# wq2012/SpectralCluster

Measured on AMD Instinct MI355X. Metric: predict() calls/sec, n=8192 d=256 ICASSP2018 (GraphCut, eigengap k in [2,20], cosine k-means), higher is better.
Workload: dtype f64; 1 GPU; icassp2018_graphcut_n8192_d256_k8_max20; n_samples=8192, n_features=256, parallelism=replicas x1, collectives=none

## Files before the change

### include/spectralcluster_amd.h

```cpp
#ifndef SPECTRALCLUSTER_AMD_H_
#define SPECTRALCLUSTER_AMD_H_

#include <stddef.h>
#include <stdint.h>

#ifdef __cplusplus
extern "C" {
#endif

#define SC_ABI_VERSION 10
#define SC_MAX_OPS 16
#define SC_MAX_BLUR_RADIUS 32
#define SC_MAX_EIG 128
#define SC_MAX_STAGES 16

typedef struct sc_handle_s* sc_handle;

typedef enum sc_status {
  SC_OK = 0,
  SC_ERR_INVALID = -1,
  SC_ERR_OOM = -2,
  SC_ERR_HIP = -3,
  SC_ERR_NOT_CONVERGED = -4,
  SC_ERR_UNSUPPORTED = -5,
// ... 104 lines not shown

typedef struct sc_diag {
  int32_t n;
  int32_t n_clusters_raw;
  int32_t n_clusters;
  int32_t eig_path;
  double max_delta;
  int32_t n_eigenvalues;
  int32_t eig_descending;
  double eigenvalues[SC_MAX_EIG];
  int32_t eig_matvec_passes;
  int32_t eig_block;
  int32_t eig_basis;
  int32_t eig_cycles;
  double eig_max_residual;
  int32_t kmeans_iterations;
  int32_t symmetry_state;
  int32_t eig_host_chain;
  int32_t eig_fallback;
  float stage_ms[SC_MAX_STAGES];
  int32_t diffuse_path;
  int32_t free_candidates;
  int32_t free_overflow_rows;
  int32_t free_tiles_run;
} sc_diag;

int sc_abi_version(void);
int sc_struct_sizes(int* config_bytes, int* diag_bytes);

enum { SC_DTYPE_F64 = 0, SC_DTYPE_F32 = 1, SC_DTYPE_F16 = 2, SC_DTYPE_BF16 = 3 };
enum { SC_MEM_HOST = 0, SC_MEM_DEVICE = 1 };
typedef struct sc_array {
  const void* data;
  int32_t dtype;
  int32_t location;
  int64_t rows, cols;
  int64_t row_stride;
  int64_t col_stride;
} sc_array;
int sc_array_layout(int* array_bytes, int* field_offsets);
int sc_device_count(void);
int sc_device_info(int device, char* name, int name_len, char* arch, int arch_len,
                   int* compute_units, int64_t* total_mem_bytes);

int sc_create(int device, sc_handle* out);
int sc_destroy(sc_handle h);
int sc_reserve(sc_handle h, int n_max, int d_max);
const char* sc_last_error(sc_handle h);
int sc_synchronize(sc_handle h);
void* sc_stream(sc_handle h);
int sc_set_profiling(sc_handle h, int level);
int sc_set_diffuse_mode(sc_handle h, int mode);
int sc_set_free_prune(sc_handle h, int on);

int sc_config_default(sc_config* cfg);
int sc_gaussian_weights(double sigma, int32_t* radius, double* weights);
int sc_set_blur_weights(sc_handle h, int radius, const double* weights);

int sc_predict(sc_handle h, const double* x, int n, int d, const sc_config* cfg,
               int64_t* labels, sc_diag* diag);

int sc_predict_array(sc_handle h, const sc_array* x, const sc_config* cfg, int64_t* labels,
                     sc_diag* diag);

int sc_set_embeddings(sc_handle h, const double* x, int n, int d);
int sc_set_embeddings_array(sc_handle h, const sc_array* x);
int sc_compute_affinity(sc_handle h);
int sc_set_affinity(sc_handle h, const double* affinity, int n);
int sc_eig_ncluster(sc_handle h, const sc_config* cfg, sc_diag* diag);
int sc_num_eigenvalues(sc_handle h);
int sc_get_eigenvalues(sc_handle h, double* out, int count);
int sc_num_eigenvectors(sc_handle h);
int sc_get_eigenvectors(sc_handle h, double* out, int n, int ncols);
int sc_cluster(sc_handle h, const sc_config* cfg, int n_clusters,
               int64_t* labels, sc_diag* diag);
int sc_set_constraint(sc_handle h, const double* constraint_matrix, int n);
int sc_set_constraint_band(sc_handle h, const double* band, int n);
int sc_set_constraint_pairs(sc_handle h, const int32_t* rows, const int32_t* cols,
                            const double* vals, int count, int n);
int sc_constraint_pairs_info(sc_handle h, int* count, size_t* pair_bytes);
int sc_clear_constraint(sc_handle h);
int sc_apply_constraint(sc_handle h, const sc_config* cfg);
int sc_constraint_info(sc_handle h, int* kind, int* n, size_t* band_bytes,
                       size_t* dense_bytes);
int sc_run_resident(sc_handle h, const sc_config* cfg, int64_t* labels,
                    sc_diag* diag);
int sc_eig_ncluster_sweep(sc_handle h, const sc_config* cfg, const double* p_values, int count,
                          sc_diag* diags);
int sc_sweep_adopt(sc_handle h, const sc_config* cfg, int index, sc_diag* diag);
int sc_predict_batch(sc_handle h, const double* const* xs, const int* ns, int d,
                     int count, const sc_config* cfg, int64_t* const* labels,
                     sc_diag* diags);
int sc_predict_batch_streams(sc_handle h, const double* const* xs, const int* ns, int d,
                             int count, const sc_config* cfg, int64_t* const* labels,
                             sc_diag* diags, int streams);
int sc_predict_batch_grouped(sc_handle h, const double* const* xs, const int* ns, int d,
                             int count, const sc_config* cfg, int64_t* const* labels,
                             sc_diag* diags, int group);
int sc_predict_batch_arrays(sc_handle h, const sc_array* xs, int count, const sc_config* cfg,
                            int64_t* const* labels, sc_diag* diags, int group, int streams);
int sc_predict_batch_constrained(sc_handle h, const sc_array* xs, const double* const* bands,
                                 int count, const sc_config* cfg, int64_t* const* labels,
                                 sc_diag* diags, int group);
typedef struct sc_constraint_desc {
  int32_t kind;
  int32_t count;
// ... 69 lines not shown

typedef struct sc_pool_s* sc_pool;
enum { SC_POOL_CACHE = 0, SC_POOL_CENTROIDS = 1 };
int sc_pool_create(sc_handle h, int capacity, int d, int u1, int u2, sc_pool* out);
int sc_pool_destroy(sc_pool pool);
int sc_pool_reset(sc_pool pool, int slot);
int sc_pool_rows(sc_pool pool, int slot);
int sc_pool_append(sc_pool pool, const int32_t* slots, const int32_t* counts, int count,
                   const sc_array* rows);
int sc_pool_precluster(sc_pool pool, const int32_t* slots, int count, int64_t* const* labels_out);
int sc_pool_centroids(sc_pool pool, int slot, sc_array* out);
int sc_pool_fallback(sc_pool pool, const int32_t* slots, int count, double distance_threshold,
                     int64_t* const* labels_out);
int sc_pool_cache(sc_pool pool, int slot, sc_array* out);
int sc_pool_get(sc_pool pool, int slot, int what, double* out);
int sc_pool_compress(sc_pool pool, int slot);

int sc_affinity_stats(sc_handle h, double* out);
int sc_affinity_gmm_bic(sc_handle h, int diagonal_offset, double* bic1, double* bic2);
int sc_naive_cluster(sc_handle h, const double* x, int n, int d, double threshold,
                     double adaptation_threshold, double* centroids, int32_t* counts,
                     int32_t* n_centroids, int capacity, int64_t* labels);

int sc_stage_ingest(sc_handle h, const sc_array* x, double* out);
int sc_stage_affinity(sc_handle h, const double* x, int n, int d, double* out);
int sc_stage_refine(sc_handle h, int op, const sc_config* cfg, const double* in,
                    int n, double* out);
int sc_stage_constraint(sc_handle h, const sc_config* cfg, const double* affinity,
                        const double* constraint_matrix, int n, double* out);
int sc_stage_constraint_band(sc_handle h, const sc_config* cfg, const double* affinity,
                             const double* band, int n, double* out);
int sc_stage_constraint_band_group(sc_handle h, const sc_config* cfg, int count, const int32_t* ns,
                                   const double* const* affinities, const double* const* bands,
                                   double* const* outs);
int sc_stage_constraint_pairs(sc_handle h, const sc_config* cfg, const double* affinity,
                              const int32_t* rows, const int32_t* cols, const double* vals,
                              int count, int n, double* out);
int sc_stage_constraint_pairs_group(sc_handle h, const sc_config* cfg, int count,
                                    const int32_t* ns, const double* const* affinities,
                                    const int32_t* const* rows, const int32_t* const* cols,
                                    const double* const* vals, const int32_t* counts,
                                    double* const* outs);
int sc_stage_diffuse_rowstats(sc_handle h, const double* a, int n, int mode, double* rowmax,
                              double* rowsum, int32_t* info);
enum {
  SC_BLOCK_ROUTE_SYM = 1,
  SC_BLOCK_ROUTE_TWO_PRODUCT = 2,
  SC_BLOCK_ROUTE_GROUPED = 4
};
int sc_stage_block_operator(sc_handle h, int count, const int32_t* ns,
                            const double* const* matrices, const double* const* cvecs,
                            const double* const* pvecs, const double* const* vs_scales,
                            const double* const* vs, double* const* ws, int route);
int sc_stage_krylov_state(sc_handle h, int32_t* info, double* q, double* t, double* g, double* c,
                          double* p);
enum { SC_FRONT_ROUTE_SINGLE = 0, SC_FRONT_ROUTE_GROUPED = 1, SC_FRONT_ROUTE_SWEEP = 2,
       SC_FRONT_ROUTE_SHORT_SWEEP = 3, SC_FRONT_ROUTE_SHORT_WAVE = 4 };
enum {
  SC_FRONT_INFO_DIFFUSE_PATH = 0,
  SC_FRONT_INFO_SYMMETRIC = 1,
  SC_FRONT_INFO_FOLDED_ROWNORM = 2,
  SC_FRONT_INFO_FREE_OP = 3,
  SC_FRONT_INFO_DIGITS_FUSED = 4,
  SC_FRONT_INFO_BLUR_KERNEL = 5,
  SC_FRONT_INFO_BLUR_ROWS = 6,
  SC_FRONT_INFO_FREE_CANDIDATES = 7,
  SC_FRONT_INFO_FREE_OVERFLOW_ROWS = 8,
  SC_FRONT_INFO_FREE_FORMS_S = 9,
  SC_FRONT_INFO_CROP_SOURCE = 10,
  SC_FRONT_INFO_CUT_KERNEL = 11,
  SC_FRONT_INFO_WRITTEN = 12,
  SC_FRONT_INFO_LAUNCHES = 13,
  SC_FRONT_INFO_COUNT = 16
};
typedef struct sc_front_out {
  double* a0;
  double* cropval;
  double* cut;
  double* a;
  double* s;
  double* rowmax;
  double* rowsum;
  double* c;
  double* p;
  double* t;
  int32_t info[SC_FRONT_INFO_COUNT];
} sc_front_out;
int sc_stage_front(sc_handle h, int route, const sc_config* cfg, int count, const int32_t* ns,
                   int d, const double* const* xs, const double* affinity,
                   const double* p_values, sc_front_out* outs);
enum { SC_TD_BACKTRANSFORM_GLOBAL = 1 };
int sc_stage_tridiag(sc_handle h, const double* m, int n, const double* c, const double* p,
                     double* d, double* e, double* tau, double* reflectors);
int sc_stage_tridiag_values(sc_handle h, const double* d, const double* e, int n,
                            double* values_desc);
int sc_stage_td_backtransform(sc_handle h, const double* reflectors, const double* tau, int n,
                              double* z, int cols, int flags);
int sc_stage_laplacian(sc_handle h, int laplacian_type, const double* in, int n,
                       double* out);
int sc_stage_sym_eig(sc_handle h, const double* m, int n, int count, int descend,
                     double* values, double* vectors, sc_diag* diag);
int sc_stage_eig(sc_handle h, const double* m, int n, int count, int descend,
                 double* values, double* vectors, sc_diag* diag);
int sc_random_state_doubles(uint32_t seed, int count, double* out);
int sc_uniform_choice(int n, double u);
int sc_host_symmetric_eig(const double* a, int m, double* values, double* vectors);
int sc_host_symmetric_eig_partial(const double* a, int m, int need, double* values,
                                  double* vectors);
// ... 59 lines not shown
```

### spectralcluster_amd/_lib.py

```python

from __future__ import annotations

import ctypes
import os
import threading
import typing

import numpy as np

SC_MAX_OPS = 16
SC_MAX_BLUR_RADIUS = 32
SC_MAX_EIG = 128
SC_MAX_STAGES = 16

SC_OK = 0
SC_ERR_INVALID = -1
SC_ERR_OOM = -2
SC_ERR_HIP = -3
SC_ERR_NOT_CONVERGED = -4
SC_ERR_UNSUPPORTED = -5
SC_ERR_NON_FINITE = -6

STAGE_NAMES = ("affinity", "refine", "diffuse", "scaling", "eig", "kmeans",
               "total", "blur", "threshold_sym", "matvec", "affinity_gemm",
# ... 138 lines not shown
      ("threshold", ctypes.c_double),
  ]


class ScConstraintDesc(ctypes.Structure):
  _fields_ = [
      ("kind", ctypes.c_int32),
      ("count", ctypes.c_int32),
      ("band", ctypes.POINTER(ctypes.c_double)),
      ("rows", ctypes.POINTER(ctypes.c_int32)),
      ("cols", ctypes.POINTER(ctypes.c_int32)),
      ("vals", ctypes.POINTER(ctypes.c_double)),
  ]


SC_AUTOTUNE_PERCENTILE_OVER_NME, SC_AUTOTUNE_PERCENTILE_SQRT_OVER_NME = 1, 2


class ScAutoTune(ctypes.Structure):
  _fields_ = [
      ("p_min", ctypes.c_double),
      ("p_max", ctypes.c_double),
      ("step", ctypes.c_double),
      ("levels", ctypes.c_int32),
      ("proxy", ctypes.c_int32),
  ]


AUTOTUNE_EVALUATE = ctypes.CFUNCTYPE(ctypes.c_int, _c_double_p, ctypes.c_int, _c_double_p,
                                     ctypes.c_void_p)

_c_int64_p = ctypes.POINTER(ctypes.c_int64)
_c_int_p = ctypes.POINTER(ctypes.c_int)
_handle_t = ctypes.c_void_p

PROTOTYPES = {
    "sc_abi_version": (ctypes.c_int, []),
    "sc_struct_sizes": (ctypes.c_int, [ctypes.POINTER(ctypes.c_int),
                                       ctypes.POINTER(ctypes.c_int)]),
    "sc_array_layout": (ctypes.c_int, [ctypes.POINTER(ctypes.c_int),
                                       ctypes.POINTER(ctypes.c_int)]),
    "sc_device_count": (ctypes.c_int, []),
    "sc_device_info": (ctypes.c_int, [ctypes.c_int, ctypes.c_char_p, ctypes.c_int,
                                      ctypes.c_char_p, ctypes.c_int, _c_int_p,
                                      _c_int64_p]),
    "sc_create": (ctypes.c_int, [ctypes.c_int, ctypes.POINTER(_handle_t)]),
    "sc_destroy": (ctypes.c_int, [_handle_t]),
    "sc_reserve": (ctypes.c_int, [_handle_t, ctypes.c_int, ctypes.c_int]),
    "sc_last_error": (ctypes.c_char_p, [_handle_t]),
    "sc_synchronize": (ctypes.c_int, [_handle_t]),
    "sc_set_profiling": (ctypes.c_int, [_handle_t, ctypes.c_int]),
    "sc_set_diffuse_mode": (ctypes.c_int, [_handle_t, ctypes.c_int]),
    "sc_set_free_prune": (ctypes.c_int, [_handle_t, ctypes.c_int]),
    "sc_stage_diffuse_rowstats": (ctypes.c_int, [_handle_t, _c_double_p, ctypes.c_int,
                                                 ctypes.c_int, _c_double_p, _c_double_p,
                                                 ctypes.POINTER(ctypes.c_int32)]),
    "sc_stage_block_operator": (ctypes.c_int, [_handle_t, ctypes.c_int,
                                               ctypes.POINTER(ctypes.c_int32),
                                               ctypes.POINTER(_c_double_p),
                                               ctypes.POINTER(_c_double_p),
                                               ctypes.POINTER(_c_double_p),
                                               ctypes.POINTER(_c_double_p),
                                               ctypes.POINTER(_c_double_p),
                                               ctypes.POINTER(_c_double_p), ctypes.c_int]),
    "sc_stage_krylov_state": (ctypes.c_int, [_handle_t, ctypes.POINTER(ctypes.c_int32),
                                             _c_double_p, _c_double_p, _c_double_p, _c_double_p,
                                             _c_double_p]),
    "sc_stage_front": (ctypes.c_int, [_handle_t, ctypes.c_int, ctypes.POINTER(ScConfig),
                                      ctypes.c_int, ctypes.POINTER(ctypes.c_int32), ctypes.c_int,
                                      ctypes.POINTER(_c_double_p), _c_double_p, _c_double_p,
                                      ctypes.POINTER(ScFrontOut)]),
    "sc_stage_tridiag": (ctypes.c_int, [_handle_t, _c_double_p, ctypes.c_int, _c_double_p,
                                        _c_double_p, _c_double_p, _c_double_p, _c_double_p,
                                        _c_double_p]),
    "sc_stage_tridiag_values": (ctypes.c_int, [_handle_t, _c_double_p, _c_double_p, ctypes.c_int,
                                               _c_double_p]),
    "sc_stage_td_backtransform": (ctypes.c_int, [_handle_t, _c_double_p, _c_double_p,
                                                 ctypes.c_int, _c_double_p, ctypes.c_int,
                                                 ctypes.c_int]),
    "sc_config_default": (ctypes.c_int, [ctypes.POINTER(ScConfig)]),
    "sc_gaussian_weights": (ctypes.c_int, [ctypes.c_double,
                                           ctypes.POINTER(ctypes.c_int32),
                                           _c_double_p]),
    "sc_predict": (ctypes.c_int, [_handle_t, _c_double_p, ctypes.c_int, ctypes.c_int,
                                  ctypes.POINTER(ScConfig), _c_int64_p,
                                  ctypes.POINTER(ScDiag)]),
    "sc_set_embeddings": (ctypes.c_int, [_handle_t, _c_double_p, ctypes.c_int,
                                         ctypes.c_int]),
    "sc_predict_array": (ctypes.c_int, [_handle_t, ctypes.POINTER(ScArray),
                                        ctypes.POINTER(ScConfig), _c_int64_p,
                                        ctypes.POINTER(ScDiag)]),
    "sc_set_embeddings_array": (ctypes.c_int, [_handle_t, ctypes.POINTER(ScArray)]),
    "sc_predict_batch_arrays": (ctypes.c_int, [_handle_t, ctypes.POINTER(ScArray), ctypes.c_int,
                                               ctypes.POINTER(ScConfig),
                                               ctypes.POINTER(_c_int64_p),
                                               ctypes.POINTER(ScDiag), ctypes.c_int,
                                               ctypes.c_int]),
    "sc_predict_batch_constrained": (ctypes.c_int, [_handle_t, ctypes.POINTER(ScArray),
                                                    ctypes.POINTER(_c_double_p), ctypes.c_int,
                                                    ctypes.POINTER(ScConfig),
                                                    ctypes.POINTER(_c_int64_p),
                                                    ctypes.POINTER(ScDiag), ctypes.c_int]),
    "sc_constraint_desc_layout": (ctypes.c_int, [ctypes.POINTER(ctypes.c_int),
                                                 ctypes.POINTER(ctypes.c_int)]),
    "sc_predict_batch_constraints": (ctypes.c_int, [_handle_t, ctypes.POINTER(ScArray),
                                                    ctypes.POINTER(ScConstraintDesc), ctypes.c_int,
                                                    ctypes.POINTER(ScConfig),
                                                    ctypes.POINTER(_c_int64_p),
                                                    ctypes.POINTER(ScDiag), ctypes.c_int]),
    "sc_stage_ingest": (ctypes.c_int, [_handle_t, ctypes.POINTER(ScArray), _c_double_p]),
    "sc_compute_affinity": (ctypes.c_int, [_handle_t]),
    "sc_set_affinity": (ctypes.c_int, [_handle_t, _c_double_p, ctypes.c_int]),
    "sc_eig_ncluster": (ctypes.c_int, [_handle_t, ctypes.POINTER(ScConfig),
                                       ctypes.POINTER(ScDiag)]),
    "sc_num_eigenvalues": (ctypes.c_int, [_handle_t]),
    "sc_get_eigenvalues": (ctypes.c_int, [_handle_t, _c_double_p, ctypes.c_int]),
    "sc_num_eigenvectors": (ctypes.c_int, [_handle_t]),
    "sc_get_eigenvectors": (ctypes.c_int, [_handle_t, _c_double_p, ctypes.c_int,
                                           ctypes.c_int]),
    "sc_cluster": (ctypes.c_int, [_handle_t, ctypes.POINTER(ScConfig), ctypes.c_int,
# ... 422 lines not shown
```

### spectralcluster_amd/csrc/api.hip

```cpp
#include <algorithm>
#include <array>
#include <cmath>
#include <cstdio>
#include <cstdlib>
#include <cstring>
#include <vector>

#include <condition_variable>
#include <mutex>
#include <string>
#include <thread>

#include "handle.h"
#include "host_pool.h"

int ensure_matrices(sc_handle h, int n, int d, bool affinity_copy) {
  h->krylov_m = 0;
  const size_t ldn = matrix_ld(n);
  const size_t nn = (size_t)n * ldn * sizeof(double);
  if (affinity_copy) SC_TRY(grow(h, h->A0, nn));
  SC_TRY(grow(h, h->B1, nn));
  SC_TRY(grow(h, h->B2, nn));
  if (d > 0) {
    const size_t ldx = round_up(d, 16);
// ... 3 lines not shown
  const size_t nv = (size_t)round_up(n, 16) * sizeof(double);
  SC_TRY(grow(h, h->rowmax, nv));
  SC_TRY(grow(h, h->rowsum, nv));
  SC_TRY(grow(h, h->cvec, nv));
  SC_TRY(grow(h, h->pvec, nv));
  SC_TRY(grow(h, h->tvec, nv));
  SC_TRY(grow(h, h->deg, nv));
  SC_TRY(grow(h, h->splitk, gemm_splitk_workspace_bytes()));
  SC_TRY(grow(h, h->dvec, nv));
  SC_TRY(grow(h, h->cut, nv));
  SC_TRY(grow(h, h->cropval, nv));
  SC_TRY(grow(h, h->statp, (size_t)2 * n * gemm_tile_dim(n) * sizeof(double)));
  SC_TRY(grow(h, h->rmpart, (size_t)n * blur_tile_columns(n, 8) * sizeof(double)));
  SC_TRY(grow(h, h->blurw, (2 * SC_MAX_BLUR_RADIUS + 1) * sizeof(double)));
  return SC_OK;
}

int ensure_tilemap(sc_handle h, int n) {
  const int nt = gemm_tile_dim(n);
  if (nt <= kTilemapTableMax) {
    if (!h->tilemap_table.p) {
      std::vector<int2> all, one;
      for (int t = 1; t <= kTilemapTableMax; ++t) {
        h->tilemap_off[t] = (int)all.size();
        gemm_build_sym_tilemap(t, &one);
        all.insert(all.end(), one.begin(), one.end());
      }
      SC_TRY(grow(h, h->tilemap_table, all.size() * sizeof(int2)));
      SC_HIP(h, hipMemcpyAsync(h->tilemap_table.p, all.data(), all.size() * sizeof(int2),
                               hipMemcpyHostToDevice, h->stream));
      SC_HIP(h, hipStreamSynchronize(h->stream));
    }
    h->tilemap_cur = ptr<int2>(h->tilemap_table) + h->tilemap_off[nt];
    return SC_OK;
  }
  if (h->tilemap_nt != nt) {
    std::vector<int2> map;
    gemm_build_sym_tilemap(nt, &map);
    SC_TRY(grow(h, h->tilemap, map.size() * sizeof(int2)));
    SC_HIP(h, hipMemcpyAsync(h->tilemap.p, map.data(), map.size() * sizeof(int2),
                             hipMemcpyHostToDevice, h->stream));
    SC_HIP(h, hipStreamSynchronize(h->stream));
    h->tilemap_nt = nt;
  }
  h->tilemap_cur = ptr<int2>(h->tilemap);
  return SC_OK;
}

int ensure_eig(sc_handle h, int n) {
  const size_t nq = (size_t)n * kLdq * sizeof(double);
  if (h->Q.bytes < nq) h->krylov_m = 0;
  SC_TRY(grow(h, h->Q, nq));
  SC_TRY(grow(h, h->Q2, nq));
  SC_TRY(grow(h, h->Vs, (size_t)n * kEigBlock * sizeof(double)));
  SC_TRY(grow(h, h->W, (size_t)n * kEigBlock * sizeof(double)));
  SC_TRY(grow(h, h->partial, std::max((size_t)kProjBlocks * kLdq * kEigBlock,
                                       lz_partial_doubles(n)) * sizeof(double)));
  SC_TRY(grow(h, h->T, (size_t)kLdq * kLdq * sizeof(double)));
  SC_TRY(grow(h, h->Y, (size_t)kLdq * kLdq * sizeof(double)));
  SC_TRY(grow(h, h->Yt, (size_t)kLdq * kLdq * sizeof(double)));
  SC_TRY(grow(h, h->theta, kLdq * sizeof(double)));
  SC_TRY(grow(h, h->resid, kLdq * sizeof(double)));
  SC_TRY(grow(h, h->G, 256 * sizeof(double)));
  SC_TRY(grow(h, h->Rinv, 256 * sizeof(double)));
  SC_TRY(grow(h, h->Hbuf, (size_t)kLdq * kEigBlock * sizeof(double)));
  SC_TRY(grow(h, h->hsq, 16 * sizeof(double)));
  SC_TRY(grow(h, h->colnorm, (size_t)kProjBlocks * kMaxVectors * sizeof(double)));
  if (h->flags.bytes < 16 * sizeof(int)) {
    SC_TRY(grow(h, h->flags, 16 * sizeof(int)));
    SC_HIP(h, hipMemsetAsync(h->flags.p, 0, 16 * sizeof(int), h->stream));
  }
  SC_TRY(grow(h, h->mvsym, matvec_sym_workspace_doubles(n) * sizeof(double)));
  SC_TRY(ensure_vectors(h, n, kMaxCols));
  return SC_OK;
}

int ensure_vectors(sc_handle h, int n, int cols) {
  cols = std::max(cols, kMaxCols);
  SC_TRY(grow(h, h->E, (size_t)round_up(n, 16) * cols * sizeof(double)));
  SC_TRY(grow(h, h->Eio, (size_t)n * cols * sizeof(double)));
  return SC_OK;
}

int ensure_gen(sc_handle h, int n) {
  const size_t ldv = round_up(n, 16);
  const size_t nv = ldv * sizeof(double);
  SC_TRY(grow(h, h->crvec, nv));
  SC_TRY(grow(h, h->thetai, kLdq * sizeof(double)));
  SC_TRY(grow(h, h->Vre, ldv * kGenMax * sizeof(double)));
  SC_TRY(grow(h, h->Vim, ldv * kGenMax * sizeof(double)));
  SC_TRY(grow(h, h->gpart, (size_t)gen_residual_blocks(n) * 32 * sizeof(double)));
  SC_TRY(grow(h, h->gsrc, 16 * sizeof(int)));
  SC_TRY(grow(h, h->genL, (size_t)kGenMax * kGenMax * sizeof(double)));
  return SC_OK;
}

extern "C" int sc_abi_version(void) { return SC_ABI_VERSION; }
extern "C" int sc_struct_sizes(int* config_bytes, int* diag_bytes) {
  if (config_bytes) *config_bytes = (int)sizeof(sc_config);
  if (diag_bytes) *diag_bytes = (int)sizeof(sc_diag);
  return SC_OK;
}

extern "C" int sc_device_count(void) {
  int c = 0;
  if (hipGetDeviceCount(&c) != hipSuccess) return 0;
  return c;
}

extern "C" int sc_device_info(int device, char* name, int name_len, char* arch,
                              int arch_len, int* compute_units,
                              int64_t* total_mem_bytes) {
  hipDeviceProp_t prop;
  if (hipGetDeviceProperties(&prop, device) != hipSuccess) return SC_ERR_HIP;
  if (name && name_len > 0) snprintf(name, name_len, "%s", prop.name);
  if (arch && arch_len > 0) snprintf(arch, arch_len, "%s", prop.gcnArchName);
  if (compute_units) *compute_units = prop.multiProcessorCount;
  if (total_mem_bytes) *total_mem_bytes = (int64_t)prop.totalGlobalMem;
  return SC_OK;
}


extern "C" int sc_create(int device, sc_handle* out) {
  if (!out) return SC_ERR_INVALID;
  *out = nullptr;
  int count = 0;
  if (hipGetDeviceCount(&count) != hipSuccess || count <= 0) return SC_ERR_HIP;
  if (device < 0 || device >= count) return SC_ERR_INVALID;
  sc_handle h = new sc_handle_s();
  h->device = device;
  if (hipSetDevice(device) != hipSuccess ||
      hipStreamCreateWithFlags(&h->stream, hipStreamNonBlocking) != hipSuccess) {
    delete h;
    return SC_ERR_HIP;
  }
  const unsigned ev_flags = hipEventDisableSystemFence;
  for (int i = 0; i < 48; ++i) {
    if (hipEventCreateWithFlags(&h->ev[i], ev_flags) != hipSuccess) {
      delete h;
      return SC_ERR_HIP;
    }
  }
  if (hipHostMalloc(reinterpret_cast<void**>(&h->h_theta), 3 * kLdq * sizeof(double)) !=
          hipSuccess ||
      hipHostMalloc(reinterpret_cast<void**>(&h->h_flags), 16 * sizeof(int)) !=
          hipSuccess ||
      hipHostMalloc(reinterpret_cast<void**>(&h->h_rr),
                    (2 * kHostRRSingle * kHostRRSingle + 64) * sizeof(double)) != hipSuccess) {
    delete h;
    return SC_ERR_HIP;
  }
  *out = h;
  return SC_OK;
}

extern "C" int sc_destroy(sc_handle h) {
  if (!h) return SC_OK;
  for (sc_handle sub : h->pool) sc_destroy(sub);
  h->pool.clear();
  for (sc_handle sub : h->gslots) sc_destroy(sub);
  h->gslots.clear();
  for (sc_handle sub : h->gshort) sc_destroy(sub);
  h->gshort.clear();
  hipSetDevice(h->device);
  hipStreamSynchronize(h->stream);
  DevBuf* bufs[] = {&h->X,     &h->Xn,    &h->A0,     &h->B1,      &h->B2,    &h->rowmax,
                    &h->rowsum, &h->cvec,  &h->pvec,   &h->tvec,    &h->deg,   &h->blurw, &h->blur_tmp, &h->dvec, &h->cut, &h->rmpart, &h->splitk, &h->tilemap, &h->tilemap_table, &h->cropval, &h->statp, &h->crvec, &h->thetai, &h->Vre, &h->Vim, &h->gpart, &h->gsrc, &h->genL, &h->ahc_size, &h->ahc_chain, &h->ahc_Z, &h->ahc_lab, &h->ahc_cent, &h->fb_part, &h->fb_small, &h->sck_slots, &h->sck_part, &h->sck_rec, &h->sck_mats, &h->fb_x, &h->fb_cent, &h->fb_int, &h->Cq, &h->Cband, &h->Cpairs, &h->Cporig, &h->cp[0], &h->cp[1], &h->cp[2], &h->cp[3], &h->cp[4], &h->symflag,
                    &h->Q,     &h->Q2,    &h->Vs,     &h->W,       &h->partial, &h->T,
                    &h->Y,     &h->Yt,    &h->theta,  &h->resid,   &h->G,     &h->Rinv,
                    &h->Hbuf,  &h->hsq,   &h->colnorm, &h->flags,  &h->E,     &h->Ek,   &h->Eio,
                    &h->td_d,  &h->td_e,  &h->td_theta, &h->td_work, &h->td_tau, &h->td_panel, &h->mvsym,
                    &h->kXc,   &h->kxsq,  &h->kclosest, &h->kcand, &h->kenorm, &h->krnd,
                    &h->kcent, &h->klab32, &h->klab64, &h->kinfo, &h->kchain, &h->gkrnd, &h->gpack, &h->gypack, &h->ginfo, &h->glabels, &h->gjtab, &h->gsftab, &h->gswtab,
                    &h->kbig, &h->kbigw, &h->fq, &h->ft32, &h->fy1, &h->fR, &h->fscal, &h->fwords, &h->fcand, &h->fY, &h->fsplit, &h->fypart, &h->frpart, &h->fq2part, &h->fmx64, &h->ftau64, &h->fplan, &h->Xalt, &h->Xstage, &h->gneg};
  for (DevBuf* b : bufs)
    if (b->p) hipFree(b->p);
  for (DevBuf& b : h->kgen)
    if (b.p) hipFree(b.p);
  for (int i = 0; i < 48; ++i) hipEventDestroy(h->ev[i]);
  if (h->h_theta) hipHostFree(h->h_theta);
  if (h->h_flags) hipHostFree(h->h_flags);
  if (h->h_rr) hipHostFree(h->h_rr);
  if (h->h_free) hipHostFree(h->h_free);
  if (h->h_reduce) hipHostFree(h->h_reduce);
  if (h->h_sck) hipHostFree(h->h_sck);
  if (h->sync_ev) hipEventDestroy(h->sync_ev);
  for (int b = 0; b < kGroupBanks; ++b) {
    if (h->gbank_ev[b]) hipEventDestroy(h->gbank_ev[b]);
    if (h->gbank_stream[b]) hipStreamDestroy(h->gbank_stream[b]);
  }
  if (h->gchain_stream) hipStreamDestroy(h->gchain_stream);
  if (h->copy_stream) hipStreamDestroy(h->copy_stream);
  if (h->gcheck_ev) hipEventDestroy(h->gcheck_ev);
  for (sc_handle lane : h->glanes) sc_destroy(lane);
  h->glanes.clear();
  delete h->gpool;
  if (h->h_gpack) hipHostFree(h->h_gpack);
  if (h->h_gypack) hipHostFree(h->h_gypack);
  if (h->h_gjtab) hipHostFree(h->h_gjtab);
  if (h->h_gsftab) hipHostFree(h->h_gsftab);
  if (h->h_gswtab) hipHostFree(h->h_gswtab);
// ... 1142 lines not shown
```

### spectralcluster_amd/csrc/eig.hip

```cpp
#include <algorithm>
#include <cstring>
#include <mutex>

#include "sc_internal.h"

namespace sc {

typedef double v4f64 __attribute__((ext_vector_type(4)));
constexpr int B = kEigBlock;
constexpr int RB = 256 / B;
static_assert(B == 8 || B == 16, "block width must divide the 16-wide MFMA tile");

__device__ __forceinline__ uint64_t splitmix64(uint64_t x) {
  x += 0x9E3779B97F4A7C15ull;
  x = (x ^ (x >> 30)) * 0xBF58476D1CE4E5B9ull;
  x = (x ^ (x >> 27)) * 0x94D049BB133111EBull;
  return x ^ (x >> 31);
}
__device__ __forceinline__ double hash_uniform(uint64_t seed, uint64_t idx) {
  const uint64_t h = splitmix64(seed ^ splitmix64(idx));
  return (double)(h >> 11) * (2.0 / 9007199254740992.0) - 1.0;
}

__global__ void k_random_block(double* W, int n, uint64_t seed) {
// ... 39 lines not shown
  for (; ch < nchunks; ch += kMvWaves) {
    if (ch + kMvWaves < nchunks) load(nxt, ch + kMvWaves);
    const int kb = ch * 32 + 2 * lg;
    double b[8];
#pragma unroll
    for (int t = 0; t < 8; ++t) {
      const int k = kb + 8 * (t >> 1) + (t & 1);
      b[t] = (k < n && li < B) ? Vs[(size_t)k * B + li] : 0.0;
    }
#pragma unroll
    for (int q = 0; q < 4; ++q) {
      const double a0 = (kb + 8 * q < n) ? cur[q].x : 0.0;
      const double a1 = (kb + 8 * q + 1 < n) ? cur[q].y : 0.0;
      acc0 = __builtin_amdgcn_mfma_f64_16x16x4f64(a0, b[2 * q], acc0, 0, 0, 0);
      acc1 = __builtin_amdgcn_mfma_f64_16x16x4f64(a1, b[2 * q + 1], acc1, 0, 0, 0);
    }
#pragma unroll
    for (int q = 0; q < 4; ++q) cur[q] = nxt[q];
  }
#pragma unroll
  for (int r = 0; r < 4; ++r) red[wave][lane][r] = acc0[r] + acc1[r];
  __syncthreads();
  if (wave == 0) {
#pragma unroll
    for (int r = 0; r < 4; ++r) {
      double sum = 0.0;
#pragma unroll
      for (int w = 0; w < kMvWaves; ++w) sum += red[w][lane][r];
      const int row = r0 + lg + 4 * r;
      if (row < n && li < B)
        W[(size_t)row * B + li] =
            __builtin_fma(cvec ? cvec[row] : 1.0, sum,
                          pvec ? pvec[row] * V[(size_t)row * ldv + li] : 0.0);
    }
  }
}
__global__ __launch_bounds__(64 * kMvWaves) void k_block_matvec(
    const double* __restrict__ S, int ld, int n, const double* __restrict__ cvec,
    const double* __restrict__ pvec, const double* __restrict__ V, int ldv,
    const double* __restrict__ Vs, double* __restrict__ W) {
  block_matvec_body(S, ld, n, cvec, pvec, V, ldv, Vs, W);
}
__global__ __launch_bounds__(64 * kMvWaves) void k_block_matvec_g(const GroupOf<MatvecItem> g) {
  const MatvecItem& a = g.s[blockIdx.y];
  if ((int)blockIdx.x * 16 >= a.n) return;
  block_matvec_body(a.S, a.ld, a.n, a.cvec, a.pvec, a.V, a.ldv, a.Vs, a.W);
}

constexpr int kSymTile = 128;
constexpr int kSymPitch = 34;
__device__ __forceinline__ int sym_item_id(int I, int J, int nt) {
  return I * nt - I * (I - 1) / 2 + (J - I);
}
__device__ __forceinline__ void block_matvec_sym_body(
    const double* __restrict__ S, int ld, int n, const double* __restrict__ Vs,
    double* __restrict__ pdirect, double* __restrict__ pmirror, int nt) {
  __shared__ __attribute__((aligned(16))) double smem[4 * 32 * kSymPitch];
  int I = 0, rem = blockIdx.x, rowlen = nt;
  while (rem >= rowlen) {
    rem -= rowlen;
    --rowlen;
    ++I;
  }
  const int J = I + rem;
  const bool diag = I == J;
  const int lane = threadIdx.x & 63, wave = threadIdx.x >> 6;
  const int li = lane & 15, lg = lane >> 4;
  const int r0 = I * kSymTile + 32 * wave;
  const int c0 = J * kSymTile;
  double* patch = smem + wave * (32 * kSymPitch);
  double bm[8];
#pragma unroll
  for (int t = 0; t < 8; ++t) {
    const int row = r0 + 4 * t + lg;
    bm[t] = (row < n && li < B) ? Vs[(size_t)row * B + li] : 0.0;
  }
  v4f64 accd[2] = {{0.0, 0.0, 0.0, 0.0}, {0.0, 0.0, 0.0, 0.0}};
  v4f64 accm[4][2];
#pragma unroll
  for (int cs = 0; cs < 4; ++cs)
#pragma unroll
    for (int ct = 0; ct < 2; ++ct) accm[cs][ct] = (v4f64){0.0, 0.0, 0.0, 0.0};
  double2 a[1][2][4];
  auto load = [&](int buf, int cs) {
#pragma unroll
    for (int rt = 0; rt < 2; ++rt) {
      int row = r0 + 16 * rt + li;
      row = row < n ? row : n - 1;
      const double* src = S + (size_t)row * ld + c0 + 32 * cs + 2 * lg;
#pragma unroll
      for (int q = 0; q < 4; ++q) {
        if (c0 + 32 * cs + 8 * q + 2 * lg + 1 < ld)
          a[buf][rt][q] = *reinterpret_cast<const double2*>(src + 8 * q);
        else
          a[buf][rt][q] = make_double2(0.0, 0.0);
      }
    }
  };
#pragma unroll
  for (int cs = 0; cs < 4; ++cs) {
    constexpr int cur = 0;
    load(cur, cs);
    const int kb = c0 + 32 * cs + 2 * lg;
#pragma unroll
    for (int rt = 0; rt < 2; ++rt) {
      const bool rok = r0 + 16 * rt + li < n;
#pragma unroll
      for (int q = 0; q < 4; ++q) {
        if (!rok || kb + 8 * q >= n) a[cur][rt][q].x = 0.0;
        if (!rok || kb + 8 * q + 1 >= n) a[cur][rt][q].y = 0.0;
      }
    }
    double b[8];
#pragma unroll
    for (int t = 0; t < 8; ++t) {
      const int k = kb + 8 * (t >> 1) + (t & 1);
      b[t] = (k < n && li < B) ? Vs[(size_t)k * B + li] : 0.0;
    }
#pragma unroll
    for (int rt = 0; rt < 2; ++rt)
#pragma unroll
      for (int q = 0; q < 4; ++q) {
        accd[rt] = __builtin_amdgcn_mfma_f64_16x16x4f64(a[cur][rt][q].x, b[2 * q], accd[rt], 0, 0, 0);
        accd[rt] = __builtin_amdgcn_mfma_f64_16x16x4f64(a[cur][rt][q].y, b[2 * q + 1], accd[rt], 0, 0, 0);
      }
    if (!diag) {
#pragma unroll
      for (int rt = 0; rt < 2; ++rt)
#pragma unroll
        for (int q = 0; q < 4; ++q)
          *reinterpret_cast<double2*>(patch + (16 * rt + li) * kSymPitch + 8 * q + 2 * lg) =
              a[cur][rt][q];
      __builtin_amdgcn_fence(__ATOMIC_RELEASE, "wavefront");
      __builtin_amdgcn_wave_barrier();
#pragma unroll
      for (int ct = 0; ct < 2; ++ct)
#pragma unroll
        for (int t = 0; t < 8; ++t) {
          const double at = patch[(4 * t + lg) * kSymPitch + 16 * ct + li];
          accm[cs][ct] = __builtin_amdgcn_mfma_f64_16x16x4f64(at, bm[t], accm[cs][ct], 0, 0, 0);
        }
      __builtin_amdgcn_fence(__ATOMIC_ACQUIRE, "wavefront");
      __builtin_amdgcn_wave_barrier();
    }
  }
  const size_t item = blockIdx.x;
  if (li < B) {
#pragma unroll
    for (int rt = 0; rt < 2; ++rt)
#pragma unroll
      for (int r = 0; r < 4; ++r)
        pdirect[(item * kSymTile + 32 * wave + 16 * rt + lg + 4 * r) * B + li] = accd[rt][r];
  }
  if (diag) return;
  __syncthreads();
  double* red = smem;
  if (li < B) {
#pragma unroll
    for (int cs = 0; cs < 4; ++cs)
#pragma unroll
      for (int ct = 0; ct < 2; ++ct)
#pragma unroll
        for (int r = 0; r < 4; ++r)
          red[(wave * kSymTile + 32 * cs + 16 * ct + lg + 4 * r) * B + li] = accm[cs][ct][r];
  }
  __syncthreads();
  for (int e = threadIdx.x; e < kSymTile * B; e += 256)
    pmirror[item * (kSymTile * B) + e] =
        ((red[e] + red[kSymTile * B + e]) + red[2 * kSymTile * B + e]) + red[3 * kSymTile * B + e];
}
__global__ __launch_bounds__(256) void k_block_matvec_sym(
    const double* __restrict__ S, int ld, int n, const double* __restrict__ Vs,
    double* __restrict__ pdirect, double* __restrict__ pmirror, int nt) {
  block_matvec_sym_body(S, ld, n, Vs, pdirect, pmirror, nt);
}
__global__ __launch_bounds__(256) void k_block_matvec_sym_g(const GroupOf<MatvecItem> g) {
  const MatvecItem& a = g.s[blockIdx.y];
  const int nt = (a.n + kSymTile - 1) / kSymTile;
  if ((int)blockIdx.x >= nt * (nt + 1) / 2) return;
  block_matvec_sym_body(a.S, a.ld, a.n, a.Vs, a.slabs, a.slabs + (size_t)(nt * (nt + 1) / 2) * kSymTile * B, nt);
}

__device__ __forceinline__ void matvec_sym_reduce_body(
    const double* __restrict__ pdirect, const double* __restrict__ pmirror, int nt, int n,
    const double* __restrict__ cvec, const double* __restrict__ pvec,
    const double* __restrict__ V, int ldv, double* __restrict__ W) {
  const int R = blockIdx.x / 4;
  const int e = (blockIdx.x & 3) * 256 + threadIdx.x;
  const int rl = e / B, v = e % B;
  const int row = R * kSymTile + rl;
  double acc = 0.0;
  const int total = nt;
  for (int s0 = 0; s0 < total; s0 += 8) {
    double x[8];
#pragma unroll
    for (int u = 0; u < 8; ++u) {
      const int sidx = s0 + u;
      x[u] = 0.0;
      if (sidx < nt - R) {
        x[u] = pdirect[(size_t)sym_item_id(R, R + sidx, nt) * (kSymTile * B) + e];
      } else if (sidx < total) {
        x[u] = pmirror[(size_t)sym_item_id(sidx - (nt - R), R, nt) * (kSymTile * B) + e];
      }
    }
#pragma unroll
    for (int u = 0; u < 8; ++u) acc += x[u];
  }
  if (row < n) W[(size_t)row * B + v] =
      __builtin_fma(cvec ? cvec[row] : 1.0, acc, pvec ? pvec[row] * V[(size_t)row * ldv + v] : 0.0);
}
__global__ __launch_bounds__(256) void k_matvec_sym_reduce(
    const double* __restrict__ pdirect, const double* __restrict__ pmirror, int nt, int n,
    const double* __restrict__ cvec, const double* __restrict__ pvec,
    const double* __restrict__ V, int ldv, double* __restrict__ W) {
  matvec_sym_reduce_body(pdirect, pmirror, nt, n, cvec, pvec, V, ldv, W);
}
__global__ __launch_bounds__(256) void k_matvec_sym_reduce_g(const GroupOf<MatvecItem> g) {
  const MatvecItem& a = g.s[blockIdx.y];
  const int nt = (a.n + kSymTile - 1) / kSymTile;
  if ((int)blockIdx.x >= nt * 4) return;
  matvec_sym_reduce_body(a.slabs, a.slabs + (size_t)(nt * (nt + 1) / 2) * kSymTile * B, nt, a.n,
                         a.cvec, a.pvec, a.V, a.ldv, a.W);
}

constexpr int kProjGroups = 256 / B;
constexpr int kProjAcc = (kLdq + kProjGroups - 1) / kProjGroups;
__global__ __launch_bounds__(256) void k_proj_partial(
    const double* __restrict__ Q, int ldq, int m, const double* __restrict__ W,
    int n, double* __restrict__ partial) {
  __shared__ double Ql[8][kLdq];
  __shared__ double Wl[8][B];
  const int tid = threadIdx.x;
  const int jj = tid % B, ig = tid / B;
  const int rows_per = (n + gridDim.x - 1) / gridDim.x;
  const int rbeg = blockIdx.x * rows_per;
  const int rend = min(n, rbeg + rows_per);
  double acc[kProjAcc];
#pragma unroll
  for (int q = 0; q < kProjAcc; ++q) acc[q] = 0.0;
  for (int r = rbeg; r < rend; r += 8) {
    __syncthreads();
    for (int e = tid; e < 8 * m; e += 256) {
      const int rr = e / m, i = e - rr * m;
      Ql[rr][i] = (r + rr < rend) ? Q[(size_t)(r + rr) * ldq + i] : 0.0;
    }
    if (tid < 8 * B) {
      const int rr = tid / B;
      Wl[rr][jj] = (r + rr < rend) ? W[(size_t)(r + rr) * B + jj] : 0.0;
    }
    __syncthreads();
#pragma unroll
    for (int rr = 0; rr < 8; ++rr) {
      const double w = Wl[rr][jj];
#pragma unroll
      for (int q = 0; q < kProjAcc; ++q)
        if (ig + kProjGroups * q < m)
          acc[q] = __builtin_fma(Ql[rr][ig + kProjGroups * q], w, acc[q]);
    }
  }
  double* out = partial + (size_t)blockIdx.x * (kLdq * B);
#pragma unroll
  for (int q = 0; q < kProjAcc; ++q)
    if (ig + kProjGroups * q < m) out[(ig + kProjGroups * q) * B + jj] = acc[q];
}

__global__ __launch_bounds__(256) void k_reduce_H(
    const double* __restrict__ partial, int nparts, int m, double* __restrict__ Hbuf,
    double* __restrict__ T, int ldt, int col0, int accumulate,
    double* __restrict__ hsq) {
  __shared__ double sq[32];
  const int tid = threadIdx.x;
  const int sub = tid & 7;
  const int e = blockIdx.x * 32 + (tid >> 3);
  double h = 0.0;
// ... 91 lines not shown
  const double gii = __shfl(g, i * 9), gjj = __shfl(g, j * 9);
  double defect = 0.0;
  if (flag_mode == 2 && gii != 0.0 && gjj != 0.0) defect = fabs(g - (i == j ? 1.0 : 0.0));
#pragma unroll
  for (int o = 1; o < 64; o <<= 1) defect = fmax(defect, __shfl_xor(defect, o));
  double r = 0.0;
  int mask = 0;
  double pmax = 0.0, pmin = __builtin_huge_val();
#pragma unroll
  for (int k = 0; k < B; ++k) {
    const double d = __shfl(g, k * 9);
    const double total = __shfl(gii, k * 8) + (hsq ? hsq[k] : 0.0);
    const bool drop = !(d > 1e-22 * total) || !(d > 0.0);
    const double rk = drop ? 0.0 : sqrt(d);
    if (drop) {
      mask |= 1 << k;
    } else {
      pmax = fmax(pmax, rk);
      pmin = fmin(pmin, rk);
    }
    double row = 0.0;
    if (i == k && !drop) row = j == k ? rk : (j > k ? g / rk : 0.0);
    if (i == k) r = row;
    const double rki = __shfl(row, k * 8 + i), rkj = __shfl(row, k * 8 + j);
    if (i > k && j > k) g -= rki * rkj;
  }
  const double rii = __shfl(r, i * 9), rjj = __shfl(r, j * 9);
  double ri = 0.0;
#pragma unroll
  for (int srow = B - 1; srow >= 0; --srow) {
    double v = 0.0;
#pragma unroll
    for (int k = srow + 1; k < B; ++k) {
      const double rsk = __shfl(r, srow * 8 + k), rkj = __shfl(ri, k * 8 + j);
      if (k <= j) v -= rsk * rkj;
    }
    if (i == srow && j >= i && rii != 0.0 && rjj != 0.0)
      ri = i == j ? 1.0 / rii : v / rii;
  }
  Rinv[tid] = ri;
  if (tid == 0 && flags != nullptr) {
    flags[0] = mask;
    if (defect_flag != nullptr) *defect_flag = (defect > 0.1 || pmax > 1e3 * pmin) ? 1 : 0;
    if (sticky_flag != nullptr && (mask != 0 || (sticky_on_defect && defect > 0.1))) {
      if (*sticky_flag == 0) {
        sticky_flag[1] = sticky_m;
        sticky_flag[2] = flag_mode * 1000 + mask;
      }
      *sticky_flag = 1;
    }
  }
}

__global__ __launch_bounds__(256) void k_apply_rinv(
    double* __restrict__ W, int n, const double* __restrict__ Rinv,
    double* __restrict__ Qdst, int ldq, int col0, const double* __restrict__ cvec,
    double* __restrict__ Vs) {
  __shared__ double Rl[B * B];
  const int tid = threadIdx.x;
  if (tid < B * B) Rl[tid] = Rinv[tid];
  __syncthreads();
  const int jj = tid % B;
  const int r = blockIdx.x * RB + tid / B;
  const double w = r < n ? W[(size_t)r * B + jj] : 0.0;
  double v = 0.0;
#pragma unroll
  for (int k = 0; k < B; ++k) {
    const double wk = __shfl(w, k, B);
    v = __builtin_fma(wk, Rl[k * B + jj], v);
  }
  if (r < n) {
    W[(size_t)r * B + jj] = v;
    if (Qdst) Qdst[(size_t)r * ldq + col0 + jj] = v;
    if (Vs) Vs[(size_t)r * B + jj] = cvec[r] * v;
  }
}

constexpr int kLzThreads = 512;
constexpr int kLzPartStride = (kLdq + B) * B;
struct LzStep {
  double* W;
  int n;
  const double* Q;
  int ldq, m;
  int pre;
  const double* pre_partial;
  int pre_nparts;
  double* T;
  int ldt, col0;
  double* Gsave;
  double* hsq;
  int* flags;
  int arm_defect;
  double* Tzero;
  double* Qdst;
  int store_col;
  const double* vs_scale;
  double* Vs;
  int init_random;
  uint64_t seed;
  int want_proj, want_gram;
  double* partial;
};

__device__ __forceinline__ double lz_ordered_sum(const double* src, int nparts) {
  double acc = 0.0;
  for (int p0 = 0; p0 < nparts; p0 += 16) {
    double v[16];
#pragma unroll
    for (int u = 0; u < 16; ++u)
      v[u] = (p0 + u < nparts) ? src[(size_t)(p0 + u) * kLzPartStride] : 0.0;
#pragma unroll
    for (int u = 0; u < 16; ++u) acc += v[u];
  }
  return acc;
}

template <int ROWS>
__device__ __forceinline__ void lz_rows_body(const LzStep& a) {
  extern __shared__ __attribute__((aligned(16))) double smem[];
  constexpr int kPass = kLzThreads / B;
  const int m = a.m;
  const int mq = m + 1;
  double* Ql = smem;
  double* Hl = Ql + ROWS * mq;
  double* Rl = Hl + kLdq * B;
  double* Wl = Rl + B * B;
  double* Gs = Wl + ROWS * B;
  double* hs = Gs + B * B;
  const int tid = threadIdx.x;
  const int j = tid % B;
  const int r0 = blockIdx.x * ROWS;
  const bool first_wg = blockIdx.x == 0;
  const bool pre_proj = (a.pre >= 1 && a.pre <= 3) && m > 0;
  const bool pre_gram = a.pre >= 2;
  const bool use_h = pre_proj;
  const bool use_r = pre_gram;
  const bool use_q = m > 0 && (use_h || a.want_proj);
  const int nproj = pre_proj ? m * B : 0;
  double hsum[3] = {0.0, 0.0, 0.0};
#pragma unroll
  for (int u = 0; u < 3; ++u) {
    const int e = tid + u * kLzThreads;
    if (e < nproj) hsum[u] = lz_ordered_sum(a.pre_partial + e, a.pre_nparts);
    else if (pre_gram && e < nproj + B * B)
      hsum[u] = lz_ordered_sum(a.pre_partial + kLdq * B + (e - nproj), a.pre_nparts);
  }
  double told[3] = {0.0, 0.0, 0.0};
  double hsq_old = 0.0;
  if (first_wg && a.pre == 2) {
#pragma unroll
    for (int u = 0; u < 3; ++u) {
      const int e = tid + u * kLzThreads;
      if (e < nproj) told[u] = a.T[(size_t)(e / B) * a.ldt + a.col0 + (e % B)];
    }
    if (tid < B) hsq_old = a.hsq[tid];
  }
  if (!first_wg && a.pre == 2 && tid < B) hsq_old = a.hsq[tid];
  if (use_q)
    for (int e = tid; e < ROWS * m; e += kLzThreads) {
      const int rr = e / m, i = e - rr * m;
      Ql[rr * mq + i] = (r0 + rr < a.n) ? a.Q[(size_t)(r0 + rr) * a.ldq + i] : 0.0;
    }
  double w[ROWS / kPass];
#pragma unroll
  for (int q = 0; q < ROWS / kPass; ++q) {
    const int r = r0 + q * kPass + tid / B;
    w[q] = 0.0;
    if (r < a.n)
      w[q] = a.init_random ? hash_uniform(a.seed, (uint64_t)r * B + j) : a.W[(size_t)r * B + j];
  }
#pragma unroll
  for (int u = 0; u < 3; ++u) {
    const int e = tid + u * kLzThreads;
    if (e < nproj) Hl[e] = hsum[u];
    else if (pre_gram && e < nproj + B * B) Gs[e - nproj] = hsum[u];
  }
  if (tid < B * B) Rl[tid] = (tid / B == tid % B) ? 1.0 : 0.0;
  __syncthreads();
  if (pre_proj && a.pre != 3) {
    if (first_wg && a.T != nullptr) {
#pragma unroll
      for (int u = 0; u < 3; ++u) {
        const int e = tid + u * kLzThreads;
        if (e < nproj) {
          const int i = e / B, jc = a.col0 + (e % B);
          if (i <= jc) {
            const double t = a.pre == 2 ? told[u] + hsum[u] : hsum[u];
            a.T[(size_t)i * a.ldt + jc] = t;
            a.T[(size_t)jc * a.ldt + i] = t;
          }
        }
      }
    }
    if (tid < B) {
      double sq = 0.0;
      for (int i = 0; i < m; ++i) sq = __builtin_fma(Hl[i * B + tid], Hl[i * B + tid], sq);
      sq = a.pre == 2 ? hsq_old + sq : sq;
      if (first_wg && a.pre == 1) a.hsq[tid] = sq;
      hs[tid] = sq;
    }
  } else if (tid < B) {
    hs[tid] = 0.0;
  }
  if (first_wg && a.Tzero != nullptr)
    for (int e = tid; e < kLdq * kLdq; e += kLzThreads) a.Tzero[e] = 0.0;
  if (pre_gram) {
    if (pre_proj && tid < B * B) {
      const int a1 = tid / B, b1 = tid % B;
      double g = Gs[tid];
      for (int i = 0; i < m; ++i) g = __builtin_fma(-Hl[i * B + a1], Hl[i * B + b1], g);
      Gs[tid] = g;
    }
    __syncthreads();
    if (first_wg && a.pre == 2 && a.Gsave != nullptr && tid < B * B) a.Gsave[tid] = Gs[tid];
    if (tid < 64)
      chol8_wave(Gs, Rl, a.pre == 2 ? hs : nullptr, first_wg ? a.flags : nullptr,
                 first_wg ? a.flags + (a.pre == 3 ? 10 : 11) : nullptr, a.pre == 3 ? 2 : 1,
                 first_wg ? a.flags + 13 : nullptr, m, a.arm_defect != 0);
    __syncthreads();
  }
#pragma unroll
  for (int q = 0; q < ROWS / kPass; ++q) {
    const int rl = q * kPass + tid / B;
    const int r = r0 + rl;
    double x = w[q];
    if (use_h)
      for (int i = 0; i < m; ++i) x = __builtin_fma(-Ql[rl * mq + i], Hl[i * B + j], x);
    double v = x;
    if (use_r) {
      v = 0.0;
#pragma unroll
      for (int k = 0; k < B; ++k) v = __builtin_fma(__shfl(x, k, B), Rl[k * B + j], v);
    }
    if (r < a.n) {
      a.W[(size_t)r * B + j] = v;
      if (a.Qdst) a.Qdst[(size_t)r * a.ldq + a.store_col + j] = v;
      if (a.Vs) a.Vs[(size_t)r * B + j] = a.vs_scale[r] * v;
    }
    Wl[rl * B + j] = (r < a.n) ? v : 0.0;
  }
  if (!a.want_proj && !a.want_gram) return;
  __syncthreads();
  const int oproj = a.want_proj ? m * B : 0;
  const int nent = oproj + (a.want_gram ? B * B : 0);
  double* mine = a.partial + (size_t)blockIdx.x * kLzPartStride;
  for (int base = 0; base < nent; base += kLzThreads / 2) {
    const int e = base + (tid >> 1), half = tid & 1;
    double acc = 0.0;
    if (e < nent) {
      const int rbeg = half * (ROWS / 2);
      if (e < oproj) {
        const int i = e / B, jj = e % B;
#pragma unroll 8
        for (int rr = 0; rr < ROWS / 2; ++rr)
          acc = __builtin_fma(Ql[(rbeg + rr) * mq + i], Wl[(rbeg + rr) * B + jj], acc);
      } else {
        const int g = e - oproj, a1 = g / B, b1 = g % B;
#pragma unroll 8
        for (int rr = 0; rr < ROWS / 2; ++rr)
          acc = __builtin_fma(Wl[(rbeg + rr) * B + a1], Wl[(rbeg + rr) * B + b1], acc);
      }
    }
    const double other = __shfl_xor(acc, 1);
    if (e < nent && half == 0)
      mine[e < oproj ? e : kLdq * B + (e - oproj)] = acc + other;
  }
}
template <int ROWS>
__global__ __launch_bounds__(kLzThreads) void k_lz_rows(const LzStep a) {
  lz_rows_body<ROWS>(a);
}
template <int ROWS>
__global__ __launch_bounds__(kLzThreads) void k_lz_rows_g(const GroupOf<LzStep> g) {
  const LzStep& a = g.s[blockIdx.y];
  if ((int)blockIdx.x * ROWS >= a.n) return;
  lz_rows_body<ROWS>(a);
}

__device__ __forceinline__ double fast_rcp(double x) {
  double r = __builtin_amdgcn_rcp(x);
  r = __builtin_fma(r, __builtin_fma(-x, r, 1.0), r);
  r = __builtin_fma(r, __builtin_fma(-x, r, 1.0), r);
  return r;
}
__device__ __forceinline__ double fast_rsqrt(double x) {
  double y = __builtin_amdgcn_rsq(x);
  y = __builtin_fma(y, 0.5 * __builtin_fma(-x * y, y, 1.0), y);
  y = __builtin_fma(y, 0.5 * __builtin_fma(-x * y, y, 1.0), y);
  return y;
}

template <bool YT_LDS>
__device__ __forceinline__ void jacobi_body(
    const double* __restrict__ src, int ldsrc, int m, int mode,
    const double* __restrict__ cvec, const double* __restrict__ pvec,
    const double* __restrict__ G, double* __restrict__ theta,
    double* __restrict__ Y, int ldy, double* __restrict__ resid,
    double* __restrict__ Yt_global, int* __restrict__ dbg) {
  extern __shared__ __attribute__((aligned(16))) double smem[];
  const long long t_begin = wall_clock64();
  const long long c_begin = clock64();
  const int mp = (m + 1) & ~1;
  const int lda = mp + 1;
  double* A = smem;
  double* cs = A + mp * lda;
  double* sn = cs + mp / 2;
  int* pp = reinterpret_cast<int*>(sn + mp / 2);
  int* qq = pp + mp / 2;
  double* Yl = sn + mp / 2 + mp / 2 + 2;
#define Yt(idx) (*(YT_LDS ? &Yl[idx] : &Yt_global[idx]))
  __shared__ int s_rot;
  const int tid = threadIdx.x;
  const int nth = blockDim.x;

  for (int e = tid; e < mp * mp; e += nth) {
    const int i = e / mp, j = e - i * mp;
    double v = 0.0;
    if (i < m && j < m) {
      v = src[(size_t)i * ldsrc + j];
      if (mode == 1) {
        v = cvec[i] * v * cvec[j];
        if (i == j) v += pvec[i];
      }
    }
    A[i * lda + j] = v;
    Yt((size_t)i * mp + j) = (i == j) ? 1.0 : 0.0;
  }
  __syncthreads();
  if (mode == 1) {
// ... 283 lines not shown
}
__global__ __launch_bounds__(256) void k_back_transform_g(const GroupOf<RitzItem> g) {
  const RitzItem& a = g.s[blockIdx.y];
  if ((int)blockIdx.x >= a.cols || a.n <= 0) return;
  back_transform_body(a.E, a.lde, a.n, a.tvec);
}
__device__ __forceinline__ void dense_vectors_member(const JacobiItem& a) {
  const int j = blockIdx.x;
  if (j >= a.m) return;
  for (int r = threadIdx.x; r < a.m; r += blockDim.x)
    a.E[(size_t)j * a.lde + r] = a.Y[(size_t)r * a.ldy + j];
  __syncthreads();
  back_transform_body(a.E, a.lde, a.m, a.tvec);
}
__global__ __launch_bounds__(256) void k_dense_vectors_g(const GroupOf<JacobiItem> g) {
  dense_vectors_member(g.s[blockIdx.y]);
}
__global__ __launch_bounds__(256) void k_dense_vectors_t(const JacobiItem* __restrict__ table) {
  const JacobiItem a = table[blockIdx.y];
  dense_vectors_member(a);
}

__global__ void k_rowmajor_to_colmajor(const double* __restrict__ src, int lds, int n,
                                       int cols, double* __restrict__ dst, int ldd) {
  const int e = blockIdx.x * blockDim.x + threadIdx.x;
  if (e >= n * cols) return;
  const int j = e / n, r = e - j * n;
  dst[(size_t)j * ldd + r] = src[(size_t)r * lds + j];
}
__global__ void k_colmajor_to_rowmajor(const double* __restrict__ src, int lds, int n,
                                       int cols, double* __restrict__ dst, int ldd) {
  const int e = blockIdx.x * blockDim.x + threadIdx.x;
  if (e >= n * cols) return;
  const int r = e / cols, j = e - r * cols;
  dst[(size_t)r * ldd + j] = src[(size_t)j * lds + r];
}

int proj_blocks(int n) { return std::max(1, std::min(kProjBlocks, (n + 63) / 64)); }
void launch_random_block(hipStream_t s, double* W, int n, uint64_t seed) {
  hipLaunchKernelGGL(k_random_block, dim3((n * B + 255) / 256), dim3(256), 0, s, W, n,
                     seed);
}
void launch_refill_deficient(hipStream_t s, double* W, int n, const int* flags,
                             uint64_t seed) {
  hipLaunchKernelGGL(k_refill_deficient, dim3((n * B + 255) / 256), dim3(256), 0, s,
                     W, n, flags, seed);
}
void launch_block_matvec(hipStream_t s, const double* S, int ld, int n,
                         const double* cvec, const double* pvec, const double* V,
                         int ldv, const double* Vs, double* W) {
  hipLaunchKernelGGL(k_block_matvec, dim3((n + 15) / 16), dim3(64 * kMvWaves), 0, s, S,
                     ld, n, cvec, pvec, V, ldv, Vs, W);
}
size_t matvec_sym_workspace_doubles(int n) {
  const size_t nt = (size_t)(n + kSymTile - 1) / kSymTile;
  return 2 * (nt * (nt + 1) / 2) * kSymTile * B;
}
void launch_block_matvec_sym(hipStream_t s, const double* S, int ld, int n, const double* cvec,
                             const double* pvec, const double* V, int ldv, const double* Vs,
                             double* W, double* ws) {
  const int nt = (n + kSymTile - 1) / kSymTile;
  const int items = nt * (nt + 1) / 2;
  double* pd = ws;
  double* pm = ws + (size_t)items * kSymTile * B;
  hipLaunchKernelGGL(k_block_matvec_sym, dim3(items), dim3(256), 0, s, S, ld, n, Vs, pd, pm, nt);
  hipLaunchKernelGGL(k_matvec_sym_reduce, dim3(nt * 4), dim3(256), 0, s, pd, pm, nt, n, cvec,
                     pvec, V, ldv, W);
}
void launch_proj_partial(hipStream_t s, const double* Q, int ldq, int m,
                         const double* W, int n, double* partial) {
  hipLaunchKernelGGL(k_proj_partial, dim3(proj_blocks(n)), dim3(256), 0, s, Q, ldq, m, W,
                     n, partial);
}
void launch_reduce_H(hipStream_t s, const double* partial, int nparts, int m, double* Hbuf,
                     double* T, int ldt, int col0, int accumulate, double* hsq) {
  hipLaunchKernelGGL(k_reduce_H, dim3((m * B + 31) / 32), dim3(256), 0, s, partial,
                     nparts, m, Hbuf, T, ldt, col0, accumulate, hsq);
}
void launch_update_block(hipStream_t s, const double* Q, int ldq, int m,
                         const double* Hbuf, double* W, int n) {
  hipLaunchKernelGGL(k_update_block, dim3((n + RB - 1) / RB), dim3(256), 0, s, Q, ldq, m,
                     Hbuf, W, n);
}
void launch_reduce_chol(hipStream_t s, const double* partial, int nparts, double* Rinv,
                        double* Gsave, const double* hsq, int* flags, int* defect_flag,
                        int flag_mode) {
  hipLaunchKernelGGL(k_reduce_chol, dim3(1), dim3(256), 0, s, partial, nparts,
                     Rinv, Gsave, hsq, flags, defect_flag, flag_mode);
}
void launch_apply_rinv(hipStream_t s, double* W, int n, const double* Rinv,
                       double* Qdst, int ldq, int col0, const double* cvec,
                       double* Vs) {
  hipLaunchKernelGGL(k_apply_rinv, dim3((n + RB - 1) / RB), dim3(256), 0, s, W, n, Rinv,
                     Qdst, ldq, col0, cvec, Vs);
}
static int lz_rows_for(int m) {
  if ((size_t)128 * (m + 1) * sizeof(double) <= 112 * 1024) return 128;
  if ((size_t)256 * (m + 1) * sizeof(double) <= 96 * 1024) return 256;
  if ((size_t)128 * (m + 1) * sizeof(double) <= 112 * 1024) return 128;
  return 64;
}
size_t lz_partial_doubles(int n) { return 2 * (size_t)((n + 63) / 64) * kLzPartStride; }

template <int ROWS>
static void launch_rows(hipStream_t s, const LzStep& a, int nwg) {
  const size_t lds = sizeof(double) * ((size_t)ROWS * (a.m + 1) + (size_t)kLdq * B + B * B +
                                       (size_t)ROWS * B + B * B + B);
  static std::once_flag once[16];
  int dev = 0;
  hipGetDevice(&dev);
  std::call_once(once[dev & 15], [] {
    hipFuncSetAttribute(reinterpret_cast<const void*>(k_lz_rows<ROWS>),
                        hipFuncAttributeMaxDynamicSharedMemorySize, 150 * 1024);
  });
  hipLaunchKernelGGL(k_lz_rows<ROWS>, dim3(nwg), dim3(kLzThreads), lds, s, a);
}

static LzStep lz_make_step(const EigWorkspace& ws, LzChain* chain, int n, int m, int pre,
                           int next, int store_col, const double* vs_scale, int col0,
                           bool init_random, uint64_t seed, bool zero_T) {
  LzStep a;
  a.arm_defect = (!chain->three_pass || store_col >= 0) ? 1 : 0;
  a.W = ws.W;
  a.n = n;
  a.Q = ws.Q;
  a.ldq = kLdq;
  a.m = m;
  a.pre = pre;
  const size_t half = lz_partial_doubles(n) / 2;
  a.pre_partial = ws.partial + (size_t)chain->parity * half;
  a.pre_nparts = chain->nparts;
  a.T = ws.T;
  a.ldt = kLdq;
  a.col0 = col0;
  a.Gsave = ws.G;
  a.hsq = ws.hsq;
  a.flags = ws.flags;
  a.Tzero = zero_T ? ws.T : nullptr;
  a.Qdst = store_col >= 0 ? ws.Q : nullptr;
  a.store_col = store_col >= 0 ? store_col : 0;
  a.vs_scale = vs_scale;
  a.Vs = store_col >= 0 ? ws.Vs : nullptr;
  a.init_random = init_random ? 1 : 0;
  a.seed = seed;
  a.want_proj = (next >= 1 && next <= 3 && m > 0) ? 1 : 0;
  a.want_gram = next >= 2 ? 1 : 0;
  chain->parity ^= 1;
  a.partial = ws.partial + (size_t)chain->parity * half;
  const int rows = lz_rows_for(m);
  chain->nparts = (n + rows - 1) / rows;
  return a;
}
void launch_lz_link(hipStream_t s, const EigWorkspace& ws, LzChain* chain, int n, int m,
                    int pre, int next, int store_col, const double* vs_scale, int col0,
                    bool init_random, uint64_t seed, bool zero_T) {
  const LzStep a = lz_make_step(ws, chain, n, m, pre, next, store_col, vs_scale, col0,
                                init_random, seed, zero_T);
  const int rows = lz_rows_for(m);
  const int nwg = chain->nparts;
  if (rows == 256) launch_rows<256>(s, a, nwg);
  else if (rows == 128) launch_rows<128>(s, a, nwg);
  else launch_rows<64>(s, a, nwg);
}

__global__ __launch_bounds__(256) void k_group_gather(const GroupOf<GatherItem> g, int m,
                                                      double* __restrict__ out, int stride) {
  const GatherItem& a = g.s[blockIdx.x];
  if (a.T == nullptr) return;
  double* dst = out + (size_t)blockIdx.x * stride;
  for (int e = threadIdx.x; e < m * m; e += 256) {
    const int i = e / m, j = e - i * m;
    dst[e] = a.T[(size_t)i * kLdq + j];
  }
  if (threadIdx.x < B * B) dst[m * m + threadIdx.x] = a.G[threadIdx.x];
  if (threadIdx.x < 16) reinterpret_cast<int*>(dst + m * m + B * B)[threadIdx.x] = a.flags[threadIdx.x];
}
void launch_group_gather(hipStream_t s, const GatherItem* items, int count, int m, double* out,
                         int stride) {
  GroupOf<GatherItem> g;
  memset(&g, 0, sizeof(g));
  for (int z = 0; z < count; ++z) g.s[z] = items[z];
  hipLaunchKernelGGL(k_group_gather, dim3(count), dim3(256), 0, s, g, m, out, stride);
}

template <int ROWS>
static void launch_rows_group(hipStream_t s, const GroupOf<LzStep>& g, int m, int nwg,
                              int count) {
  const size_t lds = sizeof(double) * ((size_t)ROWS * (m + 1) + (size_t)kLdq * B + B * B +
                                       (size_t)ROWS * B + B * B + B);
  SC_OPT_IN_LDS(k_lz_rows_g<ROWS>, 150 * 1024);
  hipLaunchKernelGGL(k_lz_rows_g<ROWS>, dim3(nwg, count), dim3(kLzThreads), lds, s, g);
}
void launch_lz_link_group(hipStream_t s, LzGroupMember* mem, int count, int m, int pre,
                          int next, int store_col, int col0, bool init_random, uint64_t seed,
                          bool zero_T) {
  GroupOf<LzStep> g;
  memset(&g, 0, sizeof(g));
  const int rows = lz_rows_for(m);
  int nwg = 0;
  for (int z = 0; z < count; ++z) {
    if (!mem[z].active) continue;
    g.s[z] = lz_make_step(mem[z].ws, &mem[z].chain, mem[z].n, m, pre, next, store_col,
                          mem[z].vs_scale, col0, init_random, seed, zero_T);
    mem[z].chain.nparts = (mem[z].n + rows - 1) / rows;
    nwg = std::max(nwg, mem[z].chain.nparts);
  }
  if (nwg == 0) return;
  if (rows == 256) launch_rows_group<256>(s, g, m, nwg, count);
  else if (rows == 128) launch_rows_group<128>(s, g, m, nwg, count);
  else launch_rows_group<64>(s, g, m, nwg, count);
}
void launch_block_matvec_group(hipStream_t s, const MatvecItem* items, int count,
// ... 134 lines not shown
```

### spectralcluster_amd/csrc/eig_driver.hip

```cpp
#include <ctime>

#include "handle.h"
#include "host_eig.h"
#include "host_pool.h"


static double value_error_bound(const double* theta, const double* resid, int m, int i,
                                bool symmetric) {
  const double r = resid[i];
  if (!symmetric || !(r > 0.0) || !std::isfinite(r)) return r;
  double delta = __builtin_huge_val();
  if (i > 0) delta = std::min(delta, theta[i - 1] - resid[i - 1] - theta[i]);
  if (i + 1 < m) delta = std::min(delta, theta[i] - theta[i + 1] - resid[i + 1]);
  else return r;
  delta -= r;
  if (!(delta > 0.0) || !std::isfinite(delta)) return r;
  return std::min(r, 2.0 * r * r / delta);
}

extern "C" int sc_host_value_error_bound(const double* theta, const double* resid, int m, int i,
                                         double* bound) {
  if (!theta || !resid || !bound || m < 1 || i < 0 || i >= m) return SC_ERR_INVALID;
  *bound = value_error_bound(theta, resid, m, i, true);
  return SC_OK;
// ... 75 lines not shown
        const double den_lo = b - eb + eps, den_hi = b + eb + eps;
        *upper = den_lo > 0.0 ? (a + ea) / den_lo : 1e300;
        *lower = den_hi > 0.0 ? (a - ea) / den_hi : -1e300;
      } else {
        *upper = (a - b + ea + eb) / wmax;
        *lower = (a - b - ea - eb) / wmax;
      }
    };
    double best_lo = 0.0, dummy;
    if (kb >= 1) {
      if (rq.descend) gap_bounds(kb, kb - 1, &best_lo, &dummy);
      else gap_bounds(kb - 1, kb, &best_lo, &dummy);
    }
    const int end = kw;
    if (rq.descend) {
      for (int i = 1; i < end && ok; ++i) {
        if (rq.use_stop) {
          if (std::fabs(w[i - 1] - rq.stop_eigenvalue) <= err(i - 1)) {
            ok = false; dc.fail_kind = 4; dc.fail_index = i - 1;
            break;
          }
          if (w[i - 1] < rq.stop_eigenvalue) break;
        }
        if (i == kb) continue;
        double lo, up;
        gap_bounds(i, i - 1, &lo, &up);
        if (!(up < best_lo) && !(kb == 0 && up <= 0.0)) {
          ok = false; dc.fail_kind = 4; dc.fail_index = i;
        }
      }
    } else {
      for (int i = 1; i < end - 1 && ok; ++i) {
        if (i + 1 == kb) continue;
        double lo, up;
        gap_bounds(i, i + 1, &lo, &up);
        if (!(up < best_lo) && !(kb == 0 && up <= 0.0)) {
          ok = false; dc.fail_kind = 4; dc.fail_index = i;
        }
      }
    }
  }
  for (int i = 0; i < dc.kvec; ++i) {
    if (!(resid[i] <= std::max(rq.vector_tol * scale, floor_abs))) {
      if (ok) { dc.fail_kind = 3; dc.fail_index = i; }
      ok = false;
    }
    dc.max_resid = std::max(dc.max_resid, resid[i]);
  }
  dc.converged = ok;
  return dc;
}

static bool block_multiplicity_suspect(const EigRequest& rq, const EigDecision& dc,
                                       const double* theta, int m) {
  const int kw = std::min(dc.kw, m);
  const int limit = rq.fixed_count > 0 ? kw - 2 : dc.n_clusters_raw - 1;
  const double rel = 10.0 * std::max(rq.value_tol, 1e-12);
  const double scale = std::max(std::fabs(theta[0]), std::fabs(theta[m - 1]));
  for (int i = 0; i + kEigBlock - 1 <= limit && i + kEigBlock - 1 < kw; ++i) {
    const double a = theta[i], b = theta[i + kEigBlock - 1];
    if (std::fabs(a - b) <= rel * std::max(std::max(std::fabs(a), std::fabs(b)), 1e-10 * scale))
      return true;
  }
  return false;
}

static bool host_rayleigh_ritz(const double* T, int ld, const double* G, int m, double* theta,
                               double* resid, double* Y, int ldy) {
  const int lda = m | 1;
  std::vector<double> a((size_t)m * lda), d(m), e(m);
  for (int i = 0; i < m; ++i)
    for (int j = 0; j < m; ++j)
      a[(size_t)i * lda + j] = i <= j ? T[(size_t)i * ld + j] : T[(size_t)j * ld + i];
  if (!host_symmetric_eig(a.data(), lda, m, d.data(), e.data())) return false;
  std::vector<int> order(m);
  for (int i = 0; i < m; ++i) order[i] = i;
  std::stable_sort(order.begin(), order.end(), [&](int x, int y) { return d[x] > d[y]; });
  for (int rank = 0; rank < m; ++rank) {
    const int c = order[rank];
    theta[rank] = d[c];
    double r2 = 0.0;
    for (int p = 0; p < kEigBlock; ++p) {
      double t = 0.0;
      for (int q = 0; q < kEigBlock; ++q)
        t += G[p * kEigBlock + q] * a[(size_t)(m - kEigBlock + q) * lda + c];
      r2 += a[(size_t)(m - kEigBlock + p) * lda + c] * t;
    }
    resid[rank] = std::sqrt(std::max(r2, 0.0));
    for (int r = 0; r < m; ++r) Y[(size_t)r * ldy + rank] = a[(size_t)r * lda + c];
  }
  return true;
}

template <typename CountFn>
static bool host_rayleigh_ritz_leading(const double* T, int ld, const double* G, int m,
                                       double* theta, double* resid, double* Y, int ldy,
                                       CountFn count_fn) {
  HostTridiag tw;
  if (!host_partial_values(T, ld, m, &tw)) return false;
  for (int i = 0; i < m; ++i) theta[i] = tw.theta[i];
  const int need = std::max(1, std::min(m, count_fn(theta)));
  for (int r = 0; r < m; ++r)
    for (int c = 0; c < m; ++c) Y[(size_t)r * ldy + c] = 0.0;
  if (!host_partial_vectors(tw, need, Y, ldy)) return false;
  for (int rank = 0; rank < m; ++rank) {
    if (rank >= need) {
      resid[rank] = __builtin_huge_val();
      continue;
    }
    double r2 = 0.0;
    for (int p = 0; p < kEigBlock; ++p) {
      double t = 0.0;
      for (int q = 0; q < kEigBlock; ++q)
        t += G[p * kEigBlock + q] * Y[(size_t)(m - kEigBlock + q) * ldy + rank];
      r2 += Y[(size_t)(m - kEigBlock + p) * ldy + rank] * t;
    }
    resid[rank] = std::sqrt(std::max(r2, 0.0));
  }
  return true;
}

static int cholqr_pass(sc_handle h, int n, int store_col, const double* vs_scale) {
  hipStream_t s = h->stream;
  double* W = ptr<double>(h->W);
  launch_proj_partial(s, W, kEigBlock, kEigBlock, W, n, ptr<double>(h->partial));
  launch_reduce_chol(s, ptr<double>(h->partial), proj_blocks(n), ptr<double>(h->Rinv), nullptr,
                     nullptr, ptr<int>(h->flags), ptr<int>(h->flags) + 10, 2);
  launch_apply_rinv(s, W, n, ptr<double>(h->Rinv), store_col >= 0 ? ptr<double>(h->Q) : nullptr,
                    kLdq, store_col >= 0 ? store_col : 0, vs_scale, ptr<double>(h->Vs));
  return SC_OK;
}

static const char kNonFiniteMessage[] = "Array must not contain infs or NaNs";

static int orthonormalize(sc_handle h, int n, int m, bool record, int col0, int store_col,
                          bool save_gram, const double* vs_scale) {
  hipStream_t s = h->stream;
  double* Q = ptr<double>(h->Q);
  double* W = ptr<double>(h->W);
  double* part = ptr<double>(h->partial);
  double* hsq = ptr<double>(h->hsq);
  SC_HIP(h, hipMemsetAsync(hsq, 0, 16 * sizeof(double), s));
  if (m > 0) {
    for (int pass = 0; pass < 2; ++pass) {
      launch_proj_partial(s, Q, kLdq, m, W, n, part);
      launch_reduce_H(s, part, proj_blocks(n), m, ptr<double>(h->Hbuf),
                      record ? ptr<double>(h->T) : nullptr, kLdq, col0, pass, hsq);
      launch_update_block(s, Q, kLdq, m, ptr<double>(h->Hbuf), W, n);
    }
  }
  launch_proj_partial(s, W, kEigBlock, kEigBlock, W, n, part);
  launch_reduce_chol(s, part, proj_blocks(n), ptr<double>(h->Rinv),
                     save_gram ? ptr<double>(h->G) : nullptr, hsq, ptr<int>(h->flags),
                     ptr<int>(h->flags) + 11, 1);
  launch_apply_rinv(s, W, n, ptr<double>(h->Rinv), nullptr, 0, 0, nullptr, nullptr);
  SC_TRY(cholqr_pass(h, n, store_col, vs_scale));
  return check_last(h, "orthonormalize launch");
}

static void trace_jacobi(sc_handle h) {
  if (h->h_flags[1] <= 0 || !sw::eig_trace()) return;
  fprintf(stderr, "[sc] jacobi sweeps=%d  %.1f us  %.0f MHz shader clock\n", h->h_flags[1],
          h->h_flags[2] * 0.01, h->h_flags[3] * 1024.0 / (h->h_flags[2] * 0.01));
  fprintf(stderr, "[sc]   thread-0 kcycles: param %d  barrier1 %d  update %d  barrier2 %d\n",
          h->h_flags[4], h->h_flags[5], h->h_flags[6], h->h_flags[7]);
  hipMemsetAsync(ptr<int>(h->flags) + 1, 0, 2 * sizeof(int), h->stream);
}

// ... 113 lines not shown

int sym_topk(sc_handle h, const FrontResult& op_in, int n, const EigRequest& rq_in,
             sc_diag* diag, EigDecision* out_dc, std::vector<double>* out_w) {
  hipStream_t s = h->stream;
  h->krylov_m = 0;
  SC_TRY(ensure_eig(h, n));
  FrontResult op = op_in;
  const int ld = op.ld;
  auto free_materialize = [&](bool with_stats) -> int {
    if (!op.free_op) return SC_OK;
    if (op.scratch == nullptr || op.scratch == op.matrix)
      return fail(h, SC_ERR_UNSUPPORTED, "no scratch matrix to form the Diffuse product in");
    SC_TRY(ensure_tilemap(h, n));
    GemmRowStats rs{1, ptr<double>(h->statp), ptr<double>(h->statp) + (size_t)n * gemm_tile_dim(n),
                    ptr<double>(h->rowmax), ptr<double>(h->rowsum)};
    launch_gemm_nt(s, op.matrix, ld, op.matrix, ld, op.scratch, ld, n, n, n, kEpiNone, true,
                   ptr<double>(h->splitk), h->tilemap_cur, with_stats ? &rs : nullptr);
    SC_TRY(check_last(h, "diffuse launch"));
    double* a_buffer = const_cast<double*>(op.matrix);
    op.matrix = op.scratch;
    op.scratch = a_buffer;
    op.free_op = false;
    return SC_OK;
  };
  auto free_check = [&](bool* restart) -> int {
    *restart = false;
    if (!op.free_op || h->free_checked) return SC_OK;
    bool changed = false, too_many = false;
    SC_TRY(free_fix_overflow(h, op.matrix, ld, n, &changed, &too_many));
    if (too_many) {
      SC_TRY(free_materialize(true));
      changed = true;
    }
    if (changed) {
      launch_scaling_vectors(s, ptr<double>(h->rowmax), ptr<double>(h->rowsum), n,
                             op.laplacian_type, op.folded_rownorm ? 1 : 0, ptr<double>(h->cvec),
                             ptr<double>(h->pvec), ptr<double>(h->tvec));
      launch_check_finite(s, ptr<double>(h->cvec), ptr<double>(h->pvec), n, ptr<int>(h->flags) + 12);
      SC_TRY(check_last(h, "scaling launch"));
      *restart = true;
    }
    return SC_OK;
  };
  double* theta_d = ptr<double>(h->theta);
  double* resid_d = ptr<double>(h->resid);
  const double* cvec = ptr<double>(h->cvec);
  const double* pvec = ptr<double>(h->pvec);
  EigDecision dc;
  int m = 0, passes = 0, cycles = 0;
  EigRequest rq = rq_in;
  bool fused = !sw::eig_host_chain() && !op.skip_fused;
  bool three_pass = false;
  const int sym_min_n = sw::matvec_sym_min_n();
  const bool sym_mv = n >= sym_min_n;
  EigDecision dense_dc;
  bool dense = false, many_vectors = false;
  auto run_dense = [&]() -> int {
    bool unused = false;
    SC_TRY(free_check(&unused));
    SC_TRY(free_materialize(false));
    SC_TRY(dense_spectrum(h, op.matrix, ld, n, op.scratch));
    std::vector<double> zeros(n, 0.0);
    dense_dc = analyze(rq_in, h->spectrum.data(), zeros.data(), n, n, true);
    if (!dense_dc.enough) return fail(h, SC_ERR_UNSUPPORTED, "eigen request cannot be satisfied");
    many_vectors = dense_dc.kvec > kMaxVectors;
    dense = true;
    rq = rq_in;
    rq.fixed_count = std::max(1, dense_dc.kvec);
    rq.value_tol = std::max(rq_in.value_tol, 1e-6);
    return SC_OK;
  };
  if (n > kDenseMax && wants_full_spectrum(rq_in)) SC_TRY(run_dense());
  bool vectors_from_dense = false;
  int fallback_reason = 0;
  auto dense_fallback = [&](int reason) -> int {
    if (op.scratch == nullptr || op.scratch == op.matrix)
      return fail(h, SC_ERR_NOT_CONVERGED,
                  "block Lanczos did not converge and no scratch matrix is free for the dense path");
    if (sw::eig_trace())
      fprintf(stderr, "[sc] block Lanczos gave up (reason %d, %d passes): dense path\n", reason,
              passes);
    if (!dense) SC_TRY(run_dense());
    SC_TRY(free_materialize(false));
    int cols = dense_dc.kvec;
    if (rq_in.fixed_count > 0 || rq_in.max_clusters > 0)
      cols = std::max(std::min(dense_dc.kw, kMaxVectors), cols);
    cols = std::max(1, cols);
    SC_TRY(dense_vectors(h, op.scratch, ld, n, cols));
    vectors_from_dense = true;
    fallback_reason = reason;
    return SC_OK;
  };

  if (n <= kDenseMax) {
    launch_jacobi(s, op.matrix, ld, n, 1, cvec, pvec, nullptr, theta_d, ptr<double>(h->Y), kLdq,
                  nullptr, ptr<double>(h->Yt), ptr<int>(h->flags));
    SC_TRY(check_last(h, "jacobi launch"));
    SC_HIP(h, hipMemcpyAsync(h->h_theta, theta_d, n * sizeof(double), hipMemcpyDeviceToHost, s));
    SC_HIP(h, hipMemcpyAsync(h->h_flags + 12, ptr<int>(h->flags) + 12, sizeof(int),
                             hipMemcpyDeviceToHost, s));
    if (sw::eig_trace())
      SC_HIP(h, hipMemcpyAsync(h->h_flags + 1, ptr<int>(h->flags) + 1, 7 * sizeof(int),
                               hipMemcpyDeviceToHost, s));
    SC_HIP(h, hipStreamSynchronize(s));
    if (h->h_flags[12] != 0) return fail(h, SC_ERR_NON_FINITE, kNonFiniteMessage);
    trace_jacobi(h);
    for (int i = 0; i < n; ++i) h->h_theta[kLdq + i] = 0.0;
    dc = analyze(rq, h->h_theta, h->h_theta + kLdq, n, n, true);
    if (!dc.enough) return fail(h, SC_ERR_UNSUPPORTED, "eigen request cannot be satisfied");
    m = n;
    const int cols = n;
    launch_rowmajor_to_colmajor(s, ptr<double>(h->Y), kLdq, n, cols, ptr<double>(h->E),
                                round_up(n, 16));
    back_transform_cols(h, n, cols);
    h->n_vec = cols;
    if (diag) diag->eig_path = SC_EIG_PATH_DENSE_JACOBI;
    dc.kw = n;
  } else {
  restart_lanczos:
    m = 0;
    cycles = 0;
    bool done = false;
    uint64_t seed = 0x5eed5eedull;
    LzChain chain;
    if (dense && many_vectors) {
      SC_TRY(dense_fallback(5));
      done = true;
    }
    if (done) {
    } else if (fused) {
      if (!op.chain_flags_cleared)
        SC_HIP(h, hipMemsetAsync(ptr<int>(h->flags) + 13, 0, 3 * sizeof(int), s));
      op.chain_flags_cleared = false;
      const EigWorkspace ws = eig_workspace(h);
      chain = LzChain();
      chain.three_pass = three_pass;
      launch_lz_link(s, ws, &chain, n, 0, 0, 4, -1, cvec, 0, true, seed, false);
      launch_lz_link(s, ws, &chain, n, 0, 4, 3, -1, cvec, 0, false, 0, true);
      launch_lz_link(s, ws, &chain, n, 0, 3, 0, 0, cvec, 0, false, 0, false);
      SC_TRY(check_last(h, "start block launch"));
    } else {
      launch_random_block(s, ptr<double>(h->W), n, seed);
      SC_TRY(orthonormalize(h, n, 0, false, 0, 0, false, cvec));
      const int rc0 = finish_block(h, n, 0, 0, cvec, &seed);
      if (rc0 == SC_ERR_NOT_CONVERGED) {
        SC_TRY(dense_fallback(3));
        done = true;
      } else {
        SC_TRY(rc0);
      }
      SC_HIP(h, hipMemsetAsync(h->T.p, 0, (size_t)kLdq * kLdq * sizeof(double), s));
    }
    if (!done && sw::eig_force_dense()) {
      SC_TRY(dense_fallback(4));
      done = true;
    }
    const int cap = std::min(kEigBasisCap, ((n - kEigBlock) / kEigBlock) * kEigBlock);
    const int first_check = std::min(3 * kEigBlock, cap);
    auto check_due = [&](int mm) {
      return cycles == 0 ? (mm >= first_check && (mm <= 4 * kEigBlock ||
                                                  mm % (2 * kEigBlock) == 0 || mm + kEigBlock > cap))
                         : (mm + kEigBlock > cap);
    };
    auto enqueue_step = [&](int m_before) -> int {
      const bool time_mv = h->profile_level >= 2 && h->n_mv_ev < 16;
      if (time_mv) ev_rec(h, &h->mv_ev[h->n_mv_ev][0]);
      if (op.free_op)
        free_apply_operator(h, op.matrix, ld, n, sym_mv, ptr<double>(h->Q) + m_before, kLdq);
      else if (sym_mv)
        launch_block_matvec_sym(s, op.matrix, ld, n, cvec, pvec, ptr<double>(h->Q) + m_before, kLdq,
                                ptr<double>(h->Vs), ptr<double>(h->W), ptr<double>(h->mvsym));
      else
        launch_block_matvec(s, op.matrix, ld, n, cvec, pvec, ptr<double>(h->Q) + m_before, kLdq,
                            ptr<double>(h->Vs), ptr<double>(h->W));
      if (time_mv) ev_rec(h, &h->mv_ev[h->n_mv_ev++][1]);
      ++passes;
      const int mm = m_before + kEigBlock;
      if (fused) {
        const EigWorkspace ws = eig_workspace(h);
        launch_lz_link(s, ws, &chain, n, mm, 0, 1, -1, cvec, mm - kEigBlock, false, 0, false);
        launch_lz_link(s, ws, &chain, n, mm, 1, 2, -1, cvec, mm - kEigBlock, false, 0, false);
        launch_lz_link(s, ws, &chain, n, mm, 2, 3, -1, cvec, mm - kEigBlock, false, 0, false);
        if (three_pass) launch_lz_link(s, ws, &chain, n, mm, 3, 3, -1, cvec, 0, false, 0, false);
        launch_lz_link(s, ws, &chain, n, mm, 3, 0, mm, cvec, 0, false, 0, false);
        return check_last(h, "block step launch");
      }
      return orthonormalize(h, n, mm, true, mm - kEigBlock, mm, true, cvec);
    };
    int ahead = 0;
    while (!done) {
      if (ahead > 0)
        --ahead;
      else
        SC_TRY(enqueue_step(m));
      m += kEigBlock;
      const bool check = check_due(m);
      const bool host_rr = check && m <= kHostRRSingle && !sw::eig_device_rr();
      if (host_rr) {
        SC_HIP(h, hipMemcpy2DAsync(h->h_rr, (size_t)m * sizeof(double), h->T.p,
                                   (size_t)kLdq * sizeof(double), (size_t)m * sizeof(double), m,
                                   hipMemcpyDeviceToHost, s));
        SC_HIP(h, hipMemcpyAsync(h->h_rr + kHostRRSingle * kHostRRSingle, h->G.p,
                                 kEigBlock * kEigBlock * sizeof(double), hipMemcpyDeviceToHost,
                                 s));
      } else if (check) {
        launch_jacobi(s, ptr<double>(h->T), kLdq, m, 0, nullptr, nullptr, ptr<double>(h->G),
                      theta_d, ptr<double>(h->Y), kLdq, resid_d, ptr<double>(h->Yt),
                      ptr<int>(h->flags));
        SC_TRY(check_last(h, "jacobi launch"));
        SC_HIP(h, hipMemcpyAsync(h->h_theta, theta_d, m * sizeof(double),
                                 hipMemcpyDeviceToHost, s));
        SC_HIP(h, hipMemcpyAsync(h->h_theta + kLdq, resid_d, m * sizeof(double),
                                 hipMemcpyDeviceToHost, s));
      }
      if (!fused) {
        const int rcb = finish_block(h, n, m, m, cvec, &seed);
        if (rcb == SC_ERR_NOT_CONVERGED) {
          SC_TRY(dense_fallback(3));
          break;
        }
        SC_TRY(rcb);
      } else if (check) {
        SC_HIP(h, hipMemcpyAsync(h->h_flags, h->flags.p, 16 * sizeof(int), hipMemcpyDeviceToHost, s));
        if (!h->sync_ev) SC_HIP(h, hipEventCreateWithFlags(&h->sync_ev, hipEventDisableTiming));
        SC_HIP(h, hipEventRecord(h->sync_ev, s));
        if (host_rr && cycles == 0 && m >= 6 * kEigBlock && m + kEigBlock <= cap) {
          int mm = m;
          do {
            SC_TRY(enqueue_step(mm));
            mm += kEigBlock;
            ++ahead;
          } while (!check_due(mm));
        }
        SC_HIP(h, hipEventSynchronize(h->sync_ev));
        if (h->h_flags[12] != 0) return fail(h, SC_ERR_NON_FINITE, kNonFiniteMessage);
        if (h->h_flags[13] != 0) {
          passes = 0;
          if (!three_pass && h->h_flags[15] == 2000) {
            if (sw::eig_trace())
              fprintf(stderr, "[sc] fused chain flagged at m=%d: three-pass chain\n",
                      h->h_flags[14]);
            three_pass = true;
            goto restart_lanczos;
          }
          if (sw::eig_trace()) fprintf(stderr, "[sc] fused chain flagged: host chain\n");
          fused = false;
          goto restart_lanczos;
        }
      }
      if (op.free_op && !h->free_checked && (!fused || check)) {
        bool restart = false;
        SC_TRY(free_check(&restart));
        if (restart) {
          if (sw::eig_trace())
            fprintf(stderr, "[sc] matrix-free diffuse: %d rows evaluated in full, restart\n",
                    h->h_free[0]);
          passes = 0;
          goto restart_lanczos;
        }
      }
      if (host_rr) {
        double* hy = h->h_rr + kHostRRSingle * kHostRRSingle + 64;
        const double* hG = h->h_rr + kHostRRSingle * kHostRRSingle;
        bool rr_ok;
        timespec ts0;
        if (sw::eig_trace()) clock_gettime(CLOCK_MONOTONIC, &ts0);
        if (m <= kHostRR) {
          rr_ok = host_rayleigh_ritz(h->h_rr, m, hG, m, h->h_theta, h->h_theta + kLdq, hy, m);
        } else {
          auto leading = [&](const double* theta) {
            std::vector<double> zero(m, 0.0);
            const EigDecision d0 = analyze(rq, theta, zero.data(), m, n, false);
            const int want = d0.enough ? std::max(d0.kw, d0.kvec) : cap / 4;
            return round_up(want + kEigBlock, kEigBlock) + kEigBlock;
          };
          rr_ok = host_rayleigh_ritz_leading(h->h_rr, m, hG, m, h->h_theta, h->h_theta + kLdq,
                                             hy, m, leading);
        }
        if (sw::eig_trace()) {
          timespec ts1;
          clock_gettime(CLOCK_MONOTONIC, &ts1);
          fprintf(stderr, "[sc]   host Rayleigh-Ritz m=%d: %.0f us\n", m,
                  (ts1.tv_sec - ts0.tv_sec) * 1e6 + (ts1.tv_nsec - ts0.tv_nsec) * 1e-3);
        }
        if (!rr_ok) {
          SC_TRY(dense_fallback(2));
          break;
        }
        for (int i = 0; i < m; ++i)
          if (!std::isfinite(h->h_theta[i])) return fail(h, SC_ERR_NON_FINITE, kNonFiniteMessage);
        SC_HIP(h, hipMemcpy2DAsync(h->Y.p, (size_t)kLdq * sizeof(double), hy,
                                   (size_t)m * sizeof(double), (size_t)m * sizeof(double), m,
                                   hipMemcpyHostToDevice, s));
        SC_HIP(h, hipMemcpyAsync(theta_d, h->h_theta, m * sizeof(double),
                                 hipMemcpyHostToDevice, s));
      }
      if (check) {
        dc = analyze(rq, h->h_theta, h->h_theta + kLdq, m, n, false);
        if (sw::eig_trace()) {
          int worst = 0;
          double wr = 0.0;
          for (int i = 0; i < std::min(m, dc.kw > 0 ? dc.kw : m); ++i) {
            const double r = h->h_theta[kLdq + i] / std::max(std::fabs(h->h_theta[i]), 1e-300);
            if (r > wr) { wr = r; worst = i; }
          }
          fprintf(stderr, "[sc] lanczos pass %d m=%d cycle %d: enough=%d conv=%d kw=%d kvec=%d "
                  "fail kind %d at %d (theta %.6g resid %.2e); far end theta=%.6g resid=%.2e\n",
                  passes, m, cycles, dc.enough, dc.converged, dc.kw, dc.kvec, dc.fail_kind,
                  dc.fail_index, dc.fail_index >= 0 ? h->h_theta[dc.fail_index] : 0.0,
                  dc.fail_index >= 0 ? h->h_theta[kLdq + dc.fail_index] : 0.0, h->h_theta[m - 1],
                  h->h_theta[kLdq + m - 1]);
          (void)wr; (void)worst;
        }
        if (dc.unsupported) {
          if (dense) return fail(h, SC_ERR_UNSUPPORTED, "eigen request cannot be satisfied");
          SC_TRY(run_dense());
          goto restart_lanczos;
        }
        if (dc.enough && dc.converged) {
          if (!dense && m < n && block_multiplicity_suspect(rq, dc, h->h_theta, m)) {
            if (sw::eig_trace())
              fprintf(stderr, "[sc] %d equal Ritz values ahead of the decisive gap: dense path\n",
                      kEigBlock);
            SC_TRY(dense_fallback(7));
            break;
          }
          done = true;
          break;
        }
      }
      if (m + kEigBlock > cap) {
        if (++cycles > rq.max_cycles) {
          SC_TRY(dense_fallback(1));
          break;
        }
        int want = dc.enough ? std::max(dc.kw, dc.kvec) : cap / 4;
        int keep = round_up(want + kEigBlock, kEigBlock);
        keep = std::max(kEigBlock, std::min(keep, cap - 2 * kEigBlock));
        launch_basis_times_Y(s, ptr<double>(h->Q), kLdq, m, ptr<double>(h->Y), kLdq, keep,
                             ptr<double>(h->Q2), kLdq, n, 0);
        launch_copy_block(s, ptr<double>(h->Q) + m, kLdq, ptr<double>(h->Q2) + keep, kLdq, n,
                          kEigBlock);
        std::swap(h->Q, h->Q2);
        launch_set_diag_T(s, ptr<double>(h->T), kLdq, kLdq, theta_d, keep);
        SC_TRY(check_last(h, "restart launch"));
        m = keep;
      }
    }
    if (ahead > 0) passes -= ahead;
    if (vectors_from_dense) {
      dc.max_resid = 0.0;
      if (diag) diag->eig_path = SC_EIG_PATH_DENSE_FULL;
    } else {
      const int cols = std::min(std::max(dc.kw, dc.kvec), kMaxVectors);
      launch_basis_times_Y(s, ptr<double>(h->Q), kLdq, m, ptr<double>(h->Y), kLdq, cols,
                           ptr<double>(h->E), round_up(n, 16), n, 1);
      back_transform_cols(h, n, cols);
      SC_TRY(check_last(h, "ritz vector launch"));
      h->n_vec = cols;
      if (diag) diag->eig_path = dense ? SC_EIG_PATH_DENSE_TRIDIAG : SC_EIG_PATH_BLOCK_LANCZOS;
      if (!dense) {
        h->krylov_m = m;
        h->krylov_n = n;
        h->krylov_cycles = cycles;
        h->krylov_ahead = ahead;
        h->krylov_free = op.free_op;
      }
    }
  }
  if (dense) {
    const double vec_resid = dc.max_resid;
    dc = dense_dc;
    dc.converged = true;
    dc.max_resid = vec_resid;
    if (out_w) {
      out_w->resize(n);
      for (int i = 0; i < n; ++i) (*out_w)[i] = rq.descend ? h->spectrum[i] : -h->spectrum[i];
    }
  } else if (out_w) {
    out_w->resize(dc.kw);
    for (int i = 0; i < dc.kw; ++i) (*out_w)[i] = rq.descend ? h->h_theta[i] : -h->h_theta[i];
  }
  if (diag) {
    diag->eig_matvec_passes = passes;
    diag->eig_block = kEigBlock;
    diag->eig_basis = m;
    diag->eig_cycles = cycles;
    diag->eig_max_residual = dc.max_resid;
    diag->eig_host_chain = (n > kDenseMax && !fused) ? 1 : 0;
    diag->eig_fallback = fallback_reason;
    if (op_in.free_op) {
      diag->diffuse_path = op.free_op ? SC_DIFFUSE_PATH_FREE : SC_DIFFUSE_PATH_FREE_THEN_EXPLICIT;
      diag->free_candidates = h->free_checked ? h->h_free[65] : 0;
      diag->free_overflow_rows = h->free_checked ? h->h_free[0] : 0;
      diag->free_tiles_run = h->free_checked ? h->h_free[67] : 0;
    }
  }
  *out_dc = dc;
  return SC_OK;
}

extern "C" int sc_stage_krylov_state(sc_handle h, int32_t* info, double* q, double* t, double* g,
                                     double* c, double* p) {
  if (!h) return SC_ERR_INVALID;
  if (!info) return fail(h, SC_ERR_INVALID, "krylov state: info is NULL");
  if (h->krylov_m <= 0)
    return fail(h, SC_ERR_INVALID,
                "krylov state: the last solve on this handle was not block Lanczos (dense "
                "Jacobi, tridiagonal or general path), or none has run");
  SC_HIP(h, hipSetDevice(h->device));
  const int m = h->krylov_m, n = h->krylov_n;
  memset(info, 0, 8 * sizeof(int32_t));
  info[0] = m;
  info[1] = n;
  info[2] = h->krylov_free ? 1 : 0;
  info[3] = h->krylov_ahead;
  info[4] = h->krylov_cycles;
  hipStream_t s = h->stream;
  const size_t row = (size_t)m * sizeof(double), pitch = (size_t)kLdq * sizeof(double);
  if (q) SC_HIP(h, hipMemcpy2DAsync(q, row, h->Q.p, pitch, row, n, hipMemcpyDeviceToHost, s));
  if (t) SC_HIP(h, hipMemcpy2DAsync(t, row, h->T.p, pitch, row, m, hipMemcpyDeviceToHost, s));
  if (g)
    SC_HIP(h, hipMemcpyAsync(g, h->G.p, kEigBlock * kEigBlock * sizeof(double),
                             hipMemcpyDeviceToHost, s));
  if (c) SC_HIP(h, hipMemcpyAsync(c, h->cvec.p, (size_t)n * sizeof(double), hipMemcpyDeviceToHost, s));
  if (p) SC_HIP(h, hipMemcpyAsync(p, h->pvec.p, (size_t)n * sizeof(double), hipMemcpyDeviceToHost, s));
  SC_HIP(h, hipStreamSynchronize(s));
  return SC_OK;
}

static double now_us() {
  timespec ts;
  clock_gettime(CLOCK_MONOTONIC, &ts);
  return ts.tv_sec * 1e6 + ts.tv_nsec * 1e-3;
}

bool sym_group_eligible(int n, const EigRequest& rq, bool any_size) {
  const int sym_min_n = sw::matvec_sym_min_n();
  return n > kDenseMax && (any_size || n < sym_min_n) && !wants_full_spectrum(rq) &&
         !sw::eig_host_chain() && !sw::eig_device_rr();
}

static int ensure_group_staging(sc_handle lead) {
  const size_t out_doubles = (size_t)kGroupMax * (kEigBasisCap * kEigBasisCap + 64 + 8);
  const size_t y_doubles = (size_t)kGroupMax * kEigBasisCap * kEigBasisCap;
  SC_TRY(grow(lead, lead->gpack, out_doubles * sizeof(double)));
  SC_TRY(grow(lead, lead->gypack, y_doubles * sizeof(double)));
  if (!lead->h_gpack) {
    SC_HIP(lead, hipHostMalloc(reinterpret_cast<void**>(&lead->h_gpack),
                               out_doubles * sizeof(double)));
    SC_HIP(lead, hipHostMalloc(reinterpret_cast<void**>(&lead->h_gypack),
                               y_doubles * sizeof(double)));
    SC_HIP(lead, hipEventCreateWithFlags(&lead->gcheck_ev, hipEventDisableTiming));
  }
  if (!lead->gpool) {
    const unsigned hw = std::thread::hardware_concurrency();
    lead->gpool = new HostPool(hw >= 64 ? kGroupMax - 1 : (hw >= 8 ? 6 : (hw >= 4 ? 2 : 0)));
  }
  return SC_OK;
}

int sym_topk_group(sc_handle lead, GroupEigMember* mem, int count, bool want_vectors) {
  if (count < 1 || count > kGroupMax) return fail(lead, SC_ERR_INVALID, "group size");
  hipStream_t s = lead->stream;
  SC_TRY(ensure_group_staging(lead));
  LzGroupMember lz[kGroupMax];
  int limit[kGroupMax];
  for (int z = 0; z < count; ++z) {
    sc_handle h = mem[z].h;
    SC_TRY(ensure_eig(h, mem[z].n));
    lz[z].ws = eig_workspace(h);
    lz[z].chain = LzChain();
    lz[z].chain.three_pass = true;
    lz[z].n = mem[z].n;
    lz[z].vs_scale = ptr<double>(h->cvec);
    lz[z].active = true;
    const int cap = std::min(kEigBasisCap, ((mem[z].n - kEigBlock) / kEigBlock) * kEigBlock);
    limit[z] = cap;
    mem[z].status = 0;
    mem[z].passes = 0;
    mem[z].basis = 0;
// ... 775 lines not shown
```

### spectralcluster_amd/csrc/free_api.hip

```cpp
#include <limits>

#include "handle.h"

namespace {
constexpr int kOvfWords = 80;
constexpr int kOvfRowsMax = 64;
}

extern "C" int sc_set_diffuse_mode(sc_handle h, int mode) {
  if (!h || mode < -1 || mode > 2) return SC_ERR_INVALID;
  h->diffuse_mode = mode;
  return SC_OK;
}

extern "C" int sc_set_free_prune(sc_handle h, int on) {
  if (!h || on < -1 || on > 1) return SC_ERR_INVALID;
  h->free_prune = on;
  return SC_OK;
}
static bool free_prune_on(sc_handle h) {
  return h->free_prune >= 0 ? h->free_prune != 0 : !sw::free_no_prune();
}

bool free_diffuse_wanted(sc_handle h, const sc_config* cfg, int n, const EigRequest& rq,
                         bool in_group) {
  const int mode = cfg->diffuse_mode == 1 || cfg->diffuse_mode == 2
                       ? cfg->diffuse_mode
                       : (h->diffuse_mode >= 0 ? h->diffuse_mode : sw::diffuse_mode());
  if (mode == 1) return false;
  if (n <= kDenseMax || n > 65536 || wants_full_spectrum(rq)) return false;
  if (mode == 2) return true;
  return n >= (in_group ? sw::diffuse_free_min_n_group() : sw::diffuse_free_min_n());
}

int ensure_free(sc_handle h, int n) {
  const size_t nv = (size_t)round_up(n, 16) * sizeof(double);
  SC_TRY(grow(h, h->fq, free_q_bytes(n)));
  SC_TRY(grow(h, h->ft32, free_t32_bytes(n)));
  SC_TRY(grow(h, h->fy1, nv));
  SC_TRY(grow(h, h->fR, nv));
  SC_TRY(grow(h, h->fscal, 4 * sizeof(double)));
  SC_TRY(grow(h, h->fwords, ((size_t)2 * n + kOvfWords) * sizeof(int)));
  SC_TRY(grow(h, h->fcand, (size_t)n * free_candidate_cap() * sizeof(int)));
  SC_TRY(grow(h, h->fY, (size_t)n * kEigBlock * sizeof(double)));
  SC_TRY(grow(h, h->fq2part, free_q2part_bytes(n)));
  SC_TRY(grow(h, h->fmx64, free_mx64_bytes(n)));
  SC_TRY(grow(h, h->ftau64, free_tau64_bytes(n)));
  SC_TRY(grow(h, h->fplan, free_plan_bytes(n)));
  if (!h->h_free)
    SC_HIP(h, hipHostMalloc(reinterpret_cast<void**>(&h->h_free), kOvfWords * sizeof(int)));
  return SC_OK;
}

static FreeSegs free_segs(sc_handle h) {
  return FreeSegs{ptr<double>(h->fq2part), ptr<double>(h->fmx64), ptr<float>(h->ftau64)};
}

int free_product(sc_handle h, hipStream_t s, int n) {
  SC_TRY(grow(h, h->fsplit, free_i8_split_bytes_plan()));
  launch_free_tile_flags(s, ptr<double>(h->fmx64), ptr<float>(h->ftau64), n, ptr<int>(h->fplan),
                         free_prune_on(h), ptr<int>(h->fwords));
  launch_gemm_i8_sym(s, ptr<signed char>(h->fq), n, h->tilemap_cur, ptr<float>(h->ft32),
                     ptr<unsigned>(h->fwords), ptr<int>(h->fsplit), ptr<int>(h->fplan));
  return SC_OK;
}

int free_stats_begin(sc_handle h, hipStream_t s, const double* A, int ld, int n, bool have_amax) {
  SC_TRY(ensure_free(h, n));
  SC_HIP(h, hipMemsetAsync(ptr<double>(h->fscal) + (have_amax ? 1 : 0), 0,
                           (have_amax ? 3 : 4) * sizeof(double), s));
  SC_HIP(h, hipMemsetAsync(h->fwords.p, 0, ((size_t)2 * n + kOvfWords) * sizeof(int), s));
  if (!have_amax) launch_free_absmax(s, A, n, ld, ptr<double>(h->fscal));
  launch_free_quantize(s, A, n, ld, ptr<signed char>(h->fq), ptr<double>(h->fscal),
                       ptr<double>(h->fy1), ptr<double>(h->fR), ptr<double>(h->fq2part));
  launch_free_seg_reduce(s, ptr<double>(h->fR), n, free_segs(h));
  return SC_OK;
}
int free_stats_end(sc_handle h, hipStream_t s, const double* A, int ld, int n, bool timed,
                   const int* plan) {
  unsigned* M = ptr<unsigned>(h->fwords);
  int* count = ptr<int>(h->fwords) + n;
  int* ovf = ptr<int>(h->fwords) + 2 * (size_t)n;
  launch_t32_candidates(s, ptr<float>(h->ft32), n, M, ptr<double>(h->fR), ptr<double>(h->fscal),
                        count, ptr<int>(h->fcand), plan);
  if (timed) ev_rec(h, &h->free_ev[3]);
  launch_free_row_stats(s, A, n, ld, ptr<double>(h->fy1), count, ptr<int>(h->fcand),
                        ptr<double>(h->rowmax), ptr<double>(h->rowsum), ovf);
  if (timed) ev_rec(h, &h->free_ev[4]);
  SC_TRY(check_last(h, "matrix-free diffuse launch"));
  SC_HIP(h, hipMemcpyAsync(h->h_free, ovf, kOvfWords * sizeof(int), hipMemcpyDeviceToHost, s));
  h->free_checked = false;
  return SC_OK;
}

int free_group_prepare(sc_handle* hs, const double* const* A, const double* const* cuts,
                       const double* ps, int count, const int* lds, const int* ns, hipStream_t s,
                       double floor_value, FreeItem* items, TsDigits* digits) {
// ... 29 lines not shown

int free_group_end(sc_handle* hs, const FreeItem* items, int count, hipStream_t s) {
  launch_free_scan_stats_group(s, items, count);
  SC_TRY(check_last(hs[0], "matrix-free diffuse launch"));
  for (int z = 0; z < count; ++z) {
    sc_handle h = hs[z];
    SC_HIP(h, hipMemcpyAsync(h->h_free, items[z].words + 2 * (size_t)items[z].n,
                             kOvfWords * sizeof(int), hipMemcpyDeviceToHost, s));
    h->free_checked = false;
  }
  return SC_OK;
}

int free_fused_prepare(sc_handle h, hipStream_t s, int n, const double* cut, double p,
                       double floor_value) {
  SC_TRY(ensure_free(h, n));
  const size_t rows64 = (size_t)round_up(n, 64), nblk = rows64 / 64;
  SC_TRY(grow(h, h->fypart, rows64 * nblk * sizeof(double)));
  SC_TRY(grow(h, h->frpart, rows64 * nblk * sizeof(int)));
  FreeItem item{};
  item.n = n;
  item.words = ptr<int>(h->fwords);
  item.scal = ptr<double>(h->fscal);
  item.cut = cut;
  item.p = p;
  launch_free_begin_group(s, &item, 1, floor_value);
  return SC_OK;
}

int free_diffuse_stats(sc_handle h, const double* A, int ld, int n, bool have_amax,
                       bool digits_ready) {
  hipStream_t s = h->stream;
  SC_TRY(ensure_tilemap(h, n));
  ev_rec(h, &h->free_ev[0]);
  if (digits_ready)
    launch_free_partials_reduce(s, ptr<double>(h->fypart), ptr<int>(h->frpart), n,
                                ptr<double>(h->fy1), ptr<double>(h->fR), ptr<double>(h->fscal),
                                free_segs(h));
  else
    SC_TRY(free_stats_begin(h, s, A, ld, n, have_amax));
  ev_rec(h, &h->free_ev[1]);
  SC_TRY(free_product(h, s, n));
  ev_rec(h, &h->free_ev[2]);
  return free_stats_end(h, s, A, ld, n, true, ptr<int>(h->fplan));
}

void free_front_info(sc_handle h, int* candidates, int* overflow_rows, int* forms_s) {
  *candidates = h->h_free[65];
  *overflow_rows = h->h_free[0];
  *forms_s = h->h_free[0] > kOvfRowsMax ? 1 : 0;
}

static void plain_matvec(hipStream_t s, const double* A, int ld, int n, bool sym_mv,
                         const double* Vs, double* W, double* slabs) {
  if (sym_mv)
    launch_block_matvec_sym(s, A, ld, n, nullptr, nullptr, Vs, kEigBlock, Vs, W, slabs);
  else
    launch_block_matvec(s, A, ld, n, nullptr, nullptr, Vs, kEigBlock, Vs, W);
}

int free_fix_overflow(sc_handle h, const double* A, int ld, int n, bool* changed,
                      bool* too_many) {
  *changed = *too_many = false;
  hipStream_t s = h->stream;
  SC_HIP(h, hipStreamSynchronize(s));
  h->free_checked = true;
  const int rows = h->h_free[0];
  if (rows <= 0) return SC_OK;
  if (rows > kOvfRowsMax) {
    *too_many = true;
    return SC_OK;
  }
  SC_TRY(ensure_eig(h, n));
  const bool sym_mv = n >= sw::matvec_sym_min_n();
  const int* ids = ptr<int>(h->fwords) + 2 * (size_t)n + 1;
  for (int r0 = 0; r0 < rows; r0 += kEigBlock) {
    const int nr = std::min(kEigBlock, rows - r0);
    launch_free_gather_rows(s, A, n, ld, ids + r0, nr, ptr<double>(h->Vs));
    plain_matvec(s, A, ld, n, sym_mv, ptr<double>(h->Vs), ptr<double>(h->W),
                 ptr<double>(h->mvsym));
    launch_free_colmax(s, ptr<double>(h->W), n, ids + r0, nr, ptr<double>(h->rowmax));
  }
  SC_TRY(check_last(h, "matrix-free diffuse: exact rows"));
  *changed = true;
  return SC_OK;
}

void free_apply_operator(hipStream_t s, const double* A, int ld, int n, bool sym_mv,
                         const double* cvec, const double* pvec, const double* V, int ldv,
                         const double* Vs, double* fY, double* W, double* slabs) {
  plain_matvec(s, A, ld, n, sym_mv, Vs, fY, slabs);
  if (sym_mv)
    launch_block_matvec_sym(s, A, ld, n, cvec, pvec, V, ldv, fY, W, slabs);
  else
    launch_block_matvec(s, A, ld, n, cvec, pvec, V, ldv, fY, W);
}
void free_apply_operator(sc_handle h, const double* A, int ld, int n, bool sym_mv,
                         const double* V, int ldv) {
  free_apply_operator(h->stream, A, ld, n, sym_mv, ptr<double>(h->cvec), ptr<double>(h->pvec), V,
                      ldv, ptr<double>(h->Vs), ptr<double>(h->fY), ptr<double>(h->W),
                      ptr<double>(h->mvsym));
}

extern "C" int sc_stage_diffuse_rowstats(sc_handle h, const double* a, int n, int mode,
                                         double* rowmax, double* rowsum, int32_t* info) {
  if (!h) return SC_ERR_INVALID;
  if (!a || n <= 0 || !rowmax || !rowsum || (mode != 1 && mode != 2))
    return fail(h, SC_ERR_INVALID, "bad diffuse row statistics request");
  if (mode == 2 && n > 65536) return fail(h, SC_ERR_UNSUPPORTED, "matrix-free diffuse: n <= 65536");
  SC_HIP(h, hipSetDevice(h->device));
  SC_TRY(ensure_matrices(h, n, 0));
  SC_TRY(ensure_eig(h, n));
  SC_TRY(ensure_tilemap(h, n));
  const int ld = matrix_ld(n);
  h->n = n;
  h->ldn = ld;
  h->have_affinity = h->have_cropval = false;
  h->have_x = false;
  h->n_vec = 0;
  h->nev = 0;
  hipStream_t s = h->stream;
  double* A = ptr<double>(h->B2);
  SC_TRY(h2d_matrix(h, a, n, n, A, ld));
  int inf[6] = {0, 0, 0, 0, 0, 0};
  auto explicit_stats = [&]() -> int {
    GemmRowStats rs{1, ptr<double>(h->statp), ptr<double>(h->statp) + (size_t)n * gemm_tile_dim(n),
                    ptr<double>(h->rowmax), ptr<double>(h->rowsum)};
    launch_gemm_nt(s, A, ld, A, ld, ptr<double>(h->B1), ld, n, n, n, kEpiNone, true,
                   ptr<double>(h->splitk), h->tilemap_cur, &rs);
    return check_last(h, "diffuse launch");
  };
  if (mode == 1) {
    SC_TRY(explicit_stats());
  } else {
    SC_TRY(free_diffuse_stats(h, A, ld, n));
    bool changed = false, too_many = false;
    SC_TRY(free_fix_overflow(h, A, ld, n, &changed, &too_many));
    inf[0] = h->h_free[65];
    inf[1] = h->h_free[0];
    inf[2] = h->h_free[66];
    inf[4] = h->h_free[67];
    inf[5] = gemm_tile_dim(n) * (gemm_tile_dim(n) + 1) / 2;
    if (too_many) {
      inf[3] = 1;
      SC_TRY(explicit_stats());
    }
  }
  SC_HIP(h, hipMemcpyAsync(rowmax, h->rowmax.p, (size_t)n * sizeof(double), hipMemcpyDeviceToHost, s));
  SC_HIP(h, hipMemcpyAsync(rowsum, h->rowsum.p, (size_t)n * sizeof(double), hipMemcpyDeviceToHost, s));
  SC_HIP(h, hipStreamSynchronize(s));
  if (info) memcpy(info, inf, sizeof(inf));
  return SC_OK;
}

extern "C" int sc_stage_block_operator(sc_handle h, int count, const int32_t* ns,
                                       const double* const* matrices, const double* const* cvecs,
                                       const double* const* pvecs,
                                       const double* const* vs_scales, const double* const* vs,
                                       double* const* ws, int route) {
  if (!h) return SC_ERR_INVALID;
  const int known = SC_BLOCK_ROUTE_SYM | SC_BLOCK_ROUTE_TWO_PRODUCT | SC_BLOCK_ROUTE_GROUPED;
  if (count < 1 || count > kGroupMax || !ns || !matrices || !vs || !ws || (route & ~known))
    return fail(h, SC_ERR_INVALID, "bad block operator request");
  const bool sym = (route & SC_BLOCK_ROUTE_SYM) != 0;
  const bool two = (route & SC_BLOCK_ROUTE_TWO_PRODUCT) != 0;
  const bool grouped = (route & SC_BLOCK_ROUTE_GROUPED) != 0;
  for (int z = 0; z < count; ++z) {
    if (ns[z] < 0 || (ns[z] == 0 && !grouped))
      return fail(h, SC_ERR_INVALID, "block operator: n must be positive (0: idle, grouped only)");
    if (ns[z] > 0 && (!matrices[z] || !vs[z] || !ws[z]))
      return fail(h, SC_ERR_INVALID, "block operator: NULL matrix, block or result");
  }
  SC_HIP(h, hipSetDevice(h->device));
  hipStream_t s = h->stream;
  struct Owned {
    std::vector<void*> p;
    ~Owned() {
      for (void* q : p) (void)hipFree(q);
    }
  } owned;
  const double qnan = std::numeric_limits<double>::quiet_NaN();
  std::vector<double> stage;
  auto device = [&](size_t doubles, const double* src, double** out) -> int {
    void* d = nullptr;
    SC_HIP(h, hipMalloc(&d, std::max<size_t>(doubles, 1) * sizeof(double)));
    owned.p.push_back(d);
    if (!src) {
      stage.assign(doubles, qnan);
      src = stage.data();
    }
    SC_HIP(h, hipMemcpyAsync(d, src, doubles * sizeof(double), hipMemcpyHostToDevice, s));
    SC_HIP(h, hipStreamSynchronize(s));
    *out = reinterpret_cast<double*>(d);
    return SC_OK;
  };
  MatvecItem mv[kGroupMax];
  double* fY[kGroupMax] = {nullptr};
  memset(mv, 0, sizeof(mv));
  std::vector<double> scaled;
  for (int z = 0; z < count; ++z) {
    const int n = ns[z];
    if (n == 0) continue;
    const int ld = matrix_ld(n);
    double *S, *V, *Vs, *W, *c = nullptr, *p = nullptr, *slabs = nullptr;
    SC_TRY(device((size_t)n * ld, nullptr, &S));
    SC_TRY(h2d_matrix(h, matrices[z], n, n, S, ld));
    const double* cz = cvecs ? cvecs[z] : nullptr;
    const double* pz = pvecs ? pvecs[z] : nullptr;
    const double* sz = (vs_scales && vs_scales[z]) ? vs_scales[z] : cz;
    if (cz) SC_TRY(device(n, cz, &c));
    if (pz) SC_TRY(device(n, pz, &p));
    SC_TRY(device((size_t)n * kEigBlock, vs[z], &V));
    scaled.assign(vs[z], vs[z] + (size_t)n * kEigBlock);
    if (sz)
      for (int r = 0; r < n; ++r)
        for (int j = 0; j < kEigBlock; ++j) scaled[(size_t)r * kEigBlock + j] *= sz[r];
    SC_TRY(device((size_t)n * kEigBlock, scaled.data(), &Vs));
    SC_TRY(device((size_t)n * kEigBlock, nullptr, &W));
    if (two) SC_TRY(device((size_t)n * kEigBlock, nullptr, &fY[z]));
    if (sym) SC_TRY(device(matvec_sym_workspace_doubles(n), nullptr, &slabs));
    mv[z].S = S;
    mv[z].ld = ld;
    mv[z].n = n;
    mv[z].cvec = c;
    mv[z].pvec = p;
    mv[z].V = V;
    mv[z].ldv = kEigBlock;
    mv[z].Vs = Vs;
    mv[z].W = W;
    mv[z].slabs = slabs;
  }
  if (grouped) {
    if (two) {
      MatvecItem inner[kGroupMax];
      memcpy(inner, mv, sizeof(mv));
      for (int z = 0; z < count; ++z) {
        if (mv[z].n == 0) continue;
        inner[z].cvec = inner[z].pvec = nullptr;
        inner[z].V = mv[z].Vs;
        inner[z].W = fY[z];
        mv[z].Vs = fY[z];
      }
      launch_block_matvec_group(s, inner, count, sym);
    }
    launch_block_matvec_group(s, mv, count, sym);
  } else {
    for (int z = 0; z < count; ++z) {
      const MatvecItem& a = mv[z];
      if (two)
        free_apply_operator(s, a.S, a.ld, a.n, sym, a.cvec, a.pvec, a.V, a.ldv, a.Vs, fY[z], a.W,
                            a.slabs);
      else if (sym)
        launch_block_matvec_sym(s, a.S, a.ld, a.n, a.cvec, a.pvec, a.V, a.ldv, a.Vs, a.W, a.slabs);
      else
        launch_block_matvec(s, a.S, a.ld, a.n, a.cvec, a.pvec, a.V, a.ldv, a.Vs, a.W);
    }
  }
  SC_TRY(check_last(h, "block operator launch"));
  for (int z = 0; z < count; ++z)
    if (mv[z].n > 0)
      SC_HIP(h, hipMemcpyAsync(ws[z], mv[z].W, (size_t)mv[z].n * kEigBlock * sizeof(double),
                               hipMemcpyDeviceToHost, s));
  SC_HIP(h, hipStreamSynchronize(s));
  return SC_OK;
}
```

### spectralcluster_amd/csrc/handle.h

```cpp
#ifndef SPECTRALCLUSTER_AMD_HANDLE_H_
#define SPECTRALCLUSTER_AMD_HANDLE_H_

#include <algorithm>
#include <array>
#include <cmath>
#include <cstdio>
#include <cstdlib>
#include <cstring>
#include <string>
#include <vector>

#include "sc_internal.h"

using namespace sc;

struct DevBuf {
  void* p = nullptr;
  size_t bytes = 0;
};

constexpr int kKgenBufs = 12;
constexpr int kGroupBanks = 2;
constexpr int kGroupLanes = 3;

// ... 62 lines not shown
  std::vector<int> sweep_slot;
  std::vector<sc_diag> sweep_diags;
  std::vector<double> sweep_p;
  sc_config sweep_cfg;
  int sweep_n = 0;
  hipEvent_t sync_ev = nullptr;
  DevBuf gkrnd;
  bool gkrnd_ready = false;
  DevBuf gpack, gypack, ginfo, glabels;
  double* h_gpack = nullptr;
  double* h_gypack = nullptr;
  int* h_ginfo = nullptr;
  long long* h_glabels = nullptr;
  size_t h_glabels_count = 0;
  hipEvent_t gcheck_ev = nullptr;
  std::vector<sc_handle_s*> gshort;
  DevBuf gjtab;
  JacobiItem* h_gjtab = nullptr;
  DevBuf gsftab;
  ShortFrontItem* h_gsftab = nullptr;
  hipEvent_t gsftab_ev = nullptr;
  DevBuf gswtab;
  ShortWaveItem* h_gswtab = nullptr;
  int gsw_launches = 0;
  std::vector<int32_t> last_routes;
  int32_t* groutes = nullptr;
  std::vector<sc_handle_s*> glanes;
  class HostPool* gpool = nullptr;
  hipStream_t gbank_stream[kGroupBanks] = {nullptr};
  hipStream_t gchain_stream = nullptr;
  hipEvent_t gbank_ev[kGroupBanks] = {nullptr};
  int gconv_hist[16] = {0};
  int gconv_seen = 0;
  hipEvent_t ev[48];
  int nev = 0;
  StageEvents stage_events;
  int profile_level = 1;
  int mv_ev[16][2];
  int n_mv_ev = 0;
  int aff_ev[2] = {-1, -1};
  int blurw_radius = -1;
  double blurw_host[2 * SC_MAX_BLUR_RADIUS + 1];
  int krnd_k = -1, krnd_trials = -1;
  int kfirst_n = -1, kfirst = 0;
  int diffuse_mode = -1;
  DevBuf fq, ft32, fy1, fR, fscal, fwords, fcand, fY, fsplit, fypart, frpart;
  int free_prune = -1;
  DevBuf fq2part, fmx64, ftau64, fplan;
  int* h_free = nullptr;
  bool free_checked = false;
  int free_ev[5] = {-1, -1, -1, -1, -1};
  int krylov_m = 0, krylov_n = 0, krylov_cycles = 0, krylov_ahead = 0;
  bool krylov_free = false;
  BlurLaunch last_blur;
};

inline void ev_rec(sc_handle h, int* slot) {
  if (h->nev < 48) {
    hipEventRecord(h->ev[h->nev], h->stream);
    *slot = h->nev++;
  } else {
    *slot = -1;
  }
}
inline float ev_ms(sc_handle h, int a, int b) {
  if (a < 0 || b < 0) return 0.f;
  float ms = 0.f;
  hipEventElapsedTime(&ms, h->ev[a], h->ev[b]);
  return ms;
}

constexpr int kTilemapTableMax = 64;
constexpr int kMaxCols = 128;
inline int matrix_ld(int n) {
  int ld = round_up(n, 16);
  if (ld % 512 == 0) ld += 16;
  return ld;
}


#define SC_HIP(h, call)                                                         \
  do {                                                                          \
    hipError_t e_ = (call);                                                     \
    if (e_ != hipSuccess) {                                                     \
      (h)->err = std::string(#call) + ": " + hipGetErrorString(e_);             \
      return e_ == hipErrorOutOfMemory ? SC_ERR_OOM : SC_ERR_HIP;               \
    }                                                                           \
  } while (0)

#define SC_TRY(expr)                \
  do {                              \
    int rc_ = (expr);               \
    if (rc_ != SC_OK) return rc_;   \
  } while (0)

inline int fail(sc_handle h, int code, const std::string& msg) {
  if (h) h->err = msg;
  return code;
}

inline int grow(sc_handle h, DevBuf& b, size_t bytes) {
  if (b.bytes >= bytes) return SC_OK;
  if (b.p) {
    SC_HIP(h, hipStreamSynchronize(h->stream));
    SC_HIP(h, hipFree(b.p));
    b.p = nullptr;
// ... 100 lines not shown
  int crop_source = 0, cut_kernel = 0;
};
EigRequest make_eig_request(const sc_config* cfg);
int upload_blur_weights(sc_handle h, const sc_config* cfg);
int run_refine_op(sc_handle h, int op, const sc_config* cfg, const double* in, double* out, int n,
                  int ld);
int eig_ncluster_impl(sc_handle h, const sc_config* cfg, sc_diag* diag, FrontResult* front_only,
                      const FrontResult* resume = nullptr, bool defer_timing = false,
                      FrontResult* stop_before_solver = nullptr);
void kmeans_seed_constants(int k, double* u_first, int* trials, std::vector<double>* rnd);
KmeansWorkspace kmeans_workspace(sc_handle h);

struct GroupEigMember {
  sc_handle h = nullptr;
  const double* S = nullptr;
  int ld = 0, n = 0;
  EigRequest rq;
  int status = 0;
  EigDecision dc;
  std::vector<double> w;
  int basis = 0, passes = 0;
  bool skip_fused = false;
  bool free_op = false;
};
int sym_topk_group(sc_handle lead, GroupEigMember* mem, int count, bool want_vectors = true);
int dense_topk_group(sc_handle lead, GroupEigMember* mem, int count);
bool sym_group_eligible(int n, const EigRequest& rq, bool any_size = false);

int sym_topk(sc_handle h, const FrontResult& op, int n, const EigRequest& rq, sc_diag* diag,
             EigDecision* out_dc, std::vector<double>* out_w);
int gen_topk(sc_handle h, const double* M, int ld, int n, int laplacian_type,
             const EigRequest& rq, sc_diag* diag, EigDecision* out_dc,
             std::vector<double>* out_w, double* scratch);

bool free_diffuse_wanted(sc_handle h, const sc_config* cfg, int n, const EigRequest& rq,
                         bool in_group = false);
int free_group_prepare(sc_handle* hs, const double* const* A, const double* const* cuts,
                       const double* ps, int count, const int* lds, const int* ns, hipStream_t s,
                       double floor_value, struct FreeItem* items, struct TsDigits* digits);
int free_group_digits(sc_handle* hs, const struct FreeItem* items, int count, hipStream_t s);
int free_group_end(sc_handle* hs, const struct FreeItem* items, int count, hipStream_t s);
int free_fused_prepare(sc_handle h, hipStream_t s, int n, const double* cut, double p,
                       double floor_value);
void free_front_info(sc_handle h, int* candidates, int* overflow_rows, int* forms_s);
int free_diffuse_stats(sc_handle h, const double* A, int ld, int n, bool have_amax = false,
                       bool digits_ready = false);
int ensure_free(sc_handle h, int n);
int free_product(sc_handle h, hipStream_t s, int n);
int free_stats_begin(sc_handle h, hipStream_t s, const double* A, int ld, int n, bool have_amax);
int free_stats_end(sc_handle h, hipStream_t s, const double* A, int ld, int n, bool timed,
                   const int* plan = nullptr);
int free_fix_overflow(sc_handle h, const double* A, int ld, int n, bool* changed, bool* too_many);
void free_apply_operator(sc_handle h, const double* A, int ld, int n, bool sym_mv,
                         const double* V, int ldv);
void free_apply_operator(hipStream_t s, const double* A, int ld, int n, bool sym_mv,
                         const double* cvec, const double* pvec, const double* V, int ldv,
                         const double* Vs, double* fY, double* W, double* slabs);
bool wants_full_spectrum(const EigRequest& rq);

int device_is_symmetric(sc_handle h, const double* m, int n, int ld, bool* out);
int adjust_affinity(sc_handle h, const sc_config* cfg, const double* a, bool sym_a, double* out,
                    int n, int ld);
bool constraint_active(sc_handle h, const sc_config* cfg, bool before);
struct CpGroupMember {
  int n = 0, ld = 0;
  double* A = nullptr;
  double *P = nullptr, *T = nullptr, *Pn = nullptr, *Tn = nullptr;
  double *deg = nullptr, *rowmax = nullptr;
  const double* band = nullptr;
  const int2* tilemap = nullptr;
  bool pairs = false, psym = false;
  int pk = 0;
  const int32_t *prows = nullptr, *pcols = nullptr;
  const double* pvals = nullptr;
};
int constraint_propagation_group(sc_handle lead, hipStream_t s, const CpGroupMember* mem,
                                 int count, double alpha);
int validate_constraint_pairs(sc_handle h, const int32_t* rows, const int32_t* cols,
                              const double* vals, int count, int n, bool* symmetric);
std::vector<double> pack_constraint_pairs(const int32_t* rows, const int32_t* cols,
                                          const double* vals, int count);
int predict_batch_constrained_impl(sc_handle h, const sc_array* xs, const sc_constraint_desc* cons,
                                   const int* ns, int d, int count, const sc_config* cfg,
                                   int64_t* const* labels, sc_diag* diags, int group);

int affinity_stats_impl(sc_handle h, double* out);
int affinity_gmm_bic_impl(sc_handle h, int diagonal_offset, double* bic1, double* bic2);
struct SingleMember {
  const double* a;
  int n, ld;
};
int validate_single_check(sc_handle h, const sc_single_check* opt);
int check_single_offset(sc_handle h, const sc_single_check* opt, int n, int index);
int single_check_wave(sc_handle lead, hipStream_t s, const SingleMember* ms, int count,
                      const sc_single_check* opt, double* values, int32_t* single);
int single_check_group(sc_handle lead, hipStream_t s, const SingleMember* ms, int count,
                       const sc_single_check* opt, double* values, int32_t* single);
int single_check_resident(sc_handle h, const sc_single_check* opt, double* values,
                          int32_t* single);

#endif
```

### spectralcluster_amd/csrc/sc_internal.h

```cpp
#pragma once

#include <hip/hip_runtime.h>

#include "switches.h"
#include <stdint.h>

#include <mutex>
#include <string>
#include <vector>

#include "../../include/spectralcluster_amd.h"

namespace sc {

constexpr int kWave = 64;
constexpr int kEigBlock = 8;
constexpr int kEigBasisCap = 128;
constexpr int kLdq = kEigBasisCap + kEigBlock;
constexpr int kDenseMax = 128;
constexpr int kHostRR = 64;
constexpr int kHostRRSingle = kEigBasisCap;
constexpr int kGenMax = 64;
constexpr int kMaxVectors = 64;
constexpr int kProjBlocks = 128;

inline int round_up(int v, int m) { return (v + m - 1) / m * m; }

#define SC_OPT_IN_LDS(kernel, bytes)                                                      \
  do {                                                                                    \
    static std::once_flag sc_once_[16];                                                   \
    int sc_dev_ = 0;                                                                      \
    (void)hipGetDevice(&sc_dev_);                                                         \
    std::call_once(sc_once_[sc_dev_ & 15], [] {                                           \
      (void)hipFuncSetAttribute(reinterpret_cast<const void*>(kernel),                    \
                                hipFuncAttributeMaxDynamicSharedMemorySize, (int)(bytes)); \
    });                                                                                   \
  } while (0)

enum { kEpiNone = 0, kEpiAffinity = 1, kEpiAdd = 2 };

struct GemmRowStats {
  int mode;
  double* partial_max;
  double* partial_sum;
  double* rowmax;
  double* rowsum;
};
void launch_gemm_nt(hipStream_t s, const double* A, int lda, const double* B,
                    int ldb, double* C, int ldc, int M, int N, int K,
                    int epilogue, bool symmetric, double* splitk_ws,
                    const int2* tilemap, const GemmRowStats* rs = nullptr,
                    const double* addend = nullptr);
struct GemmGroupItem {
  const double* A = nullptr;
  int lda = 0;
  double* C = nullptr;
  int ldc = 0;
  int n = 0, K = 0;
  const int2* tilemap = nullptr;
  double* partial_max = nullptr;
  double* partial_sum = nullptr;
  double* rowmax = nullptr;
  double* rowsum = nullptr;
};
void launch_gemm_nt_group(hipStream_t s, const GemmGroupItem* items, int count, int epilogue,
                          int stats_mode, bool reduce_stats = true);
__device__ __forceinline__ void gemm_stats_fold_row(const double* __restrict__ pmax,
                                                    const double* __restrict__ psum, int ntiles,
                                                    int mode, double* mx_out, double* sm_out) {
// ... 76 lines not shown
void launch_row_threshold(hipStream_t s, const double* in, double* out, int n,
                          int ld, double p, double mult, int binarize,
                          int preserve_diag);
void launch_symmetrize(hipStream_t s, const double* in, double* out, int n, int ld,
                       int type);

void launch_affinity_integration(hipStream_t s, const double* a, const double* q, double* out,
                                 int n, int ld, int type);
void launch_affinity_integration_band(hipStream_t s, const double* a, const double* band,
                                      double* out, int n, int ld, int type);
void launch_cp_band_product(hipStream_t s, const double* tt, const double* band, double* x,
                            int n, int ld);
void launch_cp_prepare(hipStream_t s, const double* a, const double* deg, double alpha,
                       double* p, double* t0, int n, int ld);
void launch_cp_adjust(hipStream_t s, const double* tqt, const double* a, double scale,
                      double* out, int n, int ld);
void launch_transpose(hipStream_t s, const double* in, double* out, int n, int ld);
void launch_symmetry_flag(hipStream_t s, const double* in, int n, int ld, int* flag);
void launch_row_normalize(hipStream_t s, const double* in, double* out, int n,
                          int ld);
void launch_row_stats(hipStream_t s, const double* in, int n, int ld,
                      double* rowmax, double* rowsum);
void launch_scaling_vectors(hipStream_t s, const double* rowmax,
                            const double* rowsum, int n, int laplacian_type,
                            int row_normalized, double* c, double* p, double* t,
                            int* flags = nullptr, int* symflag = nullptr);
void launch_laplacian(hipStream_t s, const double* in, double* out, int n, int ld,
                      int laplacian_type, double* deg_ws);
void launch_check_finite(hipStream_t s, const double* a, const double* b, int n, int* flag);

struct EigWorkspace {
  double* Q = nullptr;
  double* Q2 = nullptr;
  double* Vs = nullptr;
  double* W = nullptr;
  double* partial = nullptr;
  double* T = nullptr;
  double* Y = nullptr;
  double* theta = nullptr;
  double* resid = nullptr;
  double* G = nullptr;
  double* Rinv = nullptr;
  double* Hbuf = nullptr;
  double* hsq = nullptr;
  double* Yt = nullptr;
  double* colnorm = nullptr;
  int* flags = nullptr;
};

void launch_random_block(hipStream_t s, double* W, int n, uint64_t seed);
void launch_block_matvec(hipStream_t s, const double* S, int ld, int n,
                         const double* cvec, const double* pvec, const double* V,
                         int ldv, const double* Vs, double* W);
size_t matvec_sym_workspace_doubles(int n);
void launch_block_matvec_sym(hipStream_t s, const double* S, int ld, int n, const double* cvec,
                             const double* pvec, const double* V, int ldv, const double* Vs,
                             double* W, double* ws);
void launch_proj_partial(hipStream_t s, const double* Q, int ldq, int m,
                         const double* W, int n, double* partial);
int proj_blocks(int n);
void launch_reduce_H(hipStream_t s, const double* partial, int nparts, int m, double* Hbuf,
                     double* T, int ldt, int col0, int accumulate, double* hsq);
void launch_update_block(hipStream_t s, const double* Q, int ldq, int m,
                         const double* Hbuf, double* W, int n);
void launch_reduce_chol(hipStream_t s, const double* partial, int nparts, double* Rinv,
                        double* Gsave, const double* hsq, int* flags,
                        int* defect_flag = nullptr, int flag_mode = 1);
void launch_apply_rinv(hipStream_t s, double* W, int n, const double* Rinv,
                       double* Qdst, int ldq, int col0, const double* cvec,
                       double* Vs);
void launch_refill_deficient(hipStream_t s, double* W, int n, const int* flags,
                             uint64_t seed);
struct LzChain {
  int parity = 0;
  int nparts = 0;
  bool three_pass = false;
};
size_t lz_partial_doubles(int n);
void launch_lz_link(hipStream_t s, const EigWorkspace& ws, LzChain* chain, int n, int m,
                    int pre, int next, int store_col, const double* vs_scale, int col0,
                    bool init_random, uint64_t seed, bool zero_T);
constexpr int kGroupMax = 16;
#ifndef SC_SHORT_WIDTH
#define SC_SHORT_WIDTH 64
#endif
constexpr int kShortWidth = SC_SHORT_WIDTH;
static_assert(kShortWidth >= 1 && kShortWidth <= 256, "one workgroup per CU");
template <typename T>
struct GroupOf {
  T s[kGroupMax];
};
struct MatvecItem {
  const double* S;
  int ld, n;
  const double* cvec;
  const double* pvec;
  const double* V;
  int ldv;
  const double* Vs;
  double* W;
  double* slabs;
};
struct RitzItem {
  const double* Q;
  int ldq, m;
  const double* Y;
  int ldy, cols;
  double* E;
  int lde, n;
  const double* tvec;
};
struct JacobiItem {
  const double* src;
  int ld, m, mode;
  const double* cvec;
  const double* pvec;
  double* theta;
  double* Y;
  int ldy;
  double* Yt;
  int* flags;
  double* pack;
  double* E;
  int lde;
  const double* tvec;
};
struct FrontItem {
  const double* X;
  double* Xn;
  int ldx, n, d, ldn;
  double* A0;
// ... 461 lines not shown
```

### spectralcluster_amd/csrc/switches.h

```cpp
#ifndef SPECTRALCLUSTER_AMD_SWITCHES_H_
#define SPECTRALCLUSTER_AMD_SWITCHES_H_

#include <cstdlib>
#include <cstring>

namespace sc {
namespace sw {

inline int eig_trace() {
  static const int v = getenv("SC_EIG_TRACE") ? std::max(1, atoi(getenv("SC_EIG_TRACE"))) : 0;
  return v;
}
inline bool kmeans_trace() {
  static const bool v = getenv("SC_KMEANS_TRACE") != nullptr;
  return v;
}
inline bool group_trace() {
  static const bool v = getenv("SC_GROUP_TRACE") != nullptr;
  return v;
}
inline bool eig_host_chain() {
  static const bool v = getenv("SC_EIG_HOST_CHAIN") != nullptr;
  return v;
}
inline bool eig_device_rr() {
  static const bool v = getenv("SC_EIG_DEVICE_RR") != nullptr;
  return v;
}
inline bool eig_force_dense() {
  static const bool v = getenv("SC_EIG_FORCE_DENSE") != nullptr;
  return v;
}
inline int matvec_sym_min_n() {
  static const int v = getenv("SC_MATVEC_SYM_MIN_N") ? atoi(getenv("SC_MATVEC_SYM_MIN_N")) : 4096;
  return v;
}
inline bool kmeans_single() {
  static const bool v = getenv("SC_KMEANS_SINGLE") != nullptr;
  return v;
}
inline int diffuse_mode() {
  static const int v = [] {
    const char* e = getenv("SC_DIFFUSE");
    if (!e) return 0;
    if (!strcmp(e, "explicit")) return 1;
    if (!strcmp(e, "free")) return 2;
    return 0;
  }();
  return v;
}
inline int diffuse_free_min_n() {
  static const int v =
      getenv("SC_DIFFUSE_FREE_MIN_N") ? atoi(getenv("SC_DIFFUSE_FREE_MIN_N")) : 2048;
  return v;
}
inline int diffuse_free_min_n_group() {
  static const int v =
      getenv("SC_DIFFUSE_FREE_MIN_N") ? atoi(getenv("SC_DIFFUSE_FREE_MIN_N")) : 1536;
  return v;
}
inline int gen_dense_max_n() {
  static const int v = getenv("SC_GEN_DENSE_MAX_N") ? atoi(getenv("SC_GEN_DENSE_MAX_N")) : 512;
  return v;
}
inline bool free_no_prune() {
  static const bool v = getenv("SC_FREE_NO_PRUNE") != nullptr;
  return v;
}
inline bool sweep_one_by_one() {
  static const bool v = getenv("SC_SWEEP_ONE_BY_ONE") != nullptr;
  return v;
}
inline bool short_front_memberwise() {
  static const bool v = getenv("SC_SHORT_FRONT_MEMBERWISE") != nullptr;
  return v;
}

}
}

#endif
```

Baseline: 388.8 calls/s.

## Add optional 16-vector block Lanczos path for large symmetric eigen solves

Adds a wide block mode in which the block Krylov eigensolver carries 16 vectors per block instead of 8, filling all columns of the MFMA tile. The symmetric upper-triangle block matvec, its reduction kernel, the Lanczos link partials and a new 16x16 Cholesky are templated on the block width, and workspaces are sized to match. The intent is to get more useful work from each pass over the n x n affinity matrix, cutting the number of full-matrix sweeps per eigen solve. The cost is larger workspaces, more register and shared-memory pressure, and a two-pass shared reduction in the mirror step. The mode is selected by a new API setter or the SC_EIG_WIDE environment switch, which defaults to 0.

Result: slower. 383.4 calls/s (-1.4%).

```diff
diff --git a/include/spectralcluster_amd.h b/include/spectralcluster_amd.h
--- a/include/spectralcluster_amd.h
+++ b/include/spectralcluster_amd.h
@@ -180,6 +180,7 @@
 int sc_set_profiling(sc_handle h, int level);
 int sc_set_diffuse_mode(sc_handle h, int mode);
 int sc_set_free_prune(sc_handle h, int on);
+int sc_set_eig_wide(sc_handle h, int mode);
 
 int sc_config_default(sc_config* cfg);
 int sc_gaussian_weights(double sigma, int32_t* radius, double* weights);
@@ -355,8 +356,14 @@
                             const double* const* matrices, const double* const* cvecs,
                             const double* const* pvecs, const double* const* vs_scales,
                             const double* const* vs, double* const* ws, int route);
+int sc_stage_block_operator_w(sc_handle h, int count, const int32_t* ns,
+                              const double* const* matrices, const double* const* cvecs,
+                              const double* const* pvecs, const double* const* vs_scales,
+                              const double* const* vs, double* const* ws, int route, int width);
 int sc_stage_krylov_state(sc_handle h, int32_t* info, double* q, double* t, double* g, double* c,
                           double* p);
+int sc_stage_krylov_state_w(sc_handle h, int32_t* info, double* q, double* t, double* g,
+                            double* c, double* p);
 enum { SC_FRONT_ROUTE_SINGLE = 0, SC_FRONT_ROUTE_GROUPED = 1, SC_FRONT_ROUTE_SWEEP = 2,
        SC_FRONT_ROUTE_SHORT_SWEEP = 3, SC_FRONT_ROUTE_SHORT_WAVE = 4 };
 enum {
diff --git a/spectralcluster_amd/_lib.py b/spectralcluster_amd/_lib.py
--- a/spectralcluster_amd/_lib.py
+++ b/spectralcluster_amd/_lib.py
@@ -214,6 +214,7 @@
     "sc_set_profiling": (ctypes.c_int, [_handle_t, ctypes.c_int]),
     "sc_set_diffuse_mode": (ctypes.c_int, [_handle_t, ctypes.c_int]),
     "sc_set_free_prune": (ctypes.c_int, [_handle_t, ctypes.c_int]),
+    "sc_set_eig_wide": (ctypes.c_int, [_handle_t, ctypes.c_int]),
     "sc_stage_diffuse_rowstats": (ctypes.c_int, [_handle_t, _c_double_p, ctypes.c_int,
                                                  ctypes.c_int, _c_double_p, _c_double_p,
                                                  ctypes.POINTER(ctypes.c_int32)]),
@@ -225,9 +226,21 @@
                                                ctypes.POINTER(_c_double_p),
                                                ctypes.POINTER(_c_double_p),
                                                ctypes.POINTER(_c_double_p), ctypes.c_int]),
+    "sc_stage_block_operator_w": (ctypes.c_int, [_handle_t, ctypes.c_int,
+                                                 ctypes.POINTER(ctypes.c_int32),
+                                                 ctypes.POINTER(_c_double_p),
+                                                 ctypes.POINTER(_c_double_p),
+                                                 ctypes.POINTER(_c_double_p),
+                                                 ctypes.POINTER(_c_double_p),
+                                                 ctypes.POINTER(_c_double_p),
+                                                 ctypes.POINTER(_c_double_p), ctypes.c_int,
+                                                 ctypes.c_int]),
     "sc_stage_krylov_state": (ctypes.c_int, [_handle_t, ctypes.POINTER(ctypes.c_int32),
                                              _c_double_p, _c_double_p, _c_double_p, _c_double_p,
                                              _c_double_p]),
+    "sc_stage_krylov_state_w": (ctypes.c_int, [_handle_t, ctypes.POINTER(ctypes.c_int32),
+                                               _c_double_p, _c_double_p, _c_double_p, _c_double_p,
+                                               _c_double_p]),
     "sc_stage_front": (ctypes.c_int, [_handle_t, ctypes.c_int, ctypes.POINTER(ScConfig),
                                       ctypes.c_int, ctypes.POINTER(ctypes.c_int32), ctypes.c_int,
                                       ctypes.POINTER(_c_double_p), _c_double_p, _c_double_p,
diff --git a/spectralcluster_amd/csrc/api.hip b/spectralcluster_amd/csrc/api.hip
--- a/spectralcluster_amd/csrc/api.hip
+++ b/spectralcluster_amd/csrc/api.hip
@@ -79,10 +79,12 @@
   if (h->Q.bytes < nq) h->krylov_m = 0;
   SC_TRY(grow(h, h->Q, nq));
   SC_TRY(grow(h, h->Q2, nq));
-  SC_TRY(grow(h, h->Vs, (size_t)n * kEigBlock * sizeof(double)));
-  SC_TRY(grow(h, h->W, (size_t)n * kEigBlock * sizeof(double)));
+  const int wide = eig_wide_mode(h);
+  const int bw = (wide == 2 || (wide == 1 && n >= kEigWideMinN)) ? kEigBlockWide : kEigBlock;
+  SC_TRY(grow(h, h->Vs, (size_t)n * bw * sizeof(double)));
+  SC_TRY(grow(h, h->W, (size_t)n * bw * sizeof(double)));
   SC_TRY(grow(h, h->partial, std::max((size_t)kProjBlocks * kLdq * kEigBlock,
-                                       lz_partial_doubles(n)) * sizeof(double)));
+                                       lz_partial_doubles(n, bw)) * sizeof(double)));
   SC_TRY(grow(h, h->T, (size_t)kLdq * kLdq * sizeof(double)));
   SC_TRY(grow(h, h->Y, (size_t)kLdq * kLdq * sizeof(double)));
   SC_TRY(grow(h, h->Yt, (size_t)kLdq * kLdq * sizeof(double)));
@@ -97,7 +99,7 @@
     SC_TRY(grow(h, h->flags, 16 * sizeof(int)));
     SC_HIP(h, hipMemsetAsync(h->flags.p, 0, 16 * sizeof(int), h->stream));
   }
-  SC_TRY(grow(h, h->mvsym, matvec_sym_workspace_doubles(n) * sizeof(double)));
+  SC_TRY(grow(h, h->mvsym, matvec_sym_workspace_doubles(n, bw) * sizeof(double)));
   SC_TRY(ensure_vectors(h, n, kMaxCols));
   return SC_OK;
 }
@@ -173,7 +175,7 @@
       hipHostMalloc(reinterpret_cast<void**>(&h->h_flags), 16 * sizeof(int)) !=
           hipSuccess ||
       hipHostMalloc(reinterpret_cast<void**>(&h->h_rr),
-                    (2 * kHostRRSingle * kHostRRSingle + 64) * sizeof(double)) != hipSuccess) {
+                    (2 * kHostRRSingle * kHostRRSingle + kHostRRGram) * sizeof(double)) != hipSuccess) {
     delete h;
     return SC_ERR_HIP;
   }
diff --git a/spectralcluster_amd/csrc/eig.hip b/spectralcluster_amd/csrc/eig.hip
--- a/spectralcluster_amd/csrc/eig.hip
+++ b/spectralcluster_amd/csrc/eig.hip
@@ -115,9 +115,11 @@
 __device__ __forceinline__ int sym_item_id(int I, int J, int nt) {
   return I * nt - I * (I - 1) / 2 + (J - I);
 }
+template <int BW>
 __device__ __forceinline__ void block_matvec_sym_body(
     const double* __restrict__ S, int ld, int n, const double* __restrict__ Vs,
     double* __restrict__ pdirect, double* __restrict__ pmirror, int nt) {
+  static_assert(BW == 8 || BW == 16, "block width: half or all of the MFMA tile's columns");
   __shared__ __attribute__((aligned(16))) double smem[4 * 32 * kSymPitch];
   int I = 0, rem = blockIdx.x, rowlen = nt;
   while (rem >= rowlen) {
@@ -136,7 +138,7 @@
 #pragma unroll
   for (int t = 0; t < 8; ++t) {
     const int row = r0 + 4 * t + lg;
-    bm[t] = (row < n && li < B) ? Vs[(size_t)row * B + li] : 0.0;
+    bm[t] = (row < n && li < BW) ? Vs[(size_t)row * BW + li] : 0.0;
   }
   v4f64 accd[2] = {{0.0, 0.0, 0.0, 0.0}, {0.0, 0.0, 0.0, 0.0}};
   v4f64 accm[4][2];
@@ -178,7 +180,7 @@
 #pragma unroll
     for (int t = 0; t < 8; ++t) {
       const int k = kb + 8 * (t >> 1) + (t & 1);
-      b[t] = (k < n && li < B) ? Vs[(size_t)k * B + li] : 0.0;
+      b[t] = (k < n && li < BW) ? Vs[(size_t)k * BW + li] : 0.0;
     }
 #pragma unroll
     for (int rt = 0; rt < 2; ++rt)
@@ -208,49 +210,56 @@
     }
   }
   const size_t item = blockIdx.x;
-  if (li < B) {
+  if (li < BW) {
 #pragma unroll
     for (int rt = 0; rt < 2; ++rt)
 #pragma unroll
       for (int r = 0; r < 4; ++r)
-        pdirect[(item * kSymTile + 32 * wave + 16 * rt + lg + 4 * r) * B + li] = accd[rt][r];
+        pdirect[(item * kSymTile + 32 * wave + 16 * rt + lg + 4 * r) * BW + li] = accd[rt][r];
   }
   if (diag) return;
-  __syncthreads();
   double* red = smem;
-  if (li < B) {
-#pragma unroll
-    for (int cs = 0; cs < 4; ++cs)
-#pragma unroll
-      for (int ct = 0; ct < 2; ++ct)
-#pragma unroll
-        for (int r = 0; r < 4; ++r)
-          red[(wave * kSymTile + 32 * cs + 16 * ct + lg + 4 * r) * B + li] = accm[cs][ct][r];
-  }
-  __syncthreads();
-  for (int e = threadIdx.x; e < kSymTile * B; e += 256)
-    pmirror[item * (kSymTile * B) + e] =
-        ((red[e] + red[kSymTile * B + e]) + red[2 * kSymTile * B + e]) + red[3 * kSymTile * B + e];
-}
+#pragma unroll
+  for (int hv = 0; hv < BW / 8; ++hv) {
+    __syncthreads();
+    if (li >= 8 * hv && li < 8 * hv + 8) {
+#pragma unroll
+      for (int cs = 0; cs < 4; ++cs)
+#pragma unroll
+        for (int ct = 0; ct < 2; ++ct)
+#pragma unroll
+          for (int r = 0; r < 4; ++r)
+            red[(wave * kSymTile + 32 * cs + 16 * ct + lg + 4 * r) * 8 + (li - 8 * hv)] =
+                accm[cs][ct][r];
+    }
+    __syncthreads();
+    for (int e = threadIdx.x; e < kSymTile * 8; e += 256)
+      pmirror[item * (kSymTile * BW) + (e >> 3) * BW + 8 * hv + (e & 7)] =
+          ((red[e] + red[kSymTile * 8 + e]) + red[2 * kSymTile * 8 + e]) + red[3 * kSymTile * 8 + e];
+  }
+}
+template <int BW>
 __global__ __launch_bounds__(256) void k_block_matvec_sym(
     const double* __restrict__ S, int ld, int n, const double* __restrict__ Vs,
     double* __restrict__ pdirect, double* __restrict__ pmirror, int nt) {
-  block_matvec_sym_body(S, ld, n, Vs, pdirect, pmirror, nt);
+  block_matvec_sym_body<BW>(S, ld, n, Vs, pdirect, pmirror, nt);
 }
 __global__ __launch_bounds__(256) void k_block_matvec_sym_g(const GroupOf<MatvecItem> g) {
   const MatvecItem& a = g.s[blockIdx.y];
   const int nt = (a.n + kSymTile - 1) / kSymTile;
   if ((int)blockIdx.x >= nt * (nt + 1) / 2) return;
-  block_matvec_sym_body(a.S, a.ld, a.n, a.Vs, a.slabs, a.slabs + (size_t)(nt * (nt + 1) / 2) * kSymTile * B, nt);
-}
-
+  block_matvec_sym_body<B>(a.S, a.ld, a.n, a.Vs, a.slabs, a.slabs + (size_t)(nt * (nt + 1) / 2) * kSymTile * B, nt);
+}
+
+template <int BW>
 __device__ __forceinline__ void matvec_sym_reduce_body(
     const double* __restrict__ pdirect, const double* __restrict__ pmirror, int nt, int n,
     const double* __restrict__ cvec, const double* __restrict__ pvec,
     const double* __restrict__ V, int ldv, double* __restrict__ W) {
-  const int R = blockIdx.x / 4;
-  const int e = (blockIdx.x & 3) * 256 + threadIdx.x;
-  const int rl = e / B, v = e % B;
+  constexpr int kWg = kSymTile * BW / 256;
+  const int R = blockIdx.x / kWg;
+  const int e = (blockIdx.x % kWg) * 256 + threadIdx.x;
+  const int rl = e / BW, v = e % BW;
   const int row = R * kSymTile + rl;
   double acc = 0.0;
   const int total = nt;
@@ -261,28 +270,29 @@
       const int sidx = s0 + u;
       x[u] = 0.0;
       if (sidx < nt - R) {
-        x[u] = pdirect[(size_t)sym_item_id(R, R + sidx, nt) * (kSymTile * B) + e];
+        x[u] = pdirect[(size_t)sym_item_id(R, R + sidx, nt) * (kSymTile * BW) + e];
       } else if (sidx < total) {
-        x[u] = pmirror[(size_t)sym_item_id(sidx - (nt - R), R, nt) * (kSymTile * B) + e];
+        x[u] = pmirror[(size_t)sym_item_id(sidx - (nt - R), R, nt) * (kSymTile * BW) + e];
       }
     }
 #pragma unroll
     for (int u = 0; u < 8; ++u) acc += x[u];
   }
-  if (row < n) W[(size_t)row * B + v] =
+  if (row < n) W[(size_t)row * BW + v] =
       __builtin_fma(cvec ? cvec[row] : 1.0, acc, pvec ? pvec[row] * V[(size_t)row * ldv + v] : 0.0);
 }
+template <int BW>
 __global__ __launch_bounds__(256) void k_matvec_sym_reduce(
     const double* __restrict__ pdirect, const double* __restrict__ pmirror, int nt, int n,
     const double* __restrict__ cvec, const double* __restrict__ pvec,
     const double* __restrict__ V, int ldv, double* __restrict__ W) {
-  matvec_sym_reduce_body(pdirect, pmirror, nt, n, cvec, pvec, V, ldv, W);
+  matvec_sym_reduce_body<BW>(pdirect, pmirror, nt, n, cvec, pvec, V, ldv, W);
 }
 __global__ __launch_bounds__(256) void k_matvec_sym_reduce_g(const GroupOf<MatvecItem> g) {
   const MatvecItem& a = g.s[blockIdx.y];
   const int nt = (a.n + kSymTile - 1) / kSymTile;
   if ((int)blockIdx.x >= nt * 4) return;
-  matvec_sym_reduce_body(a.slabs, a.slabs + (size_t)(nt * (nt + 1) / 2) * kSymTile * B, nt, a.n,
+  matvec_sym_reduce_body<B>(a.slabs, a.slabs + (size_t)(nt * (nt + 1) / 2) * kSymTile * B, nt, a.n,
                          a.cvec, a.pvec, a.V, a.ldv, a.W);
 }
 
@@ -480,6 +490,78 @@
   }
 }
 
+__device__ __forceinline__ void chol16_block(const double* G, double* __restrict__ Rinv,
+                                             const double* __restrict__ hsq,
+                                             int* __restrict__ flags,
+                                             int* __restrict__ defect_flag, int flag_mode,
+                                             int* __restrict__ sticky_flag, int sticky_m,
+                                             bool sticky_on_defect) {
+  constexpr int N = 16;
+  __shared__ double Rm[N * N];
+  __shared__ double dwave[4];
+  const int tid = threadIdx.x;
+  const bool act = tid < N * N;
+  const int i = (tid >> 4) & (N - 1), j = tid & (N - 1);
+  double g = act ? G[i * N + j] : 0.0;
+  const double gii = G[i * N + i], gjj = G[j * N + j];
+  double defect = 0.0;
+  if (act && flag_mode == 2 && gii != 0.0 && gjj != 0.0) defect = fabs(g - (i == j ? 1.0 : 0.0));
+#pragma unroll
+  for (int o = 1; o < 64; o <<= 1) defect = fmax(defect, __shfl_xor(defect, o));
+  if (act && (tid & 63) == 0) dwave[tid >> 6] = defect;
+#pragma unroll
+  for (int k = 0; k < N; ++k) {
+    const double d = __shfl(g, k, N);
+    if (act && i == k) {
+      const double total = gii + (hsq ? hsq[k] : 0.0);
+      const bool drop = !(d > 1e-22 * total) || !(d > 0.0);
+      const double rk = drop ? 0.0 : sqrt(d);
+      Rm[k * N + j] = drop ? 0.0 : (j == k ? rk : (j > k ? g / rk : 0.0));
+    }
+    __syncthreads();
+    if (act && i > k && j > k) g -= Rm[k * N + i] * Rm[k * N + j];
+  }
+  if (tid < N) {
+    double col[N];
+#pragma unroll
+    for (int r = 0; r < N; ++r) col[r] = 0.0;
+    const double rjj = Rm[tid * N + tid];
+#pragma unroll
+    for (int r = N - 1; r >= 0; --r) {
+      const double rrr = Rm[r * N + r];
+      double v = 0.0;
+#pragma unroll
+      for (int k = r + 1; k < N; ++k) v -= Rm[r * N + k] * col[k];
+      if (r <= tid && rrr != 0.0 && rjj != 0.0) col[r] = r == tid ? 1.0 / rrr : v / rrr;
+    }
+#pragma unroll
+    for (int r = 0; r < N; ++r) Rinv[r * N + tid] = col[r];
+  }
+  if (tid == 0 && flags != nullptr) {
+    int mask = 0;
+    double pmax = 0.0, pmin = __builtin_huge_val();
+    for (int k = 0; k < N; ++k) {
+      const double rk = Rm[k * N + k];
+      if (rk == 0.0) {
+        mask |= 1 << k;
+      } else {
+        pmax = fmax(pmax, rk);
+        pmin = fmin(pmin, rk);
+      }
+    }
+    const double dmax = fmax(fmax(dwave[0], dwave[1]), fmax(dwave[2], dwave[3]));
+    flags[0] = mask;
+    if (defect_flag != nullptr) *defect_flag = (dmax > 0.1 || pmax > 1e3 * pmin) ? 1 : 0;
+    if (sticky_flag != nullptr && (mask != 0 || (sticky_on_defect && dmax > 0.1))) {
+      if (*sticky_flag == 0) {
+        sticky_flag[1] = sticky_m;
+        sticky_flag[2] = flag_mode * 100000 + mask;
+      }
+      *sticky_flag = 1;
+    }
+  }
+}
+
 __global__ __launch_bounds__(256) void k_apply_rinv(
     double* __restrict__ W, int n, const double* __restrict__ Rinv,
     double* __restrict__ Qdst, int ldq, int col0, const double* __restrict__ cvec,
@@ -505,7 +587,7 @@
 }
 
 constexpr int kLzThreads = 512;
-constexpr int kLzPartStride = (kLdq + B) * B;
+constexpr int lz_part_stride(int bw) { return (kLdq + bw) * bw; }
 struct LzStep {
   double* W;
   int n;
@@ -531,21 +613,24 @@
   double* partial;
 };
 
-__device__ __forceinline__ double lz_ordered_sum(const double* src, int nparts) {
+__device__ __forceinline__ double lz_ordered_sum(const double* src, int nparts, int stride) {
   double acc = 0.0;
   for (int p0 = 0; p0 < nparts; p0 += 16) {
     double v[16];
 #pragma unroll
     for (int u = 0; u < 16; ++u)
-      v[u] = (p0 + u < nparts) ? src[(size_t)(p0 + u) * kLzPartStride] : 0.0;
+      v[u] = (p0 + u < nparts) ? src[(size_t)(p0 + u) * stride] : 0.0;
 #pragma unroll
     for (int u = 0; u < 16; ++u) acc += v[u];
   }
   return acc;
 }
 
-template <int ROWS>
+template <int ROWS, int BW>
 __device__ __forceinline__ void lz_rows_body(const LzStep& a) {
+  constexpr int B = BW;
+  constexpr int kPartStride = lz_part_stride(BW);
+  constexpr int kHs = (kLdq * B + B * B + kLzThreads - 1) / kLzThreads;
   extern __shared__ __attribute__((aligned(16))) double smem[];
   constexpr int kPass = kLzThreads / B;
   const int m = a.m;
@@ -566,19 +651,22 @@
   const bool use_r = pre_gram;
   const bool use_q = m > 0 && (use_h || a.want_proj);
   const int nproj = pre_proj ? m * B : 0;
-  double hsum[3] = {0.0, 0.0, 0.0};
-#pragma unroll
-  for (int u = 0; u < 3; ++u) {
+  double hsum[kHs];
+#pragma unroll
+  for (int u = 0; u < kHs; ++u) {
     const int e = tid + u * kLzThreads;
-    if (e < nproj) hsum[u] = lz_ordered_sum(a.pre_partial + e, a.pre_nparts);
+    hsum[u] = 0.0;
+    if (e < nproj) hsum[u] = lz_ordered_sum(a.pre_partial + e, a.pre_nparts, kPartStride);
     else if (pre_gram && e < nproj + B * B)
-      hsum[u] = lz_ordered_sum(a.pre_partial + kLdq * B + (e - nproj), a.pre_nparts);
-  }
-  double told[3] = {0.0, 0.0, 0.0};
+      hsum[u] = lz_ordered_sum(a.pre_partial + kLdq * B + (e - nproj), a.pre_nparts, kPartStride);
+  }
+  double told[kHs];
+#pragma unroll
+  for (int u = 0; u < kHs; ++u) told[u] = 0.0;
   double hsq_old = 0.0;
   if (first_wg && a.pre == 2) {
 #pragma unroll
-    for (int u = 0; u < 3; ++u) {
+    for (int u = 0; u < kHs; ++u) {
       const int e = tid + u * kLzThreads;
       if (e < nproj) told[u] = a.T[(size_t)(e / B) * a.ldt + a.col0 + (e % B)];
     }
@@ -599,7 +687,7 @@
       w[q] = a.init_random ? hash_uniform(a.seed, (uint64_t)r * B + j) : a.W[(size_t)r * B + j];
   }
 #pragma unroll
-  for (int u = 0; u < 3; ++u) {
+  for (int u = 0; u < kHs; ++u) {
     const int e = tid + u * kLzThreads;
     if (e < nproj) Hl[e] = hsum[u];
     else if (pre_gram && e < nproj + B * B) Gs[e - nproj] = hsum[u];
@@ -609,7 +697,7 @@
   if (pre_proj && a.pre != 3) {
     if (first_wg && a.T != nullptr) {
 #pragma unroll
-      for (int u = 0; u < 3; ++u) {
+      for (int u = 0; u < kHs; ++u) {
         const int e = tid + u * kLzThreads;
         if (e < nproj) {
           const int i = e / B, jc = a.col0 + (e % B);
@@ -642,10 +730,16 @@
     }
     __syncthreads();
     if (first_wg && a.pre == 2 && a.Gsave != nullptr && tid < B * B) a.Gsave[tid] = Gs[tid];
-    if (tid < 64)
-      chol8_wave(Gs, Rl, a.pre == 2 ? hs : nullptr, first_wg ? a.flags : nullptr,
-                 first_wg ? a.flags + (a.pre == 3 ? 10 : 11) : nullptr, a.pre == 3 ? 2 : 1,
-                 first_wg ? a.flags + 13 : nullptr, m, a.arm_defect != 0);
+    if constexpr (BW == 8) {
+      if (tid < 64)
+        chol8_wave(Gs, Rl, a.pre == 2 ? hs : nullptr, first_wg ? a.flags : nullptr,
+                   first_wg ? a.flags + (a.pre == 3 ? 10 : 11) : nullptr, a.pre == 3 ? 2 : 1,
+                   first_wg ? a.flags + 13 : nullptr, m, a.arm_defect != 0);
+    } else {
+      chol16_block(Gs, Rl, a.pre == 2 ? hs : nullptr, first_wg ? a.flags : nullptr,
+                   first_wg ? a.flags + (a.pre == 3 ? 10 : 11) : nullptr, a.pre == 3 ? 2 : 1,
+                   first_wg ? a.flags + 13 : nullptr, m, a.arm_defect != 0);
+    }
     __syncthreads();
   }
 #pragma unroll
@@ -672,7 +766,7 @@
   __syncthreads();
   const int oproj = a.want_proj ? m * B : 0;
   const int nent = oproj + (a.want_gram ? B * B : 0);
-  double* mine = a.partial + (size_t)blockIdx.x * kLzPartStride;
+  double* mine = a.partial + (size_t)blockIdx.x * kPartStride;
   for (int base = 0; base < nent; base += kLzThreads / 2) {
     const int e = base + (tid >> 1), half = tid & 1;
     double acc = 0.0;
@@ -695,15 +789,15 @@
       mine[e < oproj ? e : kLdq * B + (e - oproj)] = acc + other;
   }
 }
-template <int ROWS>
+template <int ROWS, int BW>
 __global__ __launch_bounds__(kLzThreads) void k_lz_rows(const LzStep a) {
-  lz_rows_body<ROWS>(a);
+  lz_rows_body<ROWS, BW>(a);
 }
 template <int ROWS>
 __global__ __launch_bounds__(kLzThreads) void k_lz_rows_g(const GroupOf<LzStep> g) {
   const LzStep& a = g.s[blockIdx.y];
   if ((int)blockIdx.x * ROWS >= a.n) return;
-  lz_rows_body<ROWS>(a);
+  lz_rows_body<ROWS, B>(a);
 }
 
 __device__ __forceinline__ double fast_rcp(double x) {
@@ -1093,19 +1187,26 @@
   hipLaunchKernelGGL(k_block_matvec, dim3((n + 15) / 16), dim3(64 * kMvWaves), 0, s, S,
                      ld, n, cvec, pvec, V, ldv, Vs, W);
 }
-size_t matvec_sym_workspace_doubles(int n) {
+size_t matvec_sym_workspace_doubles(int n, int bw) {
   const size_t nt = (size_t)(n + kSymTile - 1) / kSymTile;
-  return 2 * (nt * (nt + 1) / 2) * kSymTile * B;
+  return 2 * (nt * (nt + 1) / 2) * kSymTile * bw;
 }
 void launch_block_matvec_sym(hipStream_t s, const double* S, int ld, int n, const double* cvec,
                              const double* pvec, const double* V, int ldv, const double* Vs,
-                             double* W, double* ws) {
+                             double* W, double* ws, int bw) {
   const int nt = (n + kSymTile - 1) / kSymTile;
   const int items = nt * (nt + 1) / 2;
   double* pd = ws;
-  double* pm = ws + (size_t)items * kSymTile * B;
-  hipLaunchKernelGGL(k_block_matvec_sym, dim3(items), dim3(256), 0, s, S, ld, n, Vs, pd, pm, nt);
-  hipLaunchKernelGGL(k_matvec_sym_reduce, dim3(nt * 4), dim3(256), 0, s, pd, pm, nt, n, cvec,
+  double* pm = ws + (size_t)items * kSymTile * bw;
+  if (bw == kEigBlockWide) {
+    hipLaunchKernelGGL(k_block_matvec_sym<kEigBlockWide>, dim3(items), dim3(256), 0, s, S, ld, n,
+                       Vs, pd, pm, nt);
+    hipLaunchKernelGGL(k_matvec_sym_reduce<kEigBlockWide>, dim3(nt * (kSymTile * kEigBlockWide / 256)),
+                       dim3(256), 0, s, pd, pm, nt, n, cvec, pvec, V, ldv, W);
+    return;
+  }
+  hipLaunchKernelGGL(k_block_matvec_sym<B>, dim3(items), dim3(256), 0, s, S, ld, n, Vs, pd, pm, nt);
+  hipLaunchKernelGGL(k_matvec_sym_reduce<B>, dim3(nt * 4), dim3(256), 0, s, pd, pm, nt, n, cvec,
                      pvec, V, ldv, W);
 }
 void launch_proj_partial(hipStream_t s, const double* Q, int ldq, int m,
@@ -1135,26 +1236,29 @@
   hipLaunchKernelGGL(k_apply_rinv, dim3((n + RB - 1) / RB), dim3(256), 0, s, W, n, Rinv,
                      Qdst, ldq, col0, cvec, Vs);
 }
-static int lz_rows_for(int m) {
+static int lz_rows_for(int m, int bw = B) {
+  if (bw == kEigBlockWide) return (size_t)128 * (m + 1) * sizeof(double) <= 96 * 1024 ? 128 : 64;
   if ((size_t)128 * (m + 1) * sizeof(double) <= 112 * 1024) return 128;
   if ((size_t)256 * (m + 1) * sizeof(double) <= 96 * 1024) return 256;
   if ((size_t)128 * (m + 1) * sizeof(double) <= 112 * 1024) return 128;
   return 64;
 }
-size_t lz_partial_doubles(int n) { return 2 * (size_t)((n + 63) / 64) * kLzPartStride; }
-
-template <int ROWS>
+size_t lz_partial_doubles(int n, int bw) {
+  return 2 * (size_t)((n + 63) / 64) * lz_part_stride(bw);
+}
+
+template <int ROWS, int BW = B>
 static void launch_rows(hipStream_t s, const LzStep& a, int nwg) {
-  const size_t lds = sizeof(double) * ((size_t)ROWS * (a.m + 1) + (size_t)kLdq * B + B * B +
-                                       (size_t)ROWS * B + B * B + B);
+  const size_t lds = sizeof(double) * ((size_t)ROWS * (a.m + 1) + (size_t)kLdq * BW + BW * BW +
+                                       (size_t)ROWS * BW + BW * BW + BW);
   static std::once_flag once[16];
   int dev = 0;
   hipGetDevice(&dev);
   std::call_once(once[dev & 15], [] {
-    hipFuncSetAttribute(reinterpret_cast<const void*>(k_lz_rows<ROWS>),
+    hipFuncSetAttribute(reinterpret_cast<const void*>(k_lz_rows<ROWS, BW>),
                         hipFuncAttributeMaxDynamicSharedMemorySize, 150 * 1024);
   });
-  hipLaunchKernelGGL(k_lz_rows<ROWS>, dim3(nwg), dim3(kLzThreads), lds, s, a);
+  hipLaunchKernelGGL((k_lz_rows<ROWS, BW>), dim3(nwg), dim3(kLzThreads), lds, s, a);
 }
 
 static LzStep lz_make_step(const EigWorkspace& ws, LzChain* chain, int n, int m, int pre,
@@ -1168,7 +1272,7 @@
   a.ldq = kLdq;
   a.m = m;
   a.pre = pre;
-  const size_t half = lz_partial_doubles(n) / 2;
+  const size_t half = lz_partial_doubles(n, chain->bw) / 2;
   a.pre_partial = ws.partial + (size_t)chain->parity * half;
   a.pre_nparts = chain->nparts;
   a.T = ws.T;
@@ -1188,7 +1292,7 @@
   a.want_gram = next >= 2 ? 1 : 0;
   chain->parity ^= 1;
   a.partial = ws.partial + (size_t)chain->parity * half;
-  const int rows = lz_rows_for(m);
+  const int rows = lz_rows_for(m, chain->bw);
   chain->nparts = (n + rows - 1) / rows;
   return a;
 }
@@ -1197,8 +1301,13 @@
                     bool init_random, uint64_t seed, bool zero_T) {
   const LzStep a = lz_make_step(ws, chain, n, m, pre, next, store_col, vs_scale, col0,
                                 init_random, seed, zero_T);
-  const int rows = lz_rows_for(m);
+  const int rows = lz_rows_for(m, chain->bw);
   const int nwg = chain->nparts;
+  if (chain->bw == kEigBlockWide) {
+    if (rows == 128) launch_rows<128, kEigBlockWide>(s, a, nwg);
+    else launch_rows<64, kEigBlockWide>(s, a, nwg);
+    return;
+  }
   if (rows == 256) launch_rows<256>(s, a, nwg);
   else if (rows == 128) launch_rows<128>(s, a, nwg);
   else launch_rows<64>(s, a, nwg);
diff --git a/spectralcluster_amd/csrc/eig_driver.hip b/spectralcluster_amd/csrc/eig_driver.hip
--- a/spectralcluster_amd/csrc/eig_driver.hip
+++ b/spectralcluster_amd/csrc/eig_driver.hip
@@ -151,13 +151,13 @@
 }
 
 static bool block_multiplicity_suspect(const EigRequest& rq, const EigDecision& dc,
-                                       const double* theta, int m) {
+                                       const double* theta, int m, int bw = kEigBlock) {
   const int kw = std::min(dc.kw, m);
   const int limit = rq.fixed_count > 0 ? kw - 2 : dc.n_clusters_raw - 1;
   const double rel = 10.0 * std::max(rq.value_tol, 1e-12);
   const double scale = std::max(std::fabs(theta[0]), std::fabs(theta[m - 1]));
-  for (int i = 0; i + kEigBlock - 1 <= limit && i + kEigBlock - 1 < kw; ++i) {
-    const double a = theta[i], b = theta[i + kEigBlock - 1];
+  for (int i = 0; i + bw - 1 <= limit && i + bw - 1 < kw; ++i) {
+    const double a = theta[i], b = theta[i + bw - 1];
     if (std::fabs(a - b) <= rel * std::max(std::max(std::fabs(a), std::fabs(b)), 1e-10 * scale))
       return true;
   }
@@ -165,7 +165,7 @@
 }
 
 static bool host_rayleigh_ritz(const double* T, int ld, const double* G, int m, double* theta,
-                               double* resid, double* Y, int ldy) {
+                               double* resid, double* Y, int ldy, int bw = kEigBlock) {
   const int lda = m | 1;
   std::vector<double> a((size_t)m * lda), d(m), e(m);
   for (int i = 0; i < m; ++i)
@@ -179,11 +179,11 @@
     const int c = order[rank];
     theta[rank] = d[c];
     double r2 = 0.0;
-    for (int p = 0; p < kEigBlock; ++p) {
+    for (int p = 0; p < bw; ++p) {
       double t = 0.0;
-      for (int q = 0; q < kEigBlock; ++q)
-        t += G[p * kEigBlock + q] * a[(size_t)(m - kEigBlock + q) * lda + c];
-      r2 += a[(size_t)(m - kEigBlock + p) * lda + c] * t;
+      for (int q = 0; q < bw; ++q)
+        t += G[p * bw + q] * a[(size_t)(m - bw + q) * lda + c];
+      r2 += a[(size_t)(m - bw + p) * lda + c] * t;
     }
     resid[rank] = std::sqrt(std::max(r2, 0.0));
     for (int r = 0; r < m; ++r) Y[(size_t)r * ldy + rank] = a[(size_t)r * lda + c];
@@ -194,7 +194,7 @@
 template <typename CountFn>
 static bool host_rayleigh_ritz_leading(const double* T, int ld, const double* G, int m,
                                        double* theta, double* resid, double* Y, int ldy,
-                                       CountFn count_fn) {
+                                       CountFn count_fn, int bw = kEigBlock) {
   HostTridiag tw;
   if (!host_partial_values(T, ld, m, &tw)) return false;
   for (int i = 0; i < m; ++i) theta[i] = tw.theta[i];
@@ -208,11 +208,11 @@
       continue;
     }
     double r2 = 0.0;
-    for (int p = 0; p < kEigBlock; ++p) {
+    for (int p = 0; p < bw; ++p) {
       double t = 0.0;
-      for (int q = 0; q < kEigBlock; ++q)
-        t += G[p * kEigBlock + q] * Y[(size_t)(m - kEigBlock + q) * ldy + rank];
-      r2 += Y[(size_t)(m - kEigBlock + p) * ldy + rank] * t;
+      for (int q = 0; q < bw; ++q)
+        t += G[p * bw + q] * Y[(size_t)(m - bw + q) * ldy + rank];
+      r2 += Y[(size_t)(m - bw + p) * ldy + rank] * t;
     }
     resid[rank] = std::sqrt(std::max(r2, 0.0));
   }
@@ -432,7 +432,15 @@
   bool fused = !sw::eig_host_chain() && !op.skip_fused;
   bool three_pass = false;
   const int sym_min_n = sw::matvec_sym_min_n();
-  const bool sym_mv = n >= sym_min_n;
+  bool sym_mv = n >= sym_min_n;
+  const int wide_mode = eig_wide_mode(h);
+  const int reads = rq_in.fixed_count > 0 ? rq_in.fixed_count
+                                          : (rq_in.max_clusters > 0 ? rq_in.max_clusters + 1 : 0);
+  bool wide = !sw::eig_device_rr() && n >= 4 * kEigBlockWide &&
+              (wide_mode == 2 || (wide_mode == 1 && sym_mv && n >= kEigWideMinN &&
+                                  reads > kEigBlockWide && reads <= kEigWideCap / 2));
+  const bool sym_mv_narrow = sym_mv;
+  int bw = kEigBlock;
   EigDecision dense_dc;
   bool dense = false, many_vectors = false;
   auto run_dense = [&]() -> int {
@@ -500,6 +508,8 @@
   restart_lanczos:
     m = 0;
     cycles = 0;
+    bw = (wide && fused && !three_pass && !dense) ? kEigBlockWide : kEigBlock;
+    sym_mv = bw == kEigBlockWide ? true : sym_mv_narrow;
     bool done = false;
     uint64_t seed = 0x5eed5eedull;
     LzChain chain;
@@ -515,6 +525,7 @@
       const EigWorkspace ws = eig_workspace(h);
       chain = LzChain();
       chain.three_pass = three_pass;
+      chain.bw = bw;
       launch_lz_link(s, ws, &chain, n, 0, 0, 4, -1, cvec, 0, true, seed, false);
       launch_lz_link(s, ws, &chain, n, 0, 4, 3, -1, cvec, 0, false, 0, true);
       launch_lz_link(s, ws, &chain, n, 0, 3, 0, 0, cvec, 0, false, 0, false);
@@ -535,32 +546,33 @@
       SC_TRY(dense_fallback(4));
       done = true;
     }
-    const int cap = std::min(kEigBasisCap, ((n - kEigBlock) / kEigBlock) * kEigBlock);
-    const int first_check = std::min(3 * kEigBlock, cap);
+    const int cap =
+        std::min(bw == kEigBlockWide ? kEigWideCap : kEigBasisCap, ((n - bw) / bw) * bw);
+    const int first_check = std::min(bw == kEigBlockWide ? 2 * bw : 3 * bw, cap);
     auto check_due = [&](int mm) {
-      return cycles == 0 ? (mm >= first_check && (mm <= 4 * kEigBlock ||
-                                                  mm % (2 * kEigBlock) == 0 || mm + kEigBlock > cap))
-                         : (mm + kEigBlock > cap);
+      return cycles == 0 ? (mm >= first_check && (mm <= 4 * bw ||
+                                                  mm % (2 * bw) == 0 || mm + bw > cap))
+                         : (mm + bw > cap);
     };
     auto enqueue_step = [&](int m_before) -> int {
       const bool time_mv = h->profile_level >= 2 && h->n_mv_ev < 16;
       if (time_mv) ev_rec(h, &h->mv_ev[h->n_mv_ev][0]);
       if (op.free_op)
-        free_apply_operator(h, op.matrix, ld, n, sym_mv, ptr<double>(h->Q) + m_before, kLdq);
+        free_apply_operator(h, op.matrix, ld, n, sym_mv, ptr<double>(h->Q) + m_before, kLdq, bw);
       else if (sym_mv)
         launch_block_matvec_sym(s, op.matrix, ld, n, cvec, pvec, ptr<double>(h->Q) + m_before, kLdq,
-                                ptr<double>(h->Vs), ptr<double>(h->W), ptr<double>(h->mvsym));
+                                ptr<double>(h->Vs), ptr<double>(h->W), ptr<double>(h->mvsym), bw);
       else
         launch_block_matvec(s, op.matrix, ld, n, cvec, pvec, ptr<double>(h->Q) + m_before, kLdq,
                             ptr<double>(h->Vs), ptr<double>(h->W));
       if (time_mv) ev_rec(h, &h->mv_ev[h->n_mv_ev++][1]);
       ++passes;
-      const int mm = m_before + kEigBlock;
+      const int mm = m_before + bw;
       if (fused) {
         const EigWorkspace ws = eig_workspace(h);
-        launch_lz_link(s, ws, &chain, n, mm, 0, 1, -1, cvec, mm - kEigBlock, false, 0, false);
-        launch_lz_link(s, ws, &chain, n, mm, 1, 2, -1, cvec, mm - kEigBlock, false, 0, false);
-        launch_lz_link(s, ws, &chain, n, mm, 2, 3, -1, cvec, mm - kEigBlock, false, 0, false);
+        launch_lz_link(s, ws, &chain, n, mm, 0, 1, -1, cvec, mm - bw, false, 0, false);
+        launch_lz_link(s, ws, &chain, n, mm, 1, 2, -1, cvec, mm - bw, false, 0, false);
+        launch_lz_link(s, ws, &chain, n, mm, 2, 3, -1, cvec, mm - bw, false, 0, false);
         if (three_pass) launch_lz_link(s, ws, &chain, n, mm, 3, 3, -1, cvec, 0, false, 0, false);
         launch_lz_link(s, ws, &chain, n, mm, 3, 0, mm, cvec, 0, false, 0, false);
         return check_last(h, "block step launch");
@@ -573,7 +585,7 @@
         --ahead;
       else
         SC_TRY(enqueue_step(m));
-      m += kEigBlock;
+      m += bw;
       const bool check = check_due(m);
       const bool host_rr = check && m <= kHostRRSingle && !sw::eig_device_rr();
       if (host_rr) {
@@ -581,8 +593,7 @@
                                    (size_t)kLdq * sizeof(double), (size_t)m * sizeof(double), m,
                                    hipMemcpyDeviceToHost, s));
         SC_HIP(h, hipMemcpyAsync(h->h_rr + kHostRRSingle * kHostRRSingle, h->G.p,
-                                 kEigBlock * kEigBlock * sizeof(double), hipMemcpyDeviceToHost,
-                                 s));
+                                 bw * bw * sizeof(double), hipMemcpyDeviceToHost, s));
       } else if (check) {
         launch_jacobi(s, ptr<double>(h->T), kLdq, m, 0, nullptr, nullptr, ptr<double>(h->G),
                       theta_d, ptr<double>(h->Y), kLdq, resid_d, ptr<double>(h->Yt),
@@ -604,11 +615,11 @@
         SC_HIP(h, hipMemcpyAsync(h->h_flags, h->flags.p, 16 * sizeof(int), hipMemcpyDeviceToHost, s));
         if (!h->sync_ev) SC_HIP(h, hipEventCreateWithFlags(&h->sync_ev, hipEventDisableTiming));
         SC_HIP(h, hipEventRecord(h->sync_ev, s));
-        if (host_rr && cycles == 0 && m >= 6 * kEigBlock && m + kEigBlock <= cap) {
+        if (host_rr && cycles == 0 && m >= 6 * bw && m + bw <= cap) {
           int mm = m;
           do {
             SC_TRY(enqueue_step(mm));
-            mm += kEigBlock;
+            mm += bw;
             ++ahead;
           } while (!check_due(mm));
         }
@@ -616,6 +627,13 @@
         if (h->h_flags[12] != 0) return fail(h, SC_ERR_NON_FINITE, kNonFiniteMessage);
         if (h->h_flags[13] != 0) {
           passes = 0;
+          if (bw == kEigBlockWide) {
+            if (sw::eig_trace())
+              fprintf(stderr, "[sc] wide chain flagged at m=%d (%d): 8-vector chain\n",
+                      h->h_flags[14], h->h_flags[15]);
+            wide = false;
+            goto restart_lanczos;
+          }
           if (!three_pass && h->h_flags[15] == 2000) {
             if (sw::eig_trace())
               fprintf(stderr, "[sc] fused chain flagged at m=%d: three-pass chain\n",
@@ -640,22 +658,22 @@
         }
       }
       if (host_rr) {
-        double* hy = h->h_rr + kHostRRSingle * kHostRRSingle + 64;
+        double* hy = h->h_rr + kHostRRSingle * kHostRRSingle + kHostRRGram;
         const double* hG = h->h_rr + kHostRRSingle * kHostRRSingle;
         bool rr_ok;
         timespec ts0;
         if (sw::eig_trace()) clock_gettime(CLOCK_MONOTONIC, &ts0);
         if (m <= kHostRR) {
-          rr_ok = host_rayleigh_ritz(h->h_rr, m, hG, m, h->h_theta, h->h_theta + kLdq, hy, m);
+          rr_ok = host_rayleigh_ritz(h->h_rr, m, hG, m, h->h_theta, h->h_theta + kLdq, hy, m, bw);
         } else {
           auto leading = [&](const double* theta) {
             std::vector<double> zero(m, 0.0);
             const EigDecision d0 = analyze(rq, theta, zero.data(), m, n, false);
             const int want = d0.enough ? std::max(d0.kw, d0.kvec) : cap / 4;
-            return round_up(want + kEigBlock, kEigBlock) + kEigBlock;
+            return round_up(want + bw, bw) + bw;
           };
           rr_ok = host_rayleigh_ritz_leading(h->h_rr, m, hG, m, h->h_theta, h->h_theta + kLdq,
-                                             hy, m, leading);
+                                             hy, m, leading, bw);
         }
         if (sw::eig_trace()) {
           timespec ts1;
@@ -698,10 +716,10 @@
           goto restart_lanczos;
         }
         if (dc.enough && dc.converged) {
-          if (!dense && m < n && block_multiplicity_suspect(rq, dc, h->h_theta, m)) {
+          if (!dense && m < n && block_multiplicity_suspect(rq, dc, h->h_theta, m, bw)) {
             if (sw::eig_trace())
               fprintf(stderr, "[sc] %d equal Ritz values ahead of the decisive gap: dense path\n",
-                      kEigBlock);
+                      bw);
             SC_TRY(dense_fallback(7));
             break;
           }
@@ -709,18 +727,18 @@
           break;
         }
       }
-      if (m + kEigBlock > cap) {
+      if (m + bw > cap) {
         if (++cycles > rq.max_cycles) {
           SC_TRY(dense_fallback(1));
           break;
         }
         int want = dc.enough ? std::max(dc.kw, dc.kvec) : cap / 4;
-        int keep = round_up(want + kEigBlock, kEigBlock);
-        keep = std::max(kEigBlock, std::min(keep, cap - 2 * kEigBlock));
+        int keep = round_up(want + bw, bw);
+        keep = std::max(bw, std::min(keep, cap - 2 * bw));
         launch_basis_times_Y(s, ptr<double>(h->Q), kLdq, m, ptr<double>(h->Y), kLdq, keep,
                              ptr<double>(h->Q2), kLdq, n, 0);
         launch_copy_block(s, ptr<double>(h->Q) + m, kLdq, ptr<double>(h->Q2) + keep, kLdq, n,
-                          kEigBlock);
+                          bw);
         std::swap(h->Q, h->Q2);
         launch_set_diag_T(s, ptr<double>(h->T), kLdq, kLdq, theta_d, keep);
         SC_TRY(check_last(h, "restart launch"));
@@ -745,6 +763,7 @@
         h->krylov_cycles = cycles;
         h->krylov_ahead = ahead;
         h->krylov_free = op.free_op;
+        h->krylov_block = bw;
       }
     }
   }
@@ -763,7 +782,7 @@
   }
   if (diag) {
     diag->eig_matvec_passes = passes;
-    diag->eig_block = kEigBlock;
+    diag->eig_block = n > kDenseMax ? bw : kEigBlock;
     diag->eig_basis = m;
     diag->eig_cycles = cycles;
     diag->eig_max_residual = dc.max_resid;
@@ -780,14 +799,17 @@
   return SC_OK;
 }
 
-extern "C" int sc_stage_krylov_state(sc_handle h, int32_t* info, double* q, double* t, double* g,
-                                     double* c, double* p) {
+static int krylov_state(sc_handle h, int32_t* info, double* q, double* t, double* g, double* c,
+                        double* p, bool any_width) {
   if (!h) return SC_ERR_INVALID;
   if (!info) return fail(h, SC_ERR_INVALID, "krylov state: info is NULL");
   if (h->krylov_m <= 0)
     return fail(h, SC_ERR_INVALID,
                 "krylov state: the last solve on this handle was not block Lanczos (dense "
                 "Jacobi, tridiagonal or general path), or none has run");
+  if (!any_width && h->krylov_block != kEigBlock)
+    return fail(h, SC_ERR_INVALID,
+                "krylov state: the last solve ran on 16-vector blocks (sc_stage_krylov_state_w)");
   SC_HIP(h, hipSetDevice(h->device));
   const int m = h->krylov_m, n = h->krylov_n;
   memset(info, 0, 8 * sizeof(int32_t));
@@ -796,17 +818,26 @@
   info[2] = h->krylov_free ? 1 : 0;
   info[3] = h->krylov_ahead;
   info[4] = h->krylov_cycles;
+  if (any_width) info[5] = h->krylov_block;
+  const int bw = h->krylov_block;
   hipStream_t s = h->stream;
   const size_t row = (size_t)m * sizeof(double), pitch = (size_t)kLdq * sizeof(double);
   if (q) SC_HIP(h, hipMemcpy2DAsync(q, row, h->Q.p, pitch, row, n, hipMemcpyDeviceToHost, s));
   if (t) SC_HIP(h, hipMemcpy2DAsync(t, row, h->T.p, pitch, row, m, hipMemcpyDeviceToHost, s));
   if (g)
-    SC_HIP(h, hipMemcpyAsync(g, h->G.p, kEigBlock * kEigBlock * sizeof(double),
-                             hipMemcpyDeviceToHost, s));
+    SC_HIP(h, hipMemcpyAsync(g, h->G.p, bw * bw * sizeof(double), hipMemcpyDeviceToHost, s));
   if (c) SC_HIP(h, hipMemcpyAsync(c, h->cvec.p, (size_t)n * sizeof(double), hipMemcpyDeviceToHost, s));
   if (p) SC_HIP(h, hipMemcpyAsync(p, h->pvec.p, (size_t)n * sizeof(double), hipMemcpyDeviceToHost, s));
   SC_HIP(h, hipStreamSynchronize(s));
   return SC_OK;
+}
+extern "C" int sc_stage_krylov_state(sc_handle h, int32_t* info, double* q, double* t, double* g,
+                                     double* c, double* p) {
+  return krylov_state(h, info, q, t, g, c, p, false);
+}
+extern "C" int sc_stage_krylov_state_w(sc_handle h, int32_t* info, double* q, double* t, double* g,
+                                       double* c, double* p) {
+  return krylov_state(h, info, q, t, g, c, p, true);
 }
 
 static double now_us() {
diff --git a/spectralcluster_amd/csrc/free_api.hip b/spectralcluster_amd/csrc/free_api.hip
--- a/spectralcluster_amd/csrc/free_api.hip
+++ b/spectralcluster_amd/csrc/free_api.hip
@@ -18,6 +18,14 @@
   h->free_prune = on;
   return SC_OK;
 }
+extern "C" int sc_set_eig_wide(sc_handle h, int mode) {
+  if (!h) return SC_ERR_INVALID;
+  if (mode < -1 || mode > 2) return fail(h, SC_ERR_INVALID, "eig wide mode: -1, 0, 1 or 2");
+  h->eig_wide = mode;
+  return SC_OK;
+}
+int eig_wide_mode(sc_handle h) { return h->eig_wide >= 0 ? h->eig_wide : sw::eig_wide(); }
+
 static bool free_prune_on(sc_handle h) {
   return h->free_prune >= 0 ? h->free_prune != 0 : !sw::free_no_prune();
 }
@@ -42,7 +50,7 @@
   SC_TRY(grow(h, h->fscal, 4 * sizeof(double)));
   SC_TRY(grow(h, h->fwords, ((size_t)2 * n + kOvfWords) * sizeof(int)));
   SC_TRY(grow(h, h->fcand, (size_t)n * free_candidate_cap() * sizeof(int)));
-  SC_TRY(grow(h, h->fY, (size_t)n * kEigBlock * sizeof(double)));
+  SC_TRY(grow(h, h->fY, (size_t)n * kEigBlockWide * sizeof(double)));
   SC_TRY(grow(h, h->fq2part, free_q2part_bytes(n)));
   SC_TRY(grow(h, h->fmx64, free_mx64_bytes(n)));
   SC_TRY(grow(h, h->ftau64, free_tau64_bytes(n)));
@@ -178,9 +186,9 @@
 }
 
 static void plain_matvec(hipStream_t s, const double* A, int ld, int n, bool sym_mv,
-                         const double* Vs, double* W, double* slabs) {
+                         const double* Vs, double* W, double* slabs, int bw = kEigBlock) {
   if (sym_mv)
-    launch_block_matvec_sym(s, A, ld, n, nullptr, nullptr, Vs, kEigBlock, Vs, W, slabs);
+    launch_block_matvec_sym(s, A, ld, n, nullptr, nullptr, Vs, bw, Vs, W, slabs, bw);
   else
     launch_block_matvec(s, A, ld, n, nullptr, nullptr, Vs, kEigBlock, Vs, W);
 }
@@ -214,18 +222,18 @@
 
 void free_apply_operator(hipStream_t s, const double* A, int ld, int n, bool sym_mv,
                          const double* cvec, const double* pvec, const double* V, int ldv,
-                         const double* Vs, double* fY, double* W, double* slabs) {
-  plain_matvec(s, A, ld, n, sym_mv, Vs, fY, slabs);
+                         const double* Vs, double* fY, double* W, double* slabs, int bw) {
+  plain_matvec(s, A, ld, n, sym_mv, Vs, fY, slabs, bw);
   if (sym_mv)
-    launch_block_matvec_sym(s, A, ld, n, cvec, pvec, V, ldv, fY, W, slabs);
+    launch_block_matvec_sym(s, A, ld, n, cvec, pvec, V, ldv, fY, W, slabs, bw);
   else
     launch_block_matvec(s, A, ld, n, cvec, pvec, V, ldv, fY, W);
 }
 void free_apply_operator(sc_handle h, const double* A, int ld, int n, bool sym_mv,
-                         const double* V, int ldv) {
+                         const double* V, int ldv, int bw) {
   free_apply_operator(h->stream, A, ld, n, sym_mv, ptr<double>(h->cvec), ptr<double>(h->pvec), V,
                       ldv, ptr<double>(h->Vs), ptr<double>(h->fY), ptr<double>(h->W),
-                      ptr<double>(h->mvsym));
+                      ptr<double>(h->mvsym), bw);
 }
 
 extern "C" int sc_stage_diffuse_rowstats(sc_handle h, const double* a, int n, int mode,
@@ -279,12 +287,16 @@
   return SC_OK;
 }
 
-extern "C" int sc_stage_block_operator(sc_handle h, int count, const int32_t* ns,
-                                       const double* const* matrices, const double* const* cvecs,
-                                       const double* const* pvecs,
-                                       const double* const* vs_scales, const double* const* vs,
-                                       double* const* ws, int route) {
+static int block_operator(sc_handle h, int count, const int32_t* ns, const double* const* matrices,
+                          const double* const* cvecs, const double* const* pvecs,
+                          const double* const* vs_scales, const double* const* vs,
+                          double* const* ws, int route, int bw) {
   if (!h) return SC_ERR_INVALID;
+  if (bw != kEigBlock && bw != kEigBlockWide)
+    return fail(h, SC_ERR_INVALID, "block operator: width 8 or 16");
+  if (bw == kEigBlockWide && (!(route & SC_BLOCK_ROUTE_SYM) || (route & SC_BLOCK_ROUTE_GROUPED)))
+    return fail(h, SC_ERR_INVALID,
+                "block operator: 16-vector blocks run on the upper-triangle route of single launches");
   const int known = SC_BLOCK_ROUTE_SYM | SC_BLOCK_ROUTE_TWO_PRODUCT | SC_BLOCK_ROUTE_GROUPED;
   if (count < 1 || count > kGroupMax || !ns || !matrices || !vs || !ws || (route & ~known))
     return fail(h, SC_ERR_INVALID, "bad block operator request");
@@ -336,22 +348,22 @@
     const double* sz = (vs_scales && vs_scales[z]) ? vs_scales[z] : cz;
     if (cz) SC_TRY(device(n, cz, &c));
     if (pz) SC_TRY(device(n, pz, &p));
-    SC_TRY(device((size_t)n * kEigBlock, vs[z], &V));
-    scaled.assign(vs[z], vs[z] + (size_t)n * kEigBlock);
+    SC_TRY(device((size_t)n * bw, vs[z], &V));
+    scaled.assign(vs[z], vs[z] + (size_t)n * bw);
     if (sz)
       for (int r = 0; r < n; ++r)
-        for (int j = 0; j < kEigBlock; ++j) scaled[(size_t)r * kEigBlock + j] *= sz[r];
-    SC_TRY(device((size_t)n * kEigBlock, scaled.data(), &Vs));
-    SC_TRY(device((size_t)n * kEigBlock, nullptr, &W));
-    if (two) SC_TRY(device((size_t)n * kEigBlock, nullptr, &fY[z]));
-    if (sym) SC_TRY(device(matvec_sym_workspace_doubles(n), nullptr, &slabs));
+        for (int j = 0; j < bw; ++j) scaled[(size_t)r * bw + j] *= sz[r];
+    SC_TRY(device((size_t)n * bw, scaled.data(), &Vs));
+    SC_TRY(device((size_t)n * bw, nullptr, &W));
+    if (two) SC_TRY(device((size_t)n * bw, nullptr, &fY[z]));
+    if (sym) SC_TRY(device(matvec_sym_workspace_doubles(n, bw), nullptr, &slabs));
     mv[z].S = S;
     mv[z].ld = ld;
     mv[z].n = n;
     mv[z].cvec = c;
     mv[z].pvec = p;
     mv[z].V = V;
-    mv[z].ldv = kEigBlock;
+    mv[z].ldv = bw;
     mv[z].Vs = Vs;
     mv[z].W = W;
     mv[z].slabs = slabs;
@@ -375,9 +387,10 @@
       const MatvecItem& a = mv[z];
       if (two)
         free_apply_operator(s, a.S, a.ld, a.n, sym, a.cvec, a.pvec, a.V, a.ldv, a.Vs, fY[z], a.W,
-                            a.slabs);
+                            a.slabs, bw);
       else if (sym)
-        launch_block_matvec_sym(s, a.S, a.ld, a.n, a.cvec, a.pvec, a.V, a.ldv, a.Vs, a.W, a.slabs);
+        launch_block_matvec_sym(s, a.S, a.ld, a.n, a.cvec, a.pvec, a.V, a.ldv, a.Vs, a.W, a.slabs,
+                                bw);
       else
         launch_block_matvec(s, a.S, a.ld, a.n, a.cvec, a.pvec, a.V, a.ldv, a.Vs, a.W);
     }
@@ -385,8 +398,22 @@
   SC_TRY(check_last(h, "block operator launch"));
   for (int z = 0; z < count; ++z)
     if (mv[z].n > 0)
-      SC_HIP(h, hipMemcpyAsync(ws[z], mv[z].W, (size_t)mv[z].n * kEigBlock * sizeof(double),
+      SC_HIP(h, hipMemcpyAsync(ws[z], mv[z].W, (size_t)mv[z].n * bw * sizeof(double),
                                hipMemcpyDeviceToHost, s));
   SC_HIP(h, hipStreamSynchronize(s));
   return SC_OK;
 }
+extern "C" int sc_stage_block_operator(sc_handle h, int count, const int32_t* ns,
+                                       const double* const* matrices, const double* const* cvecs,
+                                       const double* const* pvecs,
+                                       const double* const* vs_scales, const double* const* vs,
+                                       double* const* ws, int route) {
+  return block_operator(h, count, ns, matrices, cvecs, pvecs, vs_scales, vs, ws, route, kEigBlock);
+}
+extern "C" int sc_stage_block_operator_w(sc_handle h, int count, const int32_t* ns,
+                                         const double* const* matrices, const double* const* cvecs,
+                                         const double* const* pvecs,
+                                         const double* const* vs_scales, const double* const* vs,
+                                         double* const* ws, int route, int width) {
+  return block_operator(h, count, ns, matrices, cvecs, pvecs, vs_scales, vs, ws, route, width);
+}
diff --git a/spectralcluster_amd/csrc/handle.h b/spectralcluster_amd/csrc/handle.h
--- a/spectralcluster_amd/csrc/handle.h
+++ b/spectralcluster_amd/csrc/handle.h
@@ -138,6 +138,8 @@
   int free_ev[5] = {-1, -1, -1, -1, -1};
   int krylov_m = 0, krylov_n = 0, krylov_cycles = 0, krylov_ahead = 0;
   bool krylov_free = false;
+  int krylov_block = kEigBlock;
+  int eig_wide = -1;
   BlurLaunch last_blur;
 };
 
@@ -344,10 +346,12 @@
                    const int* plan = nullptr);
 int free_fix_overflow(sc_handle h, const double* A, int ld, int n, bool* changed, bool* too_many);
 void free_apply_operator(sc_handle h, const double* A, int ld, int n, bool sym_mv,
-                         const double* V, int ldv);
+                         const double* V, int ldv, int bw = kEigBlock);
 void free_apply_operator(hipStream_t s, const double* A, int ld, int n, bool sym_mv,
                          const double* cvec, const double* pvec, const double* V, int ldv,
-                         const double* Vs, double* fY, double* W, double* slabs);
+                         const double* Vs, double* fY, double* W, double* slabs,
+                         int bw = kEigBlock);
+int eig_wide_mode(sc_handle h);
 bool wants_full_spectrum(const EigRequest& rq);
 
 int device_is_symmetric(sc_handle h, const double* m, int n, int ld, bool* out);
diff --git a/spectralcluster_amd/csrc/sc_internal.h b/spectralcluster_amd/csrc/sc_internal.h
--- a/spectralcluster_amd/csrc/sc_internal.h
+++ b/spectralcluster_amd/csrc/sc_internal.h
@@ -15,6 +15,10 @@
 
 constexpr int kWave = 64;
 constexpr int kEigBlock = 8;
+constexpr int kEigBlockWide = 16;
+constexpr int kEigWideCap = 112;
+constexpr int kEigWideMinN = 4096;
+constexpr int kHostRRGram = kEigBlockWide * kEigBlockWide;
 constexpr int kEigBasisCap = 128;
 constexpr int kLdq = kEigBasisCap + kEigBlock;
 constexpr int kDenseMax = 128;
@@ -197,10 +201,10 @@
 void launch_block_matvec(hipStream_t s, const double* S, int ld, int n,
                          const double* cvec, const double* pvec, const double* V,
                          int ldv, const double* Vs, double* W);
-size_t matvec_sym_workspace_doubles(int n);
+size_t matvec_sym_workspace_doubles(int n, int bw = kEigBlock);
 void launch_block_matvec_sym(hipStream_t s, const double* S, int ld, int n, const double* cvec,
                              const double* pvec, const double* V, int ldv, const double* Vs,
-                             double* W, double* ws);
+                             double* W, double* ws, int bw = kEigBlock);
 void launch_proj_partial(hipStream_t s, const double* Q, int ldq, int m,
                          const double* W, int n, double* partial);
 int proj_blocks(int n);
@@ -220,8 +224,9 @@
   int parity = 0;
   int nparts = 0;
   bool three_pass = false;
-};
-size_t lz_partial_doubles(int n);
+  int bw = kEigBlock;
+};
+size_t lz_partial_doubles(int n, int bw = kEigBlock);
 void launch_lz_link(hipStream_t s, const EigWorkspace& ws, LzChain* chain, int n, int m,
                     int pre, int next, int store_col, const double* vs_scale, int col0,
                     bool init_random, uint64_t seed, bool zero_T);
diff --git a/spectralcluster_amd/csrc/switches.h b/spectralcluster_amd/csrc/switches.h
--- a/spectralcluster_amd/csrc/switches.h
+++ b/spectralcluster_amd/csrc/switches.h
@@ -1,6 +1,7 @@
 #ifndef SPECTRALCLUSTER_AMD_SWITCHES_H_
 #define SPECTRALCLUSTER_AMD_SWITCHES_H_
 
+#include <algorithm>
 #include <cstdlib>
 #include <cstring>
 
@@ -33,6 +34,10 @@
 }
 inline int matvec_sym_min_n() {
   static const int v = getenv("SC_MATVEC_SYM_MIN_N") ? atoi(getenv("SC_MATVEC_SYM_MIN_N")) : 4096;
+  return v;
+}
+inline int eig_wide() {
+  static const int v = getenv("SC_EIG_WIDE") ? std::min(2, std::max(0, atoi(getenv("SC_EIG_WIDE")))) : 0;
   return v;
 }
 inline bool kmeans_single() {
```
